# roymor1/OptimalStrategiesAgainstGenerativeAttacks

Measured on AMD Instinct MI355X. Metric: GIM episodes/sec (64x64x3, m=1 n=5 k=10), higher is better.
Workload: dtype f32

## Files before the change

### include/gim_hip.h

```cpp
#ifndef GIM_HIP_H
#define GIM_HIP_H

#include <stddef.h>
#include <stdint.h>

#ifdef __cplusplus
extern "C" {
#endif

#define GIM_OK 0
#define GIM_E_BADARG (-1)
#define GIM_E_LAUNCH (-2)

const char* gim_last_error(void);
int gim_version(void);

typedef struct {
    int32_t N, H, W, Cin, Cout, KH, ups;
    float pre_slope;
    int32_t pool, wfold, res_ups;
    int32_t tune_tile, tune_ksplit, tune_wgrad;
    int32_t out_zeroed;
    float post_slope;
    int32_t prec;
} gim_conv_shape;

int gim_conv2d_fold_weights(const float* w, float* f, int Cout, int Cin, int KH, void* stream);
typedef struct {
    const float* w;
    float* f;
    int32_t Cout, Cin, KH, reserved;
} gim_fold_job;
int gim_conv2d_fold_weights_batched(const gim_fold_job* jobs, const int32_t* tab, int n_blocks, void* stream);

int gim_conv2d_fwd(const float* x, const float* w, const float* bias, const float* sigma, const float* residual,
                   float* y, const gim_conv_shape* s, void* stream);

int gim_conv2d_dgrad(const float* dy, const float* w, const float* sigma, const float* mask_x, float* dx,
                     const gim_conv_shape* s, void* stream);

int gim_conv2d_dgrad_res(const float* dy, const float* w, const float* sigma, const float* mask_x, const float* res_half,
                         float res_scale, float* dx, const gim_conv_shape* s, void* stream);

int gim_conv2d_wgrad_slabs(const gim_conv_shape* s);
int gim_conv2d_wgrad(const float* dy, const float* x, float* slabs, float* bias_slabs, int n_slabs, const gim_conv_shape* s,
                     void* stream);

int gim_wgrad_finish(const float* slabs, const float* bias_slabs, int n_slabs, const float* w, const float* sigma,
                     const float* u, const float* v, float* dw, float* db, float* scratch, int Cout, int Cin, int KH,
                     int fold, float* acc_dw, float* acc_db, void* stream);

int gim_spectral_sigma(const float* w, float* u, float* v, float* sigma, float* u_out, float* v_out, float* scratch,
                       int Cout, int Cin, int KH, int training, void* stream);

typedef struct {
    const float* w;
    float* u;
    float* v;
    int64_t off_sigma, off_u, off_v, off_scratch;
    int32_t Cout, Cin, KH, reserved;
} gim_sn_job;
int gim_spectral_sigma_batched(const gim_sn_job* jobs, int n_jobs, const int32_t* tab_cols, int n_col_blocks,
                               const int32_t* tab_rows, int n_row_blocks, float* out_base, int training, void* stream);

int gim_conv2d_transpose_weights(const float* w, float* wt, int Cout, int Cin, int KF, void* stream);
int gim_conv2d_dgrad_t(const float* dy, const float* wt, const float* sigma, const float* mask_x, float* dx,
                       const gim_conv_shape* shape, void* stream);

int gim_conv2d_xfold_weights(const float* w, float* wx, int Cout, int Cin, int KH, int J, void* stream);
int gim_conv2d_dgrad_xfold(const float* dy, const float* wx, const float* sigma, const float* mask_x, float* dx,
                           const gim_conv_shape* shape, int J, void* stream);

int gim_pad_image(const float* x, float* xp, int N, int H, int W, int C, int pad, float slope, void* stream);
int gim_conv2d_pack_rows_weights(const float* w, float* wp, int Cout, int Cin, int KH, void* stream);
int gim_conv2d_fwd_rows(const float* xp, const float* wp, const float* bias, const float* sigma, const float* residual,
                        float* y, const gim_conv_shape* shape, void* stream);
int gim_conv2d_wgrad_rows_acc(const float* dy, const float* xp, float* acc, float* bias_acc, const gim_conv_shape* shape, void* stream);

int gim_conv2d_pack_subpixel_weights(const float* wf, float* wm, int Cout, int Cin, int KH, void* stream);
int gim_depth_to_space2(const float* y4, const float* bias, float* y, int N, int Hs, int Ws, int C, float post_slope, void* stream);

int gim_conv_launch_plan(const gim_conv_shape* shape, int kind, int32_t* out);

int gim_conv2d_wgrad_acc(const float* dy, const float* x, float* acc, float* bias_acc, const gim_conv_shape* shape, void* stream);

typedef struct {
    const float* src;
    const float* bias_src;
    const float* w;
    const float* sigma;
    const float* u;
    const float* v;
    float* tmp;
    float* partial;
    float* grad_w;
    float* grad_b;
    int32_t Cout, Cin, K, fold;
    int32_t n_chunks, exclusive;
} gim_wgrad_job;
int gim_wgrad_finish_batched(const gim_wgrad_job* jobs, int n_jobs, const int32_t* tab, int n_blocks, const int32_t* tab_sn,
                             int n_blocks_sn, void* stream);

int gim_colsum(const float* x, float* out, float* scratch, int64_t rows, int C, void* stream);

int gim_colsum_acc(const float* x, float* out, float* scratch, int64_t rows, int C, void* stream);
int gim_colsum2(const float* a, const float* b, float* out_a, float* out_b, int rows, int C, int accumulate, void* stream);

int gim_norm_fwd(const float* x, const float* scale, const float* shift, const float* residual, float* y, float* stats,
                 int N, int HW, int C, int mode, float eps, void* stream);
int gim_norm_fwd_act(const float* x, const float* scale, const float* shift, const float* residual, float* y, float* stats,
                     int N, int HW, int C, int mode, float eps, float post_slope, void* stream);
int gim_norm_bwd(const float* dy, const float* x, const float* scale, const float* stats, float* dx, float* dscale_nc,
                 float* dshift_nc, int N, int HW, int C, int mode, void* stream);

int gim_avgpool2_fwd(const float* x, float* y, int N, int H, int W, int C, void* stream);
int gim_avgpool2_fwd_act(const float* x, float* y, int N, int H, int W, int C, float in_slope, void* stream);
int gim_box2_fwd(const float* x, float* p, int N, int H, int W, int C, float slope, void* stream);
int gim_add_n(const float* a, const float* b, const float* c, const float* d, float* out, int64_t n, void* stream);
int gim_add_avgpool2_bwd(const float* g, const float* dy_pooled, float* out, int N, int H, int W, int C, void* stream);
int gim_avgpool2_bwd(const float* dy, float* dx, int N, int H, int W, int C, void* stream);
int gim_upsample2x_bwd(const float* dy_up, const float* mask_x, float slope, float* dx, int N, int H, int W, int C, void* stream);

int gim_maxpool_lrelu_fwd(const float* x, float* y, int32_t* idx, int N, int HW, int C, float slope, void* stream);
int gim_maxpool_lrelu_bwd(const float* dy, const float* y, const int32_t* idx, float* dx, int N, int HW, int C, float slope, void* stream);

int gim_attn_prob_fwd(const float* f, const float* g, float* P, int batch, int T, int K, void* stream);

int gim_bgemm(const float* A, const float* B, float* C, int batch, int M, int N, int K,
              int64_t sAb, int64_t sAi, int64_t sAk, int64_t sBb, int64_t sBk, int64_t sBj, void* stream);

typedef struct {
    const float* A;
    const float* B;
    float* C;
    const float* bias;
    int32_t M, N, K, ldc;
    int64_t sAi, sAk, sBk, sBj;
    int32_t flags, reserved;
} gim_gemm_job;
int gim_bgemm_grouped(const gim_gemm_job* jobs, const int32_t* tiles, int n_tiles, void* stream);
int gim_colsum_grouped(const gim_gemm_job* jobs, const int32_t* tiles, int n_tiles, void* stream);

int gim_softmax_dim1_fwd(const float* s, float* p, int B, int R, int Ccols, void* stream);
int gim_softmax_dim1_bwd(const float* dp, const float* p, float* ds, int B, int R, int Ccols, void* stream);

int gim_scale_add_fwd(const float* a, const float* x, const float* gamma, float* y, int64_t n, void* stream);
int gim_scale_add_fwd_act(const float* a, const float* x, const float* gamma, float* y, int64_t n, float post_slope, void* stream);
int gim_scale_add_bwd(const float* dy, const float* a, const float* gamma, float* da, float* dgamma, float* scratch,
                      int64_t n, void* stream);

int gim_tanh_fwd(const float* x, float* y, int64_t n, void* stream);
int gim_tanh_bwd(const float* dy, const float* y, float* dx, int64_t n, void* stream);

int gim_nchw_to_nhwc(const float* x, float* y, int N, int C, int HW, void* stream);
int gim_nhwc_to_nchw(const float* x, float* y, int N, int C, int HW, void* stream);

int gim_set_stats_fwd(const float* x, float* mean, float* std, int B, int t, int D, int64_t ld_mean, int64_t ld_std, void* stream);
int gim_set_stats_bwd(const float* x, const float* dmean, const float* dstd, float* dx, int B, int t, int D,
                      int64_t ld_dmean, int64_t ld_dstd, void* stream);

int gim_bce_logits_fwd(const float* x, float* loss, float target, int n, void* stream);
int gim_bce_logits_bwd(const float* dloss, const float* x, float* dx, float target, int n, void* stream);

int gim_sum_dim1(const float* x, float* y, int B, int t, int D, float scale, void* stream);
int gim_repeat_dim1(const float* x, float* y, int B, int t, int D, float scale, void* stream);
// ... 125 lines not shown
```

### optimalstrategiesagainstgenerativeattacks_amd/_lib.py

```python
import ctypes
import os
from ctypes import POINTER, c_float, c_int, c_int32, c_int64, c_uint64, c_void_p

_HERE = os.path.dirname(os.path.abspath(__file__))
LIB_PATH = os.environ.get("GIM_LIB_PATH") or os.path.join(_HERE, "csrc", "libgim_hip.so")


class GimConvShape(ctypes.Structure):
    _fields_ = [("N", c_int32), ("H", c_int32), ("W", c_int32), ("Cin", c_int32), ("Cout", c_int32),
                ("KH", c_int32), ("ups", c_int32), ("pre_slope", c_float),
                ("pool", c_int32), ("wfold", c_int32), ("res_ups", c_int32),
                ("tune_tile", c_int32), ("tune_ksplit", c_int32), ("tune_wgrad", c_int32),
                ("out_zeroed", c_int32), ("post_slope", c_float), ("prec", c_int32)]


class GimInferConv(ctypes.Structure):
    _fields_ = [("N", c_int32), ("H", c_int32), ("W", c_int32), ("Cin", c_int32), ("Cout", c_int32),
                ("KH", c_int32), ("stride", c_int32)]


P = c_void_p
SP = POINTER(GimConvShape)


class GimFoldJob(ctypes.Structure):
    _fields_ = [("w", P), ("f", P), ("Cout", c_int32), ("Cin", c_int32), ("KH", c_int32), ("reserved", c_int32)]


class GimSnJob(ctypes.Structure):
    _fields_ = [("w", P), ("u", P), ("v", P), ("off_sigma", c_int64), ("off_u", c_int64), ("off_v", c_int64), ("off_scratch", c_int64),
                ("Cout", c_int32), ("Cin", c_int32), ("KH", c_int32), ("reserved", c_int32)]


class GimWgradJob(ctypes.Structure):
    _fields_ = [("src", P), ("bias_src", P), ("w", P), ("sigma", P), ("u", P), ("v", P), ("tmp", P), ("partial", P),
                ("grad_w", P), ("grad_b", P), ("Cout", c_int32), ("Cin", c_int32), ("K", c_int32), ("fold", c_int32),
                ("n_chunks", c_int32), ("exclusive", c_int32)]


class GimGemmJob(ctypes.Structure):
    _fields_ = [("A", P), ("B", P), ("C", P), ("bias", P), ("M", c_int32), ("N", c_int32), ("K", c_int32), ("ldc", c_int32),
                ("sAi", c_int64), ("sAk", c_int64), ("sBk", c_int64), ("sBj", c_int64), ("flags", c_int32), ("reserved", c_int32)]


SIGNATURES = {
    "gim_conv2d_fwd": [P, P, P, P, P, P, SP, P],
    "gim_conv2d_dgrad": [P, P, P, P, P, SP, P],
    "gim_conv2d_dgrad_res": [P, P, P, P, P, c_float, P, SP, P],
    "gim_conv2d_wgrad_slabs": [SP],
    "gim_conv2d_wgrad": [P, P, P, P, c_int, SP, P],
    "gim_wgrad_finish": [P, P, c_int, P, P, P, P, P, P, P, c_int, c_int, c_int, c_int, P, P, P],
    "gim_conv2d_fold_weights": [P, P, c_int, c_int, c_int, P],
    "gim_conv2d_fold_weights_batched": [P, P, c_int, P],
    "gim_spectral_sigma": [P, P, P, P, P, P, P, c_int, c_int, c_int, c_int, P],
    "gim_spectral_sigma_batched": [P, c_int, P, c_int, P, c_int, P, c_int, P],
    "gim_colsum": [P, P, P, c_int64, c_int, P],
    "gim_norm_fwd": [P, P, P, P, P, P, c_int, c_int, c_int, c_int, c_float, P],
    "gim_norm_fwd_act": [P, P, P, P, P, P, c_int, c_int, c_int, c_int, c_float, c_float, P],
    "gim_norm_bwd": [P, P, P, P, P, P, P, c_int, c_int, c_int, c_int, P],
    "gim_avgpool2_fwd": [P, P, c_int, c_int, c_int, c_int, P],
    "gim_avgpool2_fwd_act": [P, P, c_int, c_int, c_int, c_int, c_float, P],
    "gim_box2_fwd": [P, P, c_int, c_int, c_int, c_int, c_float, P],
    "gim_add_n": [P, P, P, P, P, c_int64, P],
    "gim_add_avgpool2_bwd": [P, P, P, c_int, c_int, c_int, c_int, P],
    "gim_avgpool2_bwd": [P, P, c_int, c_int, c_int, c_int, P],
    "gim_upsample2x_bwd": [P, P, c_float, P, c_int, c_int, c_int, c_int, P],
    "gim_maxpool_lrelu_fwd": [P, P, P, c_int, c_int, c_int, c_float, P],
    "gim_maxpool_lrelu_bwd": [P, P, P, P, c_int, c_int, c_int, c_float, P],
    "gim_bgemm": [P, P, P, c_int, c_int, c_int, c_int, c_int64, c_int64, c_int64, c_int64, c_int64, c_int64, P],
    "gim_attn_prob_fwd": [P, P, P, c_int, c_int, c_int, P],
    "gim_softmax_dim1_fwd": [P, P, c_int, c_int, c_int, P],
    "gim_softmax_dim1_bwd": [P, P, P, c_int, c_int, c_int, P],
    "gim_bgemm_grouped": [P, P, c_int, P],
    "gim_colsum_grouped": [P, P, c_int, P],
    "gim_scale_add_fwd": [P, P, P, P, c_int64, P],
    "gim_scale_add_fwd_act": [P, P, P, P, c_int64, c_float, P],
    "gim_scale_add_bwd": [P, P, P, P, P, P, c_int64, P],
    "gim_tanh_fwd": [P, P, c_int64, P],
    "gim_tanh_bwd": [P, P, P, c_int64, P],
    "gim_nchw_to_nhwc": [P, P, c_int, c_int, c_int, P],
    "gim_nhwc_to_nchw": [P, P, c_int, c_int, c_int, P],
    "gim_set_stats_fwd": [P, P, P, c_int, c_int, c_int, c_int64, c_int64, P],
    "gim_set_stats_bwd": [P, P, P, P, c_int, c_int, c_int, c_int64, c_int64, P],
    "gim_bce_logits_fwd": [P, P, c_float, c_int, P],
    "gim_bce_logits_bwd": [P, P, P, c_float, c_int, P],
    "gim_sum_dim1": [P, P, c_int, c_int, c_int, c_float, P],
    "gim_repeat_dim1": [P, P, c_int, c_int, c_int, c_float, P],
    "gim_noise_combine": [P, P, P, c_int, c_int, c_int, c_int, P],
    "gim_concat2": [P, P, P, c_int64, c_int, c_int, c_int, c_int, P],
    "gim_slice_channels": [P, P, c_int64, c_int, c_int, P],
    "gim_conv2d_wgrad_acc": [P, P, P, P, SP, P],
    "gim_wgrad_finish_batched": [P, c_int, P, c_int, P, c_int, P],
    "gim_colsum_acc": [P, P, P, c_int64, c_int, P],
    "gim_colsum2": [P, P, P, P, c_int, c_int, c_int, P],
    "gim_conv_launch_plan": [SP, c_int, P],
    "gim_conv2d_transpose_weights": [P, P, c_int, c_int, c_int, P],
    "gim_conv2d_dgrad_t": [P, P, P, P, P, SP, P],
    "gim_conv2d_xfold_weights": [P, P, c_int, c_int, c_int, c_int, P],
    "gim_conv2d_dgrad_xfold": [P, P, P, P, P, SP, c_int, P],
    "gim_episode_gather": [P, P, P, P, c_int, c_int, c_int, c_int, P],
    "gim_resize_bilinear_u8": [P, c_int64, c_int, c_int, c_int, c_int, P, c_int, c_int, P, P, c_int, P, P, c_int, P],
    "gim_maxpool_gather": [P, P, P, P, c_int, c_int, c_int, c_float, P],
    "gim_softmax_dim1_bwd_dp": [P, P, P, P, c_int, c_int, c_int, P],
    "gim_set_stats_bwd_bwd": [P, P, P, P, P, P, c_int, c_int, c_int, c_int64, c_int64, P],
    "gim_lrelu_mask_mul": [P, P, c_float, P, c_int64, P],
    "gim_sqsum_rows_fwd": [P, P, c_int, c_int64, P],
    "gim_sqsum_rows_bwd": [P, P, P, c_int, c_int64, P],
    "gim_img_att_mix_fwd": [P, P, P, P, P, P, P, P, c_int64, c_int, P],
    "gim_img_att_mix_bwd": [P, P, P, P, P, P, P, P, P, P, P, P, P, P, c_int64, c_int, P],
    "gim_adam_step": [P, P, P, P, c_int64, P, P, c_int, c_float, c_float, c_float, c_float, P, P],
    "gim_adam_step_scaled": [P, P, P, P, c_int64, P, P, c_int, c_float, c_float, c_float, c_float, P, P, P],
    "gim_ema_update": [P, P, c_int64, c_float, P, P],
    "gim_buffer_exchange": [P, P, c_int64, P],
    "gim_adam_optimism": [P, P, P, P, c_int64, P, P, c_int, c_float, c_float, c_float, c_float, P, P, P],
    "gim_spin": [c_int, P],
    "gim_pad_image": [P, P, c_int, c_int, c_int, c_int, c_int, c_float, P],
    "gim_conv2d_pack_rows_weights": [P, P, c_int, c_int, c_int, P],
    "gim_conv2d_pack_subpixel_weights": [P, P, c_int, c_int, c_int, P],
    "gim_depth_to_space2": [P, P, P, c_int, c_int, c_int, c_int, c_float, P],
    "gim_conv2d_fwd_rows": [P, P, P, P, P, P, SP, P],
    "gim_conv2d_wgrad_rows_acc": [P, P, P, P, SP, P],
    "gim_conv2d_infer": [P, P, P, P, P, POINTER(GimInferConv), P],
    "gim_maxpool2_act": [P, P, c_int, c_int, c_int, c_int, c_int, P],
    "gim_channel_affine": [P, P, P, P, c_int64, c_int, P],
    "gim_se_tail": [P, P, P, P, P, P, P, c_int, c_int, c_int, c_int, c_int, P],
    "gim_pair_score": [P, P, P, c_int, c_int, P],
    "gim_l2norm_rows": [P, P, c_int, c_int, P],
    "gim_absdiff": [P, P, P, c_int64, P],
    "gim_bn_slabs": [c_int64],
    "gim_bn_partials_floats": [c_int64, c_int],
    "gim_bn_stats": [P, P, P, P, P, P, P, c_int64, c_int, c_float, c_float, P],
    "gim_bn_relu_maxpool2_fwd": [P, P, P, P, P, P, c_int, c_int, c_int, c_int, P],
    "gim_bn_pool_bwd_reduce": [P, P, P, P, P, P, P, P, P, P, P, c_int, c_int, c_int, c_int, P],
    "gim_bn_pool_bwd_dx": [P, P, P, P, P, P, P, P, P, c_int, c_int, c_int, c_int, P],
    "gim_bn_stats_record": [P, P, P, c_int64, c_int, P],
    "gim_bn_stats_merge": [P, POINTER(c_int64), c_int, c_int, P, P, P, P, P, c_float, c_float, P],
    "gim_bn_pool_bwd_dx_total": [P, P, P, P, P, P, P, P, P, c_int, c_int, c_int, c_int, c_int64, P],
    "gim_absdiff_bwd": [P, P, P, P, P, c_int64, P],
    "gim_logit_accuracy": [P, c_int, c_int, P, P],
    "gim_bn_apply_fwd": [P, P, P, P, P, P, P, c_int64, c_int, P],
    "gim_bn_bwd_reduce": [P, P, P, P, P, P, P, P, P, P, P, P, P, P, c_int64, c_int, P],
    "gim_bn_bwd_dx": [P, P, P, P, P, P, P, P, P, P, c_int64, c_int, P],
    "gim_bn_bwd_dx_total": [P, P, P, P, P, P, P, P, P, P, c_int64, c_int64, c_int, P],
    "gim_prelu_fwd": [P, P, P, c_int64, c_int, P],
    "gim_prelu_bwd": [P, P, P, P, P, P, P, c_int64, c_int, P],
    "gim_se_tail_bwd": [P, P, P, P, P, c_int, c_int, c_int, c_int, P],
    "gim_subsample2_fwd": [P, P, c_int, c_int, c_int, c_int, P],
    "gim_subsample2_bwd": [P, P, c_int, c_int, c_int, c_int, P],
    "gim_dropout": [P, P, c_int64, c_float, c_uint64, c_uint64, P],
    "gim_l2norm_rows_bwd": [P, P, P, c_int, c_int, P],
    "gim_col_l2norm_fwd": [P, P, c_int, c_int, P],
    "gim_col_l2norm_bwd": [P, P, P, c_int, c_int, P],
    "gim_arcface_margin_fwd": [P, P, P, c_int, c_int, c_float, c_float, c_float, c_float, c_float, P],
    "gim_arcface_margin_bwd": [P, P, P, P, c_int, c_int, c_float, c_float, c_float, c_float, c_float, P],
    "gim_softmax_ce_fwd": [P, P, P, P, P, c_int, c_int, P],
    "gim_softmax_ce_bwd": [P, P, P, P, P, c_int, c_int, P],
    "gim_conv2d_strided_fwd": [P, P, P, P, POINTER(GimInferConv), P],
    "gim_conv2d_strided_dgrad": [P, P, P, POINTER(GimInferConv), c_int, P],
    "gim_conv2d_strided_wgrad_workspace": [POINTER(GimInferConv), POINTER(c_int64)],
    "gim_conv2d_strided_wgrad": [P, P, P, P, POINTER(GimInferConv), c_int, P, P],
    "gim_conv2d_strided_plan": [POINTER(GimInferConv), c_int, P],
    "gim_roc_slices": [c_int64, c_int64],
    "gim_roc_counts": [P, c_int, P, c_int, P, c_int, P, P],
    "gim_roc_calibrate": [P, c_int, P, c_int, P, P, P],
    "gim_version": [],
}

_lib = None


def load():
    global _lib
    if _lib is not None:
        return _lib
    if not os.path.exists(LIB_PATH):
        raise RuntimeError(
            "libgim_hip.so not found at %s: the HIP extension is not built "
            "(run __graft_entry__.build()); there is no CPU fallback" % LIB_PATH)
# ... 16 lines not shown
```

### optimalstrategiesagainstgenerativeattacks_amd/csrc/conv_f16.inc

```
typedef _Float16 h8_t __attribute__((ext_vector_type(8)));
typedef _Float16 h4_t __attribute__((ext_vector_type(4)));
typedef _Float16 h2_t __attribute__((ext_vector_type(2)));
typedef float f32x2 __attribute__((ext_vector_type(2)));
typedef short s16x4 __attribute__((ext_vector_type(4)));

template <bool SAT>
__device__ __forceinline__ f32x4 sat16(f32x4 v) {
    if constexpr (SAT) {
#pragma unroll
        for (int e = 0; e < 4; ++e) v[e] = __builtin_amdgcn_fmed3f(v[e], -65504.f, 65504.f);
    }
    return v;
}
template <bool SAT>
__device__ __forceinline__ h8_t cvt8_f16(f32x4 lo, f32x4 hi) {
    lo = sat16<SAT>(lo); hi = sat16<SAT>(hi);
    const h2_t a = __builtin_convertvector(f32x2{lo[0], lo[1]}, h2_t), b = __builtin_convertvector(f32x2{lo[2], lo[3]}, h2_t);
    const h2_t c = __builtin_convertvector(f32x2{hi[0], hi[1]}, h2_t), d = __builtin_convertvector(f32x2{hi[2], hi[3]}, h2_t);
    return h8_t{a[0], a[1], b[0], b[1], c[0], c[1], d[0], d[1]};
}
template <bool SAT>
__device__ __forceinline__ h4_t cvt4_f16(f32x4 v) {
    v = sat16<SAT>(v);
    const h2_t a = __builtin_convertvector(f32x2{v[0], v[1]}, h2_t), b = __builtin_convertvector(f32x2{v[2], v[3]}, h2_t);
// ... 70 lines not shown
#pragma unroll
        for (int i = 0; i < B_ROWS; ++i) {
            rb[i][0] = buf_load4(rw, b_voff[i], sb);
            rb[i][1] = buf_load4(rw, b_voff[i], sb + 16u);
        }
        k_c0 += KB;
        if (k_c0 == p.Ca) {
            k_c0 = 0;
            if (++k_tb == g.Tw) { k_tb = 0; ++k_ta; }
            set_tap(k_ta, k_tb);
        }
    };
    const bool has_act = p.pre_slope != 1.0f;
    auto store_tiles = [&](int buf) {
#pragma unroll
        for (int i = 0; i < A_ROWS; ++i) {
            if (has_act) {
#pragma unroll
                for (int q = 0; q < 2; ++q)
#pragma unroll
                    for (int e = 0; e < 4; ++e) ra[i][q][e] = __builtin_amdgcn_fmed3f(ra[i][q][e], ra[i][q][e] * p.pre_slope, p.pos_inf);
            }
            *reinterpret_cast<h8_t*>(&As[buf * A_SZ + (arow + 64 * i) * LDH + aq]) = cvt8_f16<SAT>(ra[i][0], ra[i][1]);
        }
#pragma unroll
        for (int i = 0; i < B_ROWS; ++i)
            *reinterpret_cast<h8_t*>(&Bs[buf * B_SZ + (arow + 64 * i) * LDH + aq]) = cvt8_f16<false>(rb[i][0], rb[i][1]);
    };
    const int lane = t & 63, r = lane & 31, h = lane >> 5, wv = t >> 6;
    const int wm0 = (wv / WAVES_N) * 32 * TM, wn0 = (wv % WAVES_N) * 32 * TN;
    f32x16 acc[TM][TN];
#pragma unroll
    for (int i = 0; i < TM; ++i)
#pragma unroll
        for (int j = 0; j < TN; ++j)
#pragma unroll
            for (int e = 0; e < 16; ++e) acc[i][j][e] = 0.f;
    const int nk_all = p.Ktot / KB;
    const int ks0 = kslice * p.kper;
    const int nk = min(nk_all, ks0 + p.kper);
    seek(ks0 * KB);
    load_tiles();
    store_tiles(0);
    __syncthreads();
    auto kstep = [&](int ks, auto BUFC, auto MAINC) {
        constexpr int buf = decltype(BUFC)::value;
        constexpr bool MAIN = decltype(MAINC)::value;
        if (MAIN || ks + 1 < nk) load_tiles();
        __builtin_amdgcn_sched_barrier(0);
        const _Float16* Ab = As + buf * A_SZ;
        const _Float16* Bb = Bs + buf * B_SZ;
        h8_t a[2][TM], b[2][TN];
#pragma unroll
        for (int kk = 0; kk < 2; ++kk) {
#pragma unroll
            for (int i = 0; i < TM; ++i) a[kk][i] = *reinterpret_cast<const h8_t*>(&Ab[(wm0 + 32 * i + r) * LDH + 16 * kk + 8 * h]);
#pragma unroll
            for (int j = 0; j < TN; ++j) b[kk][j] = *reinterpret_cast<const h8_t*>(&Bb[(wn0 + 32 * j + r) * LDH + 16 * kk + 8 * h]);
        }
#pragma unroll
        for (int kk = 0; kk < 2; ++kk)
#pragma unroll
            for (int i = 0; i < TM; ++i)
#pragma unroll
                for (int j = 0; j < TN; ++j)
                    acc[i][j] = __builtin_amdgcn_mfma_f32_32x32x16_f16(a[kk][i], b[kk][j], acc[i][j], 0, 0, 0);
        __builtin_amdgcn_sched_barrier(0);
        if (MAIN || ks + 1 < nk) store_tiles(buf ^ 1);
        __syncthreads();
    };
    int ks = ks0;
    for (; ks + 2 < nk; ks += 2) {
        kstep(ks, std::integral_constant<int, 0>(), std::true_type());
        kstep(ks + 1, std::integral_constant<int, 1>(), std::true_type());
    }
    for (; ks < nk; ks += 2) {
        kstep(ks, std::integral_constant<int, 0>(), std::false_type());
        if (ks + 1 < nk) kstep(ks + 1, std::integral_constant<int, 1>(), std::false_type());
    }

    EpiCtx ec;
    const bool first = kslice == 0;
    bool has_res, has_mask;
    epi_fill<false, false>(ec, p, g, first, has_res, has_mask);
    auto run = [&](auto MODEC) {
        constexpr int MODE = decltype(MODEC)::value;
#pragma unroll
        for (int i = 0; i < TM; ++i)
#pragma unroll
            for (int j = 0; j < TN; ++j) {
                const int co = n0 + wn0 + 32 * j + r;
                const bool cok = co < p.Cb;
                const float bv = (p.bias && first && cok) ? p.bias[co] : 0.f;
                float a_[16];
#pragma unroll
                for (int e = 0; e < 16; ++e) a_[e] = acc[i][j][e];
                epi_block<16, MODE>(ec, a_, m0 + wm0 + 32 * i + 4 * h, co, cok, bv);
            }
    };
    epi_dispatch<0, 0>(p, has_res, has_mask, run);
}

template <int BM, int BN, int TM, int TN, bool SAT = true>
__global__ __launch_bounds__(256, 2) void conv_igemm_patch_f16_kernel(const ConvP p) {
    constexpr int KB = 32, LDH = 40;
    constexpr int WAVES_N = BN / (32 * TN), WAVES_M = BM / (32 * TM);
    static_assert(WAVES_M * WAVES_N == 4, "4 waves per workgroup");
    constexpr int P_PER = BM == 64 ? 4 : 5;
    constexpr int B_ROWS = BN / 64;
    constexpr int B_SZ = BN * LDH;
    extern __shared__ __attribute__((aligned(16))) _Float16 patch16_lds[];
    const Geo& g = p.g;
    const int t = threadIdx.x, lane = t & 63, wv = t >> 6;
    const int kslice = blockIdx.z;
    const int m0 = blockIdx.x * BM, n0 = blockIdx.y * BN;
    const int Wt = min(g.W, BM), logWt = 31 - __builtin_clz(Wt);
    const int PW = Wt + 2, PP = (BM / Wt + 2) * PW;
    const int P_SZ = (PP * LDH + 7) & ~7;
    _Float16* Ps = patch16_lds;
    _Float16* Bs = patch16_lds + 2 * P_SZ;
    const int n_img = m0 >> (g.logH + g.logW);
    const int oy0 = ((m0 >> g.logW) & (g.H - 1)) + g.off_y, ox0 = (m0 & (g.W - 1)) + g.off_x;
    const int KF2 = g.KF * g.KFw;
    const __amdgpu_buffer_rsrc_t rx = __builtin_amdgcn_make_buffer_rsrc((void*)p.x, 0, p.x_bytes, 0x00020000);
    const __amdgpu_buffer_rsrc_t rw = __builtin_amdgcn_make_buffer_rsrc((void*)p.w, 0, 0xFFFFFFFFu, 0x00020000);
    unsigned p_voff[P_PER];
    int p_lds[P_PER];
#pragma unroll
    for (int i = 0; i < P_PER; ++i) {
        const int q = t + 256 * i, pp = q >> 2, grp = q & 3;
        const int pr = pp / PW, pc = pp - pr * PW;
        const int iy = oy0 + pr, ix = ox0 + pc;
        const bool v = pp < PP && (unsigned)iy < (unsigned)g.H && (unsigned)ix < (unsigned)g.W;
        p_voff[i] = v ? (unsigned)((((n_img * g.Hin + iy) * g.Win + ix) * p.Ca + grp * 8) * 4) : BUF_OOB;
        p_lds[i] = pp < PP ? pp * LDH + grp * 8 : -1;
    }
    unsigned b_voff[B_ROWS];
    const int brow = t >> 2, bq = (t & 3) * 8;
#pragma unroll
    for (int i = 0; i < B_ROWS; ++i) b_voff[i] = (unsigned)((min(n0 + brow + 64 * i, p.Cb - 1) * KF2 * p.Cin_w + bq) * 4);
    const bool has_act = p.pre_slope != 1.0f;
    f32x4 rp[P_PER][2], rb[B_ROWS][2];
    auto load_patch = [&](int c0) __attribute__((always_inline)) {
#pragma unroll
        for (int i = 0; i < P_PER; ++i) {
            rp[i][0] = buf_load4(rx, p_voff[i], (unsigned)(c0 * 4));
            rp[i][1] = buf_load4(rx, p_voff[i], (unsigned)(c0 * 4) + 16u);
        }
    };
    int p_wr = 0;
    auto store_patch = [&]() __attribute__((always_inline)) {
#pragma unroll
        for (int i = 0; i < P_PER; ++i) {
            if (has_act) {
#pragma unroll
                for (int q = 0; q < 2; ++q)
#pragma unroll
                    for (int e = 0; e < 4; ++e) rp[i][q][e] = __builtin_amdgcn_fmed3f(rp[i][q][e], rp[i][q][e] * p.pre_slope, p.pos_inf);
            }
            if (p_lds[i] >= 0) *reinterpret_cast<h8_t*>(&Ps[p_wr + p_lds[i]]) = cvt8_f16<SAT>(rp[i][0], rp[i][1]);
        }
        p_wr = p_wr ? 0 : P_SZ;
    };
    auto load_b = [&](int ta, int tb, int c0) __attribute__((always_inline)) {
        const int wtap = (g.wa_base + g.wa_step * ta) * g.KFw + g.wb_base + g.wb_step * tb;
        const unsigned sb = (unsigned)((wtap * p.Cin_w + c0) * 4);
#pragma unroll
// ... 11 lines not shown
    int a_row[3][TM];
#pragma unroll
    for (int i = 0; i < TM; ++i) {
        const int q = wm0 + 32 * i + r;
        const int base = ((q >> logWt) * PW + (q & (Wt - 1))) * LDH + 8 * h;
#pragma unroll
        for (int ta = 0; ta < 3; ++ta) a_row[ta][i] = base + ta * PW * LDH;
    }
    f32x16 acc[TM][TN];
#pragma unroll
    for (int i = 0; i < TM; ++i)
#pragma unroll
        for (int j = 0; j < TN; ++j)
#pragma unroll
            for (int e = 0; e < 16; ++e) acc[i][j][e] = 0.f;
    const int nchunk = p.Ca / KB;
    const int ch0 = kslice * (p.kper / 9);
    const int ch1 = min(nchunk, ch0 + p.kper / 9);
    load_patch(ch0 * KB);
    load_b(0, 0, ch0 * KB);
    store_patch();
    store_b(0);
    __syncthreads();
    auto kstep = [&](int ch, bool more_chunks, auto TAPC, auto BBC) __attribute__((always_inline)) {
        constexpr int TAP = decltype(TAPC)::value, BB = decltype(BBC)::value;
        constexpr int TA = TAP / 3, TB = TAP % 3;
        if (TAP == 0 && more_chunks) load_patch((ch + 1) * KB);
        if (TAP < 8) load_b((TAP + 1) / 3, (TAP + 1) % 3, ch * KB);
        else if (more_chunks) load_b(0, 0, (ch + 1) * KB);
        __builtin_amdgcn_sched_barrier(0);
        const _Float16* Bb = Bs + BB * B_SZ;
        h8_t a[2][TM], b[2][TN];
#pragma unroll
        for (int kk = 0; kk < 2; ++kk) {
#pragma unroll
            for (int i = 0; i < TM; ++i) a[kk][i] = *reinterpret_cast<const h8_t*>(&Ps[a_row[TA][i] + TB * LDH + 16 * kk]);
#pragma unroll
            for (int j = 0; j < TN; ++j) b[kk][j] = *reinterpret_cast<const h8_t*>(&Bb[(wn0 + 32 * j + r) * LDH + 16 * kk + 8 * h]);
        }
#pragma unroll
        for (int kk = 0; kk < 2; ++kk)
#pragma unroll
            for (int i = 0; i < TM; ++i)
#pragma unroll
                for (int j = 0; j < TN; ++j)
                    acc[i][j] = __builtin_amdgcn_mfma_f32_32x32x16_f16(a[kk][i], b[kk][j], acc[i][j], 0, 0, 0);
        __builtin_amdgcn_sched_barrier(0);
        if (TAP < 8 || more_chunks) store_b(BB ^ 1);
        if (TAP == 8 && more_chunks) store_patch();
        __syncthreads();
    };
    int pbuf = 0;
    auto chunk = [&](int ch, auto B0C) __attribute__((always_inline)) {
        constexpr int B0 = decltype(B0C)::value;
        using Ba = std::integral_constant<int, B0>;
        using Bb_ = std::integral_constant<int, B0 ^ 1>;
        const bool more_chunks = ch + 1 < ch1;
        kstep(ch, more_chunks, std::integral_constant<int, 0>(), Ba());
        kstep(ch, more_chunks, std::integral_constant<int, 1>(), Bb_());
        kstep(ch, more_chunks, std::integral_constant<int, 2>(), Ba());
        kstep(ch, more_chunks, std::integral_constant<int, 3>(), Bb_());
        kstep(ch, more_chunks, std::integral_constant<int, 4>(), Ba());
        kstep(ch, more_chunks, std::integral_constant<int, 5>(), Bb_());
        kstep(ch, more_chunks, std::integral_constant<int, 6>(), Ba());
        kstep(ch, more_chunks, std::integral_constant<int, 7>(), Bb_());
        kstep(ch, more_chunks, std::integral_constant<int, 8>(), Ba());
        const int d = pbuf ? -P_SZ : P_SZ;
        pbuf ^= 1;
#pragma unroll
        for (int ta = 0; ta < 3; ++ta)
#pragma unroll
            for (int i = 0; i < TM; ++i) a_row[ta][i] += d;
    };
    int ch = ch0;
    for (; ch + 1 < ch1; ch += 2) {
        chunk(ch, std::integral_constant<int, 0>());
        chunk(ch + 1, std::integral_constant<int, 1>());
    }
    if (ch < ch1) chunk(ch, std::integral_constant<int, 0>());

    EpiCtx ec;
    const bool first = kslice == 0;
    bool has_res, has_mask;
    epi_fill<true, false>(ec, p, g, first, has_res, has_mask);
    auto run = [&](auto MODEC) {
        constexpr int MODE = decltype(MODEC)::value;
#pragma unroll
        for (int i = 0; i < TM; ++i)
#pragma unroll
            for (int j = 0; j < TN; ++j) {
                const int co = n0 + wn0 + 32 * j + r;
                const bool cok = co < p.Cb;
                const float bv = (p.bias && first && cok) ? p.bias[co] : 0.f;
                float a_[16];
#pragma unroll
                for (int e = 0; e < 16; ++e) a_[e] = acc[i][j][e];
                epi_block<16, MODE>(ec, a_, m0 + wm0 + 32 * i + 4 * h, co, cok, bv);
            }
    };
    epi_dispatch<0, 0>(p, has_res, has_mask, run);
}

__device__ __forceinline__ int wg16_off(int row, int chunk) {
    return 256 * row + 16 * (chunk ^ (((row & 3) << 2) | ((row >> 2) & 3)));
}

template <bool FASTB, bool SAT = true>
__global__ __launch_bounds__(256, 2) void conv_wgrad_f16_kernel(const WgP p) {
    constexpr int BM = 128, BN = 128, TM = 2, TN = 2, WBK = 32;
    constexpr int IMG = WBK * 256;
    constexpr int PER = 4;
    __shared__ __attribute__((aligned(16))) char lds[4 * IMG];
    const Geo& g = p.g;
    const int t = threadIdx.x;
    int bx, by, bz;
    if (!wgrad_block(p, bx, by, bz)) return;
    const int j0 = bx * BN, co0 = by * BM;
    const int mbeg = bz * p.mper, mend = min(p.M, mbeg + p.mper);
    const int He = g.Hin << g.ups, We = g.Win << g.ups;
    const int cq = t & 31, ak = t >> 5;
    const int ac = cq * 4;
    const int j = j0 + ac;
    const bool b_jok = j < p.Kcols;
    const int tap = b_jok ? j / p.Cin : 0;
    const int ci = b_jok ? j - tap * p.Cin : 0;
    const int ta = tap / g.Tw, tb = tap - ta * g.Tw;
    const int dh = ta + g.off_y, dw = tb + g.off_x;
    const bool do_bias = p.bias_slabs != nullptr && bx == 0;
    const int b_bias = ((g.off_y < 0 ? -g.off_y : 0) * g.Win + (g.off_x < 0 ? -g.off_x : 0)) * p.Cin * 4;
    const __amdgpu_buffer_rsrc_t rxb = __builtin_amdgcn_make_buffer_rsrc((void*)((const char*)p.x - b_bias), 0, p.x_bytes + (unsigned)b_bias, 0x00020000);
    unsigned a_v[PER], b_l[PER];
    int b_dx[PER], b_dy[PER], st_off[PER];
    const bool a_cok = co0 + ac < p.Cout;
#pragma unroll
    for (int i = 0; i < PER; ++i) {
        const int row = ak + 8 * i;
        a_v[i] = a_cok ? (unsigned)((row * p.Cout + co0 + ac) * 4) : BUF_OOB;
        b_dy[i] = (row >> g.logW) * g.s_in + dh;
        b_dx[i] = (row & (g.W - 1)) * g.s_in + dw;
        b_l[i] = b_jok ? (unsigned)(((b_dy[i] * g.Win + b_dx[i]) * p.Cin + ci) * 4 + b_bias) : BUF_OOB;
        st_off[i] = wg16_off(row, cq >> 1) + 8 * (cq & 1);
    }
    f32x4 ra[PER], rb[PER];
    float bsum[4] = {0.f, 0.f, 0.f, 0.f};
    auto load_tiles = [&](int mb) {
        const int left = mend - mb;
        const __amdgpu_buffer_rsrc_t ra_rs = __builtin_amdgcn_make_buffer_rsrc(
            (void*)(p.dy + (long long)mb * p.Cout), 0, (unsigned)min(left, WBK) * (unsigned)p.Cout * 4u, 0x00020000);
#pragma unroll
        for (int i = 0; i < PER; ++i) ra[i] = buf_load4(ra_rs, a_v[i], 0);
        if constexpr (FASTB) {
            const int n = mb >> (g.logH + g.logW);
            const int oys = ((mb >> g.logW) & (g.H - 1)) * g.s_in, oxs = (mb & (g.W - 1)) * g.s_in;
            const unsigned u = (unsigned)((((n * g.Hin + oys) * g.Win) + oxs) * p.Cin * 4);
#pragma unroll
            for (int i = 0; i < PER; ++i) {
                const bool v = (unsigned)(oys + b_dy[i]) < (unsigned)He && (unsigned)(oxs + b_dx[i]) < (unsigned)We;
                rb[i] = buf_load4(rxb, v ? b_l[i] : BUF_OOB, u);
            }
        } else {
#pragma unroll
            for (int i = 0; i < PER; ++i) {
                const int m = mb + ak + 8 * i;
                const int n = m >> (g.logH + g.logW);
                const int iy = ((m >> g.logW) & (g.H - 1)) * g.s_in + dh;
                const int ix = (m & (g.W - 1)) * g.s_in + dw;
                const bool v = b_jok && m < mend && (unsigned)iy < (unsigned)He && (unsigned)ix < (unsigned)We;
// ... 137 lines not shown
```

### optimalstrategiesagainstgenerativeattacks_amd/csrc/conv_igemm.hip

```cpp
#include <stdlib.h>

#include "common.h"
#include <type_traits>

#define PM_MAX_PIXELS 16
#define PM_MIN_IMAGES 32
#define BK 16

struct Geo {
    int N, H, W, logH, logW;
    int Hin, Win;
    int ups;
    int s_in;
    int s_in_x;
    int off_y, off_x;
    int Th, Tw;
    int KF;
    int KFw;
    int wa_base, wa_step, wb_base, wb_step;
    int os, py, px;
    int pc, pc_kind, pc_K;
    int pm;
    unsigned long long pm_perm;
    unsigned long long pm_perm_cls[4];
};

__host__ __device__ __forceinline__ int pm_pixel(unsigned long long perm, int slot) { return (int)((perm >> (4 * slot)) & 15ull); }


__device__ __forceinline__ void geo_row(const Geo& g, int m, int& n, int& oy, int& ox) {
    if (g.pm) {
        const int slot = m / g.N;
        n = m - slot * g.N;
        const int pix = pm_pixel(g.pm_perm, slot);
        oy = pix >> g.logW;
        ox = pix & (g.W - 1);
    } else {
        n = m >> (g.logH + g.logW);
        oy = (m >> g.logW) & (g.H - 1);
        ox = m & (g.W - 1);
    }
}

__host__ __device__ __forceinline__ void geo_select_class(Geo& g, int cls) {
    const int py = cls >> 1, px = cls & 1;
    const int K = g.pc_K, pd = (K - 1) / 2;
    g.py = py;
    g.px = px;
    if (g.pc_kind == 0) {
        const int oy = (py - pd) >> 1, ox = (px - pd) >> 1;
        g.off_y = oy;
        g.off_x = ox;
        g.wa_base = pd + 1 - py + 2 * oy;
        g.wb_base = pd + 1 - px + 2 * ox;
        g.wa_step = g.wb_step = 2;
    } else {
        const int th = (K + 1) / 2;
        const int a0 = (py + pd) & 1, b0 = (px + pd) & 1;
        g.off_y = ((py + pd - a0) >> 1) - (th - 1);
        g.off_x = ((px + pd - b0) >> 1) - (th - 1);
        g.wa_base = a0 + 2 * (th - 1);
        g.wb_base = b0 + 2 * (th - 1);
        g.wa_step = g.wb_step = -2;
    }
}

struct ConvP {
    Geo g;
    const float* x;
    const float* w;
    const float* bias;
    const float* sigma;
    const float* res;
    const float* mask_x;
    float* y;
    int Ca, Cb;
    int Cin_w;
    int M;
    int Ktot;
    const float* zero;
    unsigned x_bytes;
    int tune_ks;
    int tune_tile;
    int y_zeroed;
    int tune_kind;
    float pos_inf;
    float pre_slope, mask_slope, out_scale;
    float res_scale;
    float post_slope;
    int res_ups;
    int ksplit;
    int kper;
    int pix;
    int f16;
    const float* slope;
    int epi;
    int no_split;
};

__device__ __attribute__((aligned(16))) float g_zero4[4] = {0.f, 0.f, 0.f, 0.f};

static const float* zero_page() {
    static const float* z = [] {
        void* ptr = nullptr;
        if (hipGetSymbolAddress(&ptr, HIP_SYMBOL(g_zero4)) != hipSuccess) ptr = nullptr;
        return (const float*)ptr;
    }();
    return z;
}

typedef unsigned u32x4 __attribute__((ext_vector_type(4)));
#define BUF_OOB 0x80000000u
#define BUF_MAX_BYTES 0x7FFFFFF0ull
__device__ __forceinline__ f32x4 buf_load4(__amdgpu_buffer_rsrc_t r, unsigned voff, unsigned soff) {
    return __builtin_bit_cast(f32x4, __builtin_amdgcn_raw_buffer_load_b128(r, voff, soff, 0));
}

struct EpiCtx {
    __amdgpu_buffer_rsrc_t ry, rr, rm;
    float scale, mask_slope, post_slope;
    float res_scale;
    int M, Cb, logH, logW, Hm1, Wm1, os, py, px, Ho, Wo;
    int pmN;
    unsigned long long pm_perm;
    bool atom, remap;
};

template <int MODE>
__device__ __forceinline__ void epi_elem_off(const EpiCtx& c, int m, int co, unsigned& o, unsigned& ro) {
    const int n = m >> (c.logH + c.logW);
    const int oy = ((m >> c.logW) & c.Hm1) * c.os + c.py;
    const int ox = (m & c.Wm1) * c.os + c.px;
    o = (unsigned)((((n * c.Ho + oy) * c.Wo + ox) * c.Cb + co) * 4);
    if constexpr (MODE == 2 || MODE == 4) ro = (unsigned)((((n * (c.Ho >> 1) + (oy >> 1)) * (c.Wo >> 1) + (ox >> 1)) * c.Cb + co) * 4);
}

template <int NE, int MODE>
__device__ __forceinline__ void epi_block(const EpiCtx& c, const float (&a)[NE], int mbase, int co, bool cok, float bv, float sv = 1.f) {
    constexpr int CH = NE < 8 ? NE : 8;
    const unsigned rowb = (unsigned)c.Cb * 4u;
#pragma unroll
    for (int e0 = 0; e0 < NE; e0 += CH) {
        unsigned off[CH], roff[(MODE == 2 || MODE == 4) ? CH : 1];
        if (!c.remap && !c.pmN && MODE != 2 && MODE != 4) {
            const unsigned base = (unsigned)((mbase * c.Cb + co) * 4);
#pragma unroll
            for (int q = 0; q < CH; ++q) off[q] = base + (unsigned)(((e0 + q) & 3) + 8 * ((e0 + q) >> 2)) * rowb;
        } else if (c.Wm1 >= 3 && !c.pmN) {
#pragma unroll
            for (int g4 = 0; g4 < CH; g4 += 4) {
                unsigned o, ro = 0;
                epi_elem_off<MODE>(c, mbase + 8 * ((e0 + g4) >> 2), co, o, ro);
#pragma unroll
                for (int k = 0; k < 4 && g4 + k < CH; ++k) {
                    off[g4 + k] = o + (unsigned)(k * c.os) * rowb;
                    if constexpr (MODE == 2 || MODE == 4) roff[g4 + k] = ro + (unsigned)(((c.px + k * c.os) >> 1) - (c.px >> 1)) * rowb;
                }
            }
        } else if (c.pmN) {
            const int slot0 = mbase / c.pmN, n0 = mbase - slot0 * c.pmN;
            const int pixa = pm_pixel(c.pm_perm, slot0), pixb = pm_pixel(c.pm_perm, (slot0 + 1) & 15);
#pragma unroll
            for (int q = 0; q < CH; ++q) {
                const int d = ((e0 + q) & 3) + 8 * ((e0 + q) >> 2);
                const bool wrap = n0 + d >= c.pmN;
                const int n = wrap ? n0 + d - c.pmN : n0 + d, pix = wrap ? pixb : pixa;
                const int oy = ((pix >> c.logW) & c.Hm1) * c.os + c.py, ox = (pix & c.Wm1) * c.os + c.px;
                off[q] = (unsigned)((((n * c.Ho + oy) * c.Wo + ox) * c.Cb + co) * 4);
                if constexpr (MODE == 2 || MODE == 4) roff[q] = (unsigned)((((n * (c.Ho >> 1) + (oy >> 1)) * (c.Wo >> 1) + (ox >> 1)) * c.Cb + co) * 4);
            }
        } else {
#pragma unroll
            for (int q = 0; q < CH; ++q) {
                unsigned ro = 0;
                epi_elem_off<MODE>(c, mbase + ((e0 + q) & 3) + 8 * ((e0 + q) >> 2), co, off[q], ro);
                if constexpr (MODE == 2 || MODE == 4) roff[q] = ro;
            }
        }
#pragma unroll
        for (int q = 0; q < CH; ++q) {
            const unsigned bad = (cok && mbase + ((e0 + q) & 3) + 8 * ((e0 + q) >> 2) < c.M) ? 0u : BUF_OOB;
            off[q] |= bad;
            if constexpr (MODE == 2 || MODE == 4) roff[q] |= bad;
        }
        float ld[(MODE == 0 || MODE == 5) ? 1 : CH], ld2[MODE == 4 ? CH : 1];
        if constexpr (MODE == 4) {
#pragma unroll
            for (int q = 0; q < CH; ++q) ld[q] = __builtin_bit_cast(float, __builtin_amdgcn_raw_buffer_load_b32(c.rm, off[q], 0, 0));
#pragma unroll
            for (int q = 0; q < CH; ++q) ld2[q] = __builtin_bit_cast(float, __builtin_amdgcn_raw_buffer_load_b32(c.rr, roff[q], 0, 0));
        } else if constexpr (MODE == 1 || MODE == 2) {
#pragma unroll
            for (int q = 0; q < CH; ++q) ld[q] = __builtin_bit_cast(float, __builtin_amdgcn_raw_buffer_load_b32(c.rr, MODE == 2 ? roff[q] : off[q], 0, 0));
        } else if constexpr (MODE == 3) {
#pragma unroll
            for (int q = 0; q < CH; ++q) ld[q] = __builtin_bit_cast(float, __builtin_amdgcn_raw_buffer_load_b32(c.rm, off[q], 0, 0));
        }
        float v[CH];
#pragma unroll
        for (int q = 0; q < CH; ++q) {
            v[q] = a[e0 + q] * c.scale + bv;
            if constexpr (MODE == 1 || MODE == 2) v[q] += ld[q];
            if constexpr (MODE == 3 || MODE == 4) v[q] *= (ld[q] > 0.f ? 1.0f : c.mask_slope);
            if constexpr (MODE == 4) v[q] += c.res_scale * ld2[q];
            if constexpr (MODE == 5) v[q] = v[q] >= 0.f ? v[q] : v[q] * sv;
            else if constexpr (MODE != 3 && MODE != 4) v[q] = fmaxf(v[q], v[q] * c.post_slope);
        }
        if (c.atom) {
#pragma unroll
            for (int q = 0; q < CH; ++q) (void)__builtin_amdgcn_raw_ptr_buffer_atomic_fadd_f32(v[q], c.ry, off[q], 0, 0);
        } else {
#pragma unroll
            for (int q = 0; q < CH; ++q) __builtin_amdgcn_raw_buffer_store_b32(__builtin_bit_cast(unsigned, v[q]), c.ry, off[q], 0, 0);
        }
        __builtin_amdgcn_sched_barrier(0);
    }
}

template <bool PLAIN, bool PM>
__device__ __forceinline__ void epi_fill(EpiCtx& ec, const ConvP& p, const Geo& g, bool first, bool& has_res, bool& has_mask) {
    ec.scale = p.out_scale * (p.sigma ? 1.0f / p.sigma[0] : 1.0f);
    ec.mask_slope = p.mask_slope;
    ec.post_slope = p.post_slope;
    ec.res_scale = p.res_scale;
    has_res = p.res != nullptr && first;
    has_mask = p.mask_x != nullptr;
    ec.atom = p.ksplit > 1;
    ec.remap = PLAIN ? false : g.os != 1;
    ec.M = p.M; ec.Cb = p.Cb;
    ec.logH = g.logH; ec.logW = g.logW; ec.Hm1 = g.H - 1; ec.Wm1 = g.W - 1;
    ec.os = PLAIN ? 1 : g.os; ec.py = PLAIN ? 0 : g.py; ec.px = PLAIN ? 0 : g.px;
    ec.Ho = g.H * ec.os; ec.Wo = g.W * ec.os;
    ec.pmN = (PM && g.pm) ? g.N : 0;
    if constexpr (PM) ec.pm_perm = g.pm_perm;
    const unsigned ybytes = (unsigned)g.N * (unsigned)ec.Ho * (unsigned)ec.Wo * (unsigned)p.Cb * 4u;
    ec.ry = __builtin_amdgcn_make_buffer_rsrc((void*)p.y, 0, ybytes, 0x00020000);
    ec.rr = __builtin_amdgcn_make_buffer_rsrc((void*)p.res, 0, has_res ? ((p.res_ups || has_mask) ? ybytes >> 2 : ybytes) : 0u, 0x00020000);
    ec.rm = __builtin_amdgcn_make_buffer_rsrc((void*)p.mask_x, 0, has_mask ? ybytes : 0u, 0x00020000);
}

template <int EPI, int BMODE, class Run>
__device__ __forceinline__ void epi_dispatch(const ConvP& p, bool has_res, bool has_mask, Run&& run) {
    if constexpr (EPI == 1) {
        run(std::integral_constant<int, 5>());
    } else if (has_res) {
        if constexpr (BMODE == 1) run(std::integral_constant<int, 4>());
        else if (p.res_ups) run(std::integral_constant<int, 2>());
        else run(std::integral_constant<int, 1>());
    } else if (has_mask) {
        run(std::integral_constant<int, 3>());
    } else {
        run(std::integral_constant<int, 0>());
    }
}

constexpr int igemm_lds_bytes(int BM, int BN, int KB, int BMODE) {
    return 2 * (BM * (KB + 4) + (BMODE == 0 ? BN * (KB + 4) : KB * BN)) * 4;
}

template <int BM, int BN, int TM, int TN, int BMODE, int GENF, int KB, int EPI = 0>
__global__ __launch_bounds__(256, igemm_lds_bytes(BM, BN, KB, BMODE) <= 40960 ? 4 : 2) void conv_igemm_kernel(const ConvP p) {
    constexpr bool GEN = (GENF & 1) != 0;
    constexpr bool BSCALAR = (GENF & 2) != 0;
    constexpr bool N16 = BN == 16;
    constexpr int WAVES_N = N16 ? 1 : BN / (32 * TN);
    constexpr int WAVES_M = BM / (32 * TM);
    static_assert(WAVES_M * WAVES_N == 4, "4 waves per workgroup");
    constexpr int LDK = KB + 4;
    constexpr int QPR = KB / 4;
    constexpr int RP = 256 / QPR;
    constexpr int A_ROWS = BM / RP;
    constexpr int B_ROWS = (BN + RP - 1) / RP;
    constexpr int B_PER = KB * BN / 256;
    constexpr int B_U = BN / 4;
    constexpr int B_RSTEP = 256 / B_U;
    constexpr int B_PER4 = (KB + B_RSTEP - 1) / B_RSTEP;
    constexpr int LDA = LDK;
    constexpr int A_SZ = BM * LDA;
    constexpr int B_SZ = (BMODE == 0) ? BN * LDA : KB * BN;
    __shared__ __attribute__((aligned(16))) float lds[2 * A_SZ + 2 * B_SZ];
    float* As = lds;
    float* Bs = lds + 2 * A_SZ;

    Geo g = p.g;
    int kslice = blockIdx.z;
    if (g.pc) {
        geo_select_class(g, blockIdx.z & 3);
        g.pm_perm = p.g.pm_perm_cls[blockIdx.z & 3];
        kslice = blockIdx.z >> 2;
    }
    const int t = threadIdx.x;
    const int m0 = blockIdx.x * BM;
    const int n0 = blockIdx.y * BN;
    const int arow = t / QPR, aq = (t % QPR) * 4;
    const int He = g.Hin << g.ups, We = g.Win << g.ups;
    const int KF2 = g.KF * g.KFw;

    int a_oy[A_ROWS], a_ox[A_ROWS];
    long long a_off[A_ROWS];
    bool a_ok[A_ROWS];
#pragma unroll
    for (int i = 0; i < A_ROWS; ++i) {
        const int m = m0 + arow + RP * i;
        a_ok[i] = m < p.M;
// ... 260 lines not shown
            const int per = (nv + p.ksplit - 1) / p.ksplit;
            ks0 = kslice * per;
            nk = min(nv, ks0 + per);
            if (ks0 >= nk) {
                if (kslice != 0) return;
            }
            pm_seek(ks0);
            set_tap(k_ta, k_tb);
            pm_started = true;
        }
    }
    if constexpr (!GEN) { if (!pm_started) seek(ks0 * KB); }
    load_tiles(ks0 * KB);
    store_tiles(0);
    __syncthreads();
    auto kstep = [&](int ks, auto BUFC, auto MAINC) {
        constexpr int buf = decltype(BUFC)::value;
        constexpr bool MAIN = decltype(MAINC)::value;
        if (MAIN || ks + 1 < nk) load_tiles((ks + 1) * KB);
        __builtin_amdgcn_sched_barrier(0);
        const float* Ab = As + buf * A_SZ;
        const float* Bb = Bs + buf * B_SZ;
        if constexpr (N16) {
#pragma unroll
            for (int kk = 0; kk < KB / 16; ++kk) {
                f32x4 a[NB16], b;
#pragma unroll
                for (int i = 0; i < NB16; ++i) a[i] = *reinterpret_cast<const f32x4*>(&Ab[(wm0 + 16 * i + r16) * LDK + 16 * kk + 4 * q16]);
                if constexpr (BMODE == 0) {
                    b = *reinterpret_cast<const f32x4*>(&Bb[r16 * LDK + 16 * kk + 4 * q16]);
                } else {
#pragma unroll
                    for (int e = 0; e < 4; ++e) b[e] = Bb[(16 * kk + 4 * q16 + e) * BN + r16];
                }
#pragma unroll
                for (int e = 0; e < 4; ++e)
#pragma unroll
                    for (int i = 0; i < NB16; ++i) acc16[i] = __builtin_amdgcn_mfma_f32_16x16x4f32(a[i][e], b[e], acc16[i], 0, 0, 0);
            }
        } else {
            f32x4 a[KB / 8][TM], b[KB / 8][TN];
#pragma unroll
            for (int kk = 0; kk < KB / 8; ++kk) {
#pragma unroll
                for (int i = 0; i < TM; ++i) a[kk][i] = *reinterpret_cast<const f32x4*>(&Ab[(wm0 + 32 * i + r) * LDK + 8 * kk + 4 * h]);
#pragma unroll
                for (int j = 0; j < TN; ++j) {
                    if constexpr (BMODE == 0) {
                        b[kk][j] = *reinterpret_cast<const f32x4*>(&Bb[(wn0 + 32 * j + r) * LDK + 8 * kk + 4 * h]);
                    } else {
#pragma unroll
                        for (int e = 0; e < 4; ++e) b[kk][j][e] = Bb[(8 * kk + 4 * h + e) * BN + wn0 + 32 * j + r];
                    }
                }
            }
            if constexpr (TM * TN <= 2) __builtin_amdgcn_sched_barrier(0);
#pragma unroll
            for (int kk = 0; kk < KB / 8; ++kk)
#pragma unroll
                for (int e = 0; e < 4; ++e)
#pragma unroll
                    for (int i = 0; i < TM; ++i)
#pragma unroll
                        for (int j = 0; j < TN; ++j)
                            acc[i][j] = __builtin_amdgcn_mfma_f32_32x32x2f32(a[kk][i][e], b[kk][j][e], acc[i][j], 0, 0, 0);
        }
        __builtin_amdgcn_sched_barrier(0);
        if (MAIN || ks + 1 < nk) store_tiles(buf ^ 1);
        __syncthreads();
    };
    int ks = ks0;
    for (; ks + 2 < nk; ks += 2) {
        kstep(ks, std::integral_constant<int, 0>(), std::true_type());
        kstep(ks + 1, std::integral_constant<int, 1>(), std::true_type());
    }
    for (; ks < nk; ks += 2) {
        kstep(ks, std::integral_constant<int, 0>(), std::false_type());
        if (ks + 1 < nk) kstep(ks + 1, std::integral_constant<int, 1>(), std::false_type());
    }

    EpiCtx ec;
    const bool first = kslice == 0;
    bool has_res, has_mask;
    epi_fill<false, true>(ec, p, g, first, has_res, has_mask);
    auto run = [&](auto MODEC) {
        constexpr int MODE = decltype(MODEC)::value;
        if constexpr (N16) {
            const int co = n0 + r16;
            const bool cok = co < p.Cb;
            const float bv = (p.bias && first && cok) ? p.bias[co] : 0.f;
#pragma unroll
            for (int i = 0; i < NB16; ++i) {
                const float a[4] = {acc16[i][0], acc16[i][1], acc16[i][2], acc16[i][3]};
                if constexpr (MODE == 5) epi_block<4, MODE>(ec, a, m0 + wm0 + 16 * i + 4 * q16, co, cok, bv, (p.slope && cok) ? p.slope[co] : 1.f);
                else epi_block<4, MODE>(ec, a, m0 + wm0 + 16 * i + 4 * q16, co, cok, bv);
            }
        } else {
#pragma unroll
            for (int i = 0; i < TM; ++i)
#pragma unroll
                for (int j = 0; j < TN; ++j) {
                    const int co = n0 + wn0 + 32 * j + r;
                    const bool cok = co < p.Cb;
                    const float bv = (p.bias && first && cok) ? p.bias[co] : 0.f;
                    float a[16];
#pragma unroll
                    for (int e = 0; e < 16; ++e) a[e] = acc[i][j][e];
                    if constexpr (MODE == 5) epi_block<16, MODE>(ec, a, m0 + wm0 + 32 * i + 4 * h, co, cok, bv, (p.slope && cok) ? p.slope[co] : 1.f);
                    else epi_block<16, MODE>(ec, a, m0 + wm0 + 32 * i + 4 * h, co, cok, bv);
                }
        }
    };
    epi_dispatch<EPI, BMODE>(p, has_res, has_mask, run);
}

template <int BM, int BN, int TM, int TN, int BMODE, int EPI = 0>
__global__ __launch_bounds__(256, TM * TN <= 2 ? 3 : 2) void conv_igemm_patch_kernel(const ConvP p) {
    constexpr int KB = 16, LDK = KB + 4;
    constexpr int WAVES_N = BN / (32 * TN), WAVES_M = BM / (32 * TM);
    static_assert(WAVES_M * WAVES_N == 4, "4 waves per workgroup");
    constexpr int P_PER = BM == 64 ? 4 : 5;
    constexpr int B_ROWS = BN / 64;
    constexpr int B_U = BN / 4, B_RSTEP = 256 / B_U;
    constexpr int B_PER4 = (KB + B_RSTEP - 1) / B_RSTEP;
    constexpr int B_SZ = (BMODE == 0) ? BN * LDK : KB * BN;
    extern __shared__ __attribute__((aligned(16))) float patch_lds[];
    const Geo& g = p.g;
    const int t = threadIdx.x, lane = t & 63, wv = t >> 6;
    const int kslice = blockIdx.z;
    const int m0 = blockIdx.x * BM, n0 = blockIdx.y * BN;
    const int Wt = min(g.W, BM), logWt = 31 - __builtin_clz(Wt);
    const int PW = Wt + 2, PP = (BM / Wt + 2) * PW;
    const int P_SZ = (PP * LDK + 3) & ~3;
    float* Ps = patch_lds;
    float* Bs = patch_lds + 2 * P_SZ;
    const int n_img = m0 >> (g.logH + g.logW);
    const int oy0 = ((m0 >> g.logW) & (g.H - 1)) + g.off_y, ox0 = (m0 & (g.W - 1)) + g.off_x;
    const int KF2 = g.KF * g.KFw;
    const __amdgpu_buffer_rsrc_t rx = __builtin_amdgcn_make_buffer_rsrc((void*)p.x, 0, p.x_bytes, 0x00020000);
    const __amdgpu_buffer_rsrc_t rw = __builtin_amdgcn_make_buffer_rsrc((void*)p.w, 0, 0xFFFFFFFFu, 0x00020000);
    unsigned p_voff[P_PER];
    int p_lds[P_PER];
#pragma unroll
    for (int i = 0; i < P_PER; ++i) {
        const int q = t + 256 * i, pp = q >> 2, quad = q & 3;
        const int pr = pp / PW, pc = pp - pr * PW;
        const int iy = oy0 + pr, ix = ox0 + pc;
        const bool v = pp < PP && (unsigned)iy < (unsigned)g.H && (unsigned)ix < (unsigned)g.W;
        p_voff[i] = v ? (unsigned)((((n_img * g.Hin + iy) * g.Win + ix) * p.Ca + quad * 4) * 4) : BUF_OOB;
        p_lds[i] = pp < PP ? pp * LDK + quad * 4 : -1;
    }
    unsigned b_voff[BMODE == 0 ? B_ROWS : B_PER4];
    const int brow = t >> 2, bq = (t & 3) * 4;
    const int b4_krow = t / B_U, b4_col = (t % B_U) * 4;
    if constexpr (BMODE == 0) {
#pragma unroll
        for (int i = 0; i < B_ROWS; ++i) b_voff[i] = (unsigned)((min(n0 + brow + 64 * i, p.Cb - 1) * KF2 * p.Cin_w + bq) * 4);
    } else {
#pragma unroll
        for (int i = 0; i < B_PER4; ++i)
            b_voff[i] = (unsigned)((min(b4_krow + i * B_RSTEP, KB - 1) * KF2 * p.Cin_w + min(n0 + b4_col, p.Cb - 4)) * 4);
    }
    const bool has_act = p.pre_slope != 1.0f;
    f32x4 rp[P_PER], rb[BMODE == 0 ? B_ROWS : B_PER4];
    auto load_patch = [&](int c0) __attribute__((always_inline)) {
#pragma unroll
        for (int i = 0; i < P_PER; ++i) rp[i] = buf_load4(rx, p_voff[i], (unsigned)(c0 * 4));
// ... 50 lines not shown
#pragma unroll
        for (int j = 0; j < TN; ++j)
#pragma unroll
            for (int e = 0; e < 16; ++e) acc[i][j][e] = 0.f;

    const int nchunk = p.Ca / KB;
    const int ch0 = kslice * (p.kper / 9);
    const int ch1 = min(nchunk, ch0 + p.kper / 9);
    load_patch(ch0 * KB);
    load_b(0, 0, ch0 * KB);
    store_patch();
    store_b(0);
    __syncthreads();
    auto kstep = [&](int ch, bool more_chunks, auto TAPC, auto BBC) __attribute__((always_inline)) {
        constexpr int TAP = decltype(TAPC)::value, BB = decltype(BBC)::value;
        constexpr int TA = TAP / 3, TB = TAP % 3;
        if (TAP == 0 && more_chunks) load_patch((ch + 1) * KB);
        if (TAP < 8) load_b((TAP + 1) / 3, (TAP + 1) % 3, ch * KB);
        else if (more_chunks) load_b(0, 0, (ch + 1) * KB);
        __builtin_amdgcn_sched_barrier(0);
        const float* Bb = Bs + BB * B_SZ;
        f32x4 a[2][TM], b[2][TN];
#pragma unroll
        for (int kk = 0; kk < 2; ++kk) {
#pragma unroll
            for (int i = 0; i < TM; ++i) a[kk][i] = *reinterpret_cast<const f32x4*>(&Ps[a_row[TA][i] + TB * LDK + 8 * kk]);
#pragma unroll
            for (int j = 0; j < TN; ++j) {
                if constexpr (BMODE == 0) {
                    b[kk][j] = *reinterpret_cast<const f32x4*>(&Bb[(wn0 + 32 * j + r) * LDK + 8 * kk + 4 * h]);
                } else {
#pragma unroll
                    for (int e = 0; e < 4; ++e) b[kk][j][e] = Bb[(8 * kk + 4 * h + e) * BN + wn0 + 32 * j + r];
                }
            }
        }
        if constexpr (TM * TN <= 2) __builtin_amdgcn_sched_barrier(0);
#pragma unroll
        for (int kk = 0; kk < 2; ++kk)
#pragma unroll
            for (int e = 0; e < 4; ++e)
#pragma unroll
                for (int i = 0; i < TM; ++i)
#pragma unroll
                    for (int j = 0; j < TN; ++j)
                        acc[i][j] = __builtin_amdgcn_mfma_f32_32x32x2f32(a[kk][i][e], b[kk][j][e], acc[i][j], 0, 0, 0);
        __builtin_amdgcn_sched_barrier(0);
        if (TAP < 8 || more_chunks) store_b(BB ^ 1);
        if (TAP == 8 && more_chunks) store_patch();
        __syncthreads();
    };
    int pbuf = 0;
    auto chunk = [&](int ch, auto B0C) __attribute__((always_inline)) {
        constexpr int B0 = decltype(B0C)::value;
        using Ba = std::integral_constant<int, B0>;
        using Bb_ = std::integral_constant<int, B0 ^ 1>;
        const bool more_chunks = ch + 1 < ch1;
        kstep(ch, more_chunks, std::integral_constant<int, 0>(), Ba());
        kstep(ch, more_chunks, std::integral_constant<int, 1>(), Bb_());
        kstep(ch, more_chunks, std::integral_constant<int, 2>(), Ba());
        kstep(ch, more_chunks, std::integral_constant<int, 3>(), Bb_());
        kstep(ch, more_chunks, std::integral_constant<int, 4>(), Ba());
        kstep(ch, more_chunks, std::integral_constant<int, 5>(), Bb_());
        kstep(ch, more_chunks, std::integral_constant<int, 6>(), Ba());
        kstep(ch, more_chunks, std::integral_constant<int, 7>(), Bb_());
        kstep(ch, more_chunks, std::integral_constant<int, 8>(), Ba());
        const int d = pbuf ? -P_SZ : P_SZ;
        pbuf ^= 1;
#pragma unroll
        for (int ta = 0; ta < 3; ++ta)
#pragma unroll
            for (int i = 0; i < TM; ++i) a_row[ta][i] += d;
    };
    int ch = ch0;
    for (; ch + 1 < ch1; ch += 2) {
        chunk(ch, std::integral_constant<int, 0>());
        chunk(ch + 1, std::integral_constant<int, 1>());
    }
    if (ch < ch1) chunk(ch, std::integral_constant<int, 0>());

    EpiCtx ec;
    const bool first = kslice == 0;
    bool has_res, has_mask;
    epi_fill<true, false>(ec, p, g, first, has_res, has_mask);
    auto run = [&](auto MODEC) {
        constexpr int MODE = decltype(MODEC)::value;
#pragma unroll
        for (int i = 0; i < TM; ++i)
#pragma unroll
            for (int j = 0; j < TN; ++j) {
                const int co = n0 + wn0 + 32 * j + r;
                const bool cok = co < p.Cb;
                const float bv = (p.bias && first && cok) ? p.bias[co] : 0.f;
                float a[16];
#pragma unroll
                for (int e = 0; e < 16; ++e) a[e] = acc[i][j][e];
                if constexpr (MODE == 5) epi_block<16, MODE>(ec, a, m0 + wm0 + 32 * i + 4 * h, co, cok, bv, (p.slope && cok) ? p.slope[co] : 1.f);
                else epi_block<16, MODE>(ec, a, m0 + wm0 + 32 * i + 4 * h, co, cok, bv);
            }
    };
    epi_dispatch<EPI, BMODE>(p, has_res, has_mask, run);
}

struct WgP {
    Geo g;
    const float* dy;
    const float* x;
    float* slabs;
    float* bias_slabs;
    int Cin, Cout;
    int M;
    int Kcols;
    int mper;
    float pre_slope;
    float a_slope;
    const float* zero;
    unsigned x_bytes;
    float pos_inf;
    int atomic;
    int ns;
    int xcd;
    int pix;
};

__device__ __forceinline__ bool wgrad_block(const WgP& p, int& bx, int& by, int& bz) {
    if (!p.xcd) {
        bx = blockIdx.x; by = blockIdx.y; bz = blockIdx.z;
        return true;
    }
    const unsigned gx = gridDim.x, gy = gridDim.y;
    const unsigned L = blockIdx.x + gx * (blockIdx.y + gy * blockIdx.z);
    const unsigned xcd = L & 7u, q = L >> 3, ntiles = gx * gy;
    const unsigned tile = (q + xcd * ((ntiles + 7u) / 8u)) % ntiles, slice = (q / ntiles) * 8u + xcd;
    bx = (int)(tile % gx); by = (int)(tile / gx); bz = (int)slice;
    return slice < (unsigned)p.ns;
}

template <int BM, int BN, int TM, int TN, int VA, int VB, bool FASTB, int WBK = BK>
__global__ __launch_bounds__(256, 1) void conv_wgrad_kernel(const WgP p) {
    constexpr int WAVES_N = BN / (32 * TN);
    constexpr int WAVES_M = BM / (32 * TM);
    static_assert(WAVES_M * WAVES_N == 4, "4 waves per workgroup");
    static_assert(!FASTB || VB == 4, "fast B addressing: vector path only");
    constexpr int AU = BM / VA, BU = BN / VB;
    constexpr int A_RSTEP = 256 / AU, B_RSTEP = 256 / BU;
    constexpr int A_PER = (WBK + A_RSTEP - 1) / A_RSTEP, B_PER = (WBK + B_RSTEP - 1) / B_RSTEP;
    constexpr int A_FLOATS = WBK * BM, B_FLOATS = WBK * BN;
    __shared__ __attribute__((aligned(16))) float As[2][A_FLOATS];
    __shared__ __attribute__((aligned(16))) float Bs[2][B_FLOATS];

    const Geo& g = p.g;
    const int t = threadIdx.x;
    int bx, by, bz;
    if (!wgrad_block(p, bx, by, bz)) return;
    const int j0 = bx * BN, co0 = by * BM;
    const int mbeg = bz * p.mper;
    const int mend = min(p.M, mbeg + p.mper);
    const int He = g.Hin << g.ups, We = g.Win << g.ups;

    const int ac = (t % AU) * VA, ak = t / AU;
    const bool a_cok = (co0 + ac) < p.Cout;
    const int bc = (t % BU) * VB, bk = t / BU;
    const int j = j0 + bc;
    const bool b_jok = j < p.Kcols;
    const int tap = b_jok ? j / p.Cin : 0;
    const int ci = b_jok ? j - tap * p.Cin : 0;
    const int ta = tap / g.Tw, tb = tap - ta * g.Tw;
// ... 551 lines not shown
                if ((unsigned)(oy + ta) < (unsigned)He && (unsigned)(ox + tb) < (unsigned)We) mk |= 1u << (ta * g.Tw + tb);
        mask[pix] = mk;
        order[pix] = pix;
    }
    for (int i = 1; i < P; ++i)
        for (int j = i; j > 0 && mask[order[j - 1]] > mask[order[j]]; --j) { const int t = order[j]; order[j] = order[j - 1]; order[j - 1] = t; }
    unsigned long long perm = 0;
    for (int sl = 0; sl < P; ++sl) perm |= (unsigned long long)order[sl] << (4 * sl);
    return perm;
}
static void pm_make_perms(Geo& g) {
    if (g.pc) {
        for (int cls = 0; cls < 4; ++cls) {
            Geo c = g;
            geo_select_class(c, cls);
            g.pm_perm_cls[cls] = pm_perm_of(c);
        }
    } else {
        g.pm_perm = pm_perm_of(g);
    }
}

static int pm_valid_permille(const Geo& g0, int M, int BM) {
    if (!g0.pm) return 1000;
    long long valid = 0, total = 0;
    for (int cls = 0; cls < (g0.pc ? 4 : 1); ++cls) {
        Geo g = g0;
        if (g.pc) { geo_select_class(g, cls); g.pm_perm = g0.pm_perm_cls[cls]; }
        const int He = g.Hin << g.ups, We = g.Win << g.ups;
        for (int m0 = 0; m0 < M; m0 += BM) {
            unsigned mask = 0;
            const int last = m0 + BM - 1 < M - 1 ? m0 + BM - 1 : M - 1;
            for (int slot = m0 / g.N; slot <= last / g.N; ++slot) {
                const int pix = pm_pixel(g.pm_perm, slot);
                const int oy = (pix >> g.logW) * g.s_in + g.off_y, ox = (pix & (g.W - 1)) * g.s_in_x + g.off_x;
                for (int ta = 0; ta < g.Th; ++ta)
                    for (int tb = 0; tb < g.Tw; ++tb)
                        if ((unsigned)(oy + ta) < (unsigned)He && (unsigned)(ox + tb) < (unsigned)We) mask |= 1u << (ta * g.Tw + tb);
            }
            valid += __builtin_popcount(mask);
            total += g.Th * g.Tw;
        }
    }
    return (int)((valid * 1000 + total / 2) / total);
}

static int plan_ksplit(long long wgs, int nk, int tile_area, int want_ks) {
    if (want_ks > 0) return want_ks > nk ? nk : want_ks;
    const long long target = tile_area >= 128 * 128 ? 512 : 1024;
    if (wgs >= target - target / 8 || nk < 16) return 1;
    long long ks = (target + wgs / 2) / wgs;
    if (ks > nk / 8) ks = nk / 8;
    if (ks > 6) ks = 6;
    return ks < 1 ? 1 : (int)ks;
}

enum IgemmFamily { IGEMM_TAP = 0, IGEMM_PATCH = 1, IGEMM_F16 = 2, IGEMM_PATCH_F16 = 3 };
struct IgemmPlan {
    int family;
    int BM, BN, KB;
    int ksplit, kper;
    int gx, gy, gz;
    int lds_bytes;
    int table_hit;
};

struct TileCfg { int code, BM, BN; };
static const TileCfg g_tiles[] = {{128, 128, 128}, {641, 64, 128}, {1264, 128, 64}, {64, 64, 64}, {12832, 128, 32}, {12816, 128, 16}};

static int heuristic_tile(int family, int M, int Cb, long long t128, bool rows128) {
    if (family == IGEMM_TAP || family == IGEMM_PATCH) {
        if (Cb > 64) return M <= 64 ? 641 : (t128 < GIM_SMALL_TILES ? 64 : 641);
        return M <= 64 ? 64 : 1264;
    }
    if (family == IGEMM_F16) {
        if (M <= 64 || t128 < GIM_SMALL_TILES) return 64;
        return Cb > 64 ? (t128 < 256 ? 641 : 128) : 1264;
    }
    if (Cb > 64) {
        if (rows128 && t128 >= 256) return 128;
        return (M > 64 && t128 >= GIM_SMALL_TILES) ? 641 : 64;
    }
    return (rows128 && t128 >= GIM_SMALL_TILES) ? 1264 : 64;
}

static IgemmPlan plan_igemm(ConvP& p, int bmode, int gen) {
    IgemmPlan q{};
    const Geo& g = p.g;
    const int M = p.M, Cb = p.Cb, HW = g.H * g.W, ncls = g.pc ? 4 : 1;
    const long long t128 = (long long)((M + 127) / 128) * ((Cb + 127) / 128) * ncls;
    const bool vec_ops = p.pix == p.Ca && Cb >= 32 && !((uintptr_t)p.x & 15) && !((uintptr_t)p.w & 15);
    const bool plain3x3 = !g.pc && !g.ups && g.s_in == 1 && g.s_in_x == 1 && g.os == 1 && g.Th == 3 && g.Tw == 3 && HW >= 64 && g.W >= 2;
    const bool rows128 = HW >= 128 && g.W <= 64;
    int want_ks = p.tune_ks, cfg;
    if (bmode == 0 && gen == 0 && p.f16 && p.Ca % 32 == 0 && vec_ops) {
        q.family = plain3x3 ? IGEMM_PATCH_F16 : IGEMM_F16;
        q.KB = 32;
        cfg = heuristic_tile(q.family, M, Cb, t128, rows128);
    } else {
        const bool forced = p.tune_tile != 0 || p.tune_ks > 0;
        const TuneEntry* te = forced ? nullptr : tune_lookup(p.tune_kind, M, p.Ca, Cb, p.Ktot, g.pc);
        if (te) want_ks = te->ks;
        q.table_hit = te != nullptr;
        int want = p.tune_tile > 0 ? p.tune_tile : (te ? te->tile : 0);
        const bool patch_row = want >= 20000;
        if (patch_row) want -= 20000;
        const bool patch_ok = gen == 0 && plain3x3 && vec_ops && p.Ca % 16 == 0 && !(bmode == 1 && Cb % 4 != 0);
        q.KB = 16;
        if ((patch_row || (!te && p.tune_tile == 0 && p.tune_ks == 0)) && patch_ok) {
            q.family = IGEMM_PATCH;
            cfg = want == 6432 ? 64 : want;
            if (cfg != 128 && cfg != 641 && cfg != 1264 && cfg != 64) cfg = heuristic_tile(q.family, M, Cb, t128, rows128);
            if (Cb <= 64 && (cfg == 128 || cfg == 641)) cfg = cfg == 128 ? 1264 : 64;
            if ((cfg == 128 || cfg == 1264) && !rows128) cfg = cfg == 128 ? 641 : 64;
            if (Cb <= 64 && cfg == 641) cfg = 64;
        } else {
            q.family = IGEMM_TAP;
            if (Cb > 64) {
                cfg = want ? want : heuristic_tile(q.family, M, Cb, t128, rows128);
                if (cfg != 641 && cfg != 1264 && cfg != 64 && cfg != 6432) cfg = 128;
            } else if (Cb > 32) {
                cfg = (want == 64 || want == 6432 || want == 1264) ? want : heuristic_tile(q.family, M, Cb, t128, rows128);
            } else {
                cfg = Cb > 16 ? 12832 : 12816;
            }
            if (cfg == 6432 && gen == 0 && p.Ca % 32 == 0) q.KB = 32;
            if (cfg == 6432) cfg = 64;
        }
    }
    for (const TileCfg& t : g_tiles)
        if (t.code == cfg) { q.BM = t.BM; q.BN = t.BN; }
#ifndef GIM_NO_PM
    if (q.family == IGEMM_TAP && gen == 0) {
        const int taps = g.Th * g.Tw;
        p.g.pm = (taps > 1 && taps <= 32 && HW <= PM_MAX_PIXELS && g.N >= PM_MIN_IMAGES && p.pix == p.Ca && p.Ca % q.KB == 0) ? 1 : 0;
        if (p.g.pm) pm_make_perms(p.g);
    }
#endif
    q.gx = (M + q.BM - 1) / q.BM;
    q.gy = (Cb + q.BN - 1) / q.BN;
    const bool patch = q.family == IGEMM_PATCH || q.family == IGEMM_PATCH_F16;
    if (patch) {
        const int chunks = p.Ca / q.KB, T = 9;
        int ks = p.no_split ? 1 : plan_ksplit((long long)q.gx * q.gy, chunks * T, q.BM * q.BN, want_ks);
        if (ks > chunks) ks = chunks;
        const int cps = (chunks + ks - 1) / ks;
        q.ksplit = (chunks + cps - 1) / cps;
        q.kper = cps * T;
        const int Wt = g.W < q.BM ? g.W : q.BM;
        const int PP = (q.BM / Wt + 2) * (Wt + 2);
        if (q.family == IGEMM_PATCH) {
            const int P_SZ = (PP * 20 + 3) & ~3, B_SZ = (bmode == 0) ? q.BN * 20 : 16 * q.BN;
            q.lds_bytes = (2 * P_SZ + 2 * B_SZ) * (int)sizeof(float);
        } else {
            const int P_SZ = (PP * 40 + 7) & ~7;
            q.lds_bytes = (2 * P_SZ + 2 * q.BN * 40) * (int)sizeof(_Float16);
        }
    } else {
        const int nk = (p.Ktot + q.KB - 1) / q.KB;
        q.ksplit = p.no_split ? 1 : plan_ksplit((long long)q.gx * q.gy * ncls, nk, q.BM * q.BN, want_ks);
        q.kper = (nk + q.ksplit - 1) / q.ksplit;
        q.ksplit = (nk + q.kper - 1) / q.kper;
    }
    q.gz = q.ksplit * ncls;
    p.ksplit = q.ksplit;
    p.kper = q.kper;
    return q;
}

template <int BM, int BN, int TM, int TN, int BMODE, int GEN>
static void launch_tile(const ConvP& p, const IgemmPlan& q, hipStream_t st) {
    constexpr bool WIDE = BN >= 64;
    constexpr bool HAS_EPI = BMODE == 0 && (GEN & 2) == 0;
    void (*kernel)(const ConvP) = conv_igemm_kernel<BM, BN, TM, TN, BMODE, GEN, 16>;
    if constexpr (HAS_EPI) { if (p.epi) kernel = conv_igemm_kernel<BM, BN, TM, TN, BMODE, GEN, 16, 1>; }
    if constexpr (BM == 64 && BN == 64 && GEN == 0) {
        if (q.KB == 32) kernel = conv_igemm_kernel<BM, BN, TM, TN, BMODE, GEN, 32>;
        if constexpr (HAS_EPI) { if (q.KB == 32 && p.epi) kernel = conv_igemm_kernel<BM, BN, TM, TN, BMODE, GEN, 32, 1>; }
    }
    if constexpr (WIDE && GEN == 0) {
        if (q.family == IGEMM_PATCH) kernel = conv_igemm_patch_kernel<BM, BN, TM, TN, BMODE>;
        if constexpr (BMODE == 0) { if (q.family == IGEMM_PATCH && p.epi) kernel = conv_igemm_patch_kernel<BM, BN, TM, TN, BMODE, 1>; }
    }
    if constexpr (WIDE && BMODE == 0 && GEN == 0) {
        if (q.family == IGEMM_F16) kernel = p.f16 == 2 ? conv_igemm_f16_kernel<BM, BN, TM, TN, false> : conv_igemm_f16_kernel<BM, BN, TM, TN>;
        if (q.family == IGEMM_PATCH_F16) kernel = p.f16 == 2 ? conv_igemm_patch_f16_kernel<BM, BN, TM, TN, false> : conv_igemm_patch_f16_kernel<BM, BN, TM, TN>;
    }
    hipLaunchKernelGGL(kernel, dim3(q.gx, q.gy, q.gz), dim3(256), q.lds_bytes, st, p);
}

template <int BMODE, int GEN>
static int run_igemm(const ConvP& p, const IgemmPlan& q, size_t y_elems, hipStream_t st) {
    if (q.ksplit > 1 && p.post_slope != 1.f) {
        gim_set_error("conv fwd: post_slope with a launch that splits K (ask gim_conv_launch_plan first)");
        return GIM_E_BADARG;
    }
    if (p.res && (BMODE == 1) != (p.mask_x != nullptr)) {
        gim_set_error(BMODE == 0 ? "conv: residual and mask_x together on k-contiguous weights (the k-major dgrad has that epilogue)"
                                 : "conv dgrad (k-major): a residual needs mask_x");
        return GIM_E_BADARG;
    }
    if (q.ksplit > 1 && !p.y_zeroed) (void)hipMemsetAsync(p.y, 0, y_elems * sizeof(float), st);
    if (q.BM == 128 && q.BN == 128) launch_tile<128, 128, 2, 2, BMODE, GEN>(p, q, st);
    else if (q.BM == 64 && q.BN == 128) launch_tile<64, 128, 1, 2, BMODE, GEN>(p, q, st);
    else if (q.BM == 128 && q.BN == 64) launch_tile<128, 64, 2, 1, BMODE, GEN>(p, q, st);
    else if (q.BM == 64 && q.BN == 64) launch_tile<64, 64, 1, 1, BMODE, GEN>(p, q, st);
    else if (q.BN == 32) launch_tile<128, 32, 1, 1, BMODE, GEN>(p, q, st);
    else launch_tile<128, 16, 1, 1, BMODE, GEN>(p, q, st);
    return GIM_OK;
}

struct ConvCall { ConvP p; size_t y_elems; int bmode, gen; };

static int run_planned(const ConvCall& c, const IgemmPlan& q, void* stream, const char* what) {
    hipStream_t st = (hipStream_t)stream;
    int rc;
    if (c.bmode == 0) rc = c.gen ? run_igemm<0, 1>(c.p, q, c.y_elems, st) : run_igemm<0, 0>(c.p, q, c.y_elems, st);
    else if (c.gen == 0) rc = run_igemm<1, 0>(c.p, q, c.y_elems, st);
// ... 256 lines not shown
}

__global__ __launch_bounds__(256) void pack_rows_weights_kernel(const float* __restrict__ w, float* __restrict__ wp, int Cout, int Cin, int K, int CaP) {
    const int total = Cout * K * CaP;
    for (int i = blockIdx.x * 256 + threadIdx.x; i < total; i += gridDim.x * 256) {
        const int c = i % CaP, r = i / CaP;
        wp[i] = c < K * Cin ? w[r * K * Cin + c] : 0.f;
    }
}

extern "C" int gim_conv2d_pack_rows_weights(const float* w, float* wp, int Cout, int Cin, int KH, void* stream) {
    GIM_CHECK_ARG(w && wp && Cout > 0 && Cin > 0 && KH > 0 && (KH & 1) && KH * Cin <= 64, "pack_rows_weights: bad args");
    const int CaP = (KH * Cin + 15) & ~15, total = Cout * KH * CaP;
    hipLaunchKernelGGL(pack_rows_weights_kernel, dim3((total + 255) / 256 < 1024 ? (total + 255) / 256 : 1024), dim3(256), 0, (hipStream_t)stream,
                       w, wp, Cout, Cin, KH, CaP);
    return gim_check_launch("gim_conv2d_pack_rows_weights");
}

__global__ __launch_bounds__(256) void pad_image_kernel(const float* __restrict__ x, float* __restrict__ xp, int N, int H, int W, int C, int pad, float slope) {
    const int Hp = H + 2 * pad, Wp = W + 2 * pad;
    const long long total = (long long)N * Hp * Wp * C;
    for (long long i = (long long)blockIdx.x * 256 + threadIdx.x; i < total; i += (long long)gridDim.x * 256) {
        const int c = (int)(i % C);
        long long r = i / C;
        const int xx = (int)(r % Wp) - pad; r /= Wp;
        const int yy = (int)(r % Hp) - pad;
        const int n = (int)(r / Hp);
        float v = 0.f;
        if ((unsigned)yy < (unsigned)H && (unsigned)xx < (unsigned)W) v = x[(((long long)n * H + yy) * W + xx) * C + c];
        xp[i] = fmaxf(v, v * slope);
    }
}

extern "C" int gim_pad_image(const float* x, float* xp, int N, int H, int W, int C, int pad, float slope, void* stream) {
    GIM_CHECK_ARG(x && xp && N > 0 && H > 0 && W > 0 && C > 0 && pad >= 0 && slope > 0.f && slope <= 1.f, "pad_image: bad args");
    const long long total = (long long)N * (H + 2 * pad) * (W + 2 * pad) * C;
    hipLaunchKernelGGL(pad_image_kernel, dim3((unsigned)((total + 255) / 256 < 4096 ? (total + 255) / 256 : 4096)), dim3(256), 0, (hipStream_t)stream,
                       x, xp, N, H, W, C, pad, slope);
    return gim_check_launch("gim_pad_image");
}

__global__ __launch_bounds__(256) void pack_subpixel_weights_kernel(const float* __restrict__ f, float* __restrict__ wm, int Cout, int Cin, int K) {
    const int KF = K + 1, T = KF / 2;
    const int total = 4 * Cout * T * T * Cin;
    for (int i = blockIdx.x * 256 + threadIdx.x; i < total; i += gridDim.x * 256) {
        const int ci = i % Cin;
        int r = i / Cin;
        const int tb = r % T; r /= T;
        const int ta = r % T; r /= T;
        const int co = r % Cout, cls = r / Cout;
        const int py = cls >> 1, px = cls & 1;
        wm[i] = f[((co * KF + 1 - py + 2 * ta) * KF + 1 - px + 2 * tb) * Cin + ci];
    }
}

extern "C" int gim_conv2d_pack_subpixel_weights(const float* wf, float* wm, int Cout, int Cin, int KH, void* stream) {
    GIM_CHECK_ARG(wf && wm && Cout > 0 && Cin > 0 && KH >= 5 && (KH & 3) == 1, "pack_subpixel_weights: KH must be 5, 9, 13, ...");
    const int T = (KH + 1) / 2, total = 4 * Cout * T * T * Cin;
    hipLaunchKernelGGL(pack_subpixel_weights_kernel, dim3((total + 255) / 256 < 1024 ? (total + 255) / 256 : 1024), dim3(256), 0, (hipStream_t)stream,
                       wf, wm, Cout, Cin, KH);
    return gim_check_launch("gim_conv2d_pack_subpixel_weights");
}

static int rows_shape_ok(const gim_conv_shape* s) {
    int rc = check_shape(s);
    if (rc) return rc;
    GIM_CHECK_ARG(!s->ups && !s->pool && !s->wfold && !s->res_ups, "conv rows form: plain stride-1 convolutions only");
    GIM_CHECK_ARG(s->Cin <= 8 && s->KH * s->Cin <= 64 && s->Cout >= 16, "conv rows form: <= 8 input channels, K * Cin <= 64, >= 16 output channels");
    return GIM_OK;
}

static Geo geo_rows(const gim_conv_shape* s) {
    Geo g{};
    const int pad = (s->KH - 1) / 2;
    geo_grid(g, s->N, s->H, s->W);
    g.ups = 0; g.Hin = s->H + 2 * pad; g.Win = s->W + 2 * pad;
    g.s_in = g.s_in_x = 1; g.off_y = g.off_x = 0;
    g.Th = g.KF = s->KH; g.Tw = g.KFw = 1;
    g.wa_base = 0; g.wa_step = 1; g.wb_base = 0; g.wb_step = 0;
    g.os = 1;
    return g;
}

extern "C" int gim_conv2d_fwd_rows(const float* xp, const float* wp, const float* bias, const float* sigma, const float* residual,
                                   float* y, const gim_conv_shape* s, void* stream) {
    int rc = rows_shape_ok(s);
    if (rc) return rc;
    GIM_CHECK_ARG(xp && wp && y && !((uintptr_t)xp & 15) && !((uintptr_t)wp & 15), "conv fwd (rows form): null or unaligned pointer");
    ConvCall c;
    const int CaP = (s->KH * s->Cin + 15) & ~15;
    rc = convp_begin(c, geo_rows(s), CaP, s->Cout, s->Cin, 6, s, "conv fwd (rows form): the padded image batch exceeds 2 GiB (32-bit buffer offsets): split the batch");
    if (rc) return rc;
    ConvP& p = c.p;
    p.x = xp; p.w = wp; p.bias = bias; p.sigma = sigma; p.res = residual; p.y = y;
    p.Cin_w = CaP;
    rc = set_post_slope(p, s->post_slope);
    if (!rc) rc = set_y_elems(c, (size_t)s->N * s->H * s->W * s->Cout, "conv: the output exceeds 2 GiB (32-bit buffer offsets): split the batch");
    return rc ? rc : plan_and_run(c, stream, "gim_conv2d_fwd_rows");
}
template <int VA, int VB, bool FASTB>
static void launch_wgrad(const WgP& p, int bm, int bn, int bk, dim3 g, hipStream_t st) {
    if constexpr (VA == 4 && VB == 4) {
        if (bk == 32 && bm == 64 && bn == 64) {
            hipLaunchKernelGGL((conv_wgrad_kernel<64, 64, 1, 1, 4, 4, FASTB, 32>), g, dim3(256), 0, st, p);
            return;
        }
    }
    if (bm == 128 && bn == 128) hipLaunchKernelGGL((conv_wgrad_kernel<128, 128, 2, 2, VA, VB, FASTB>), g, dim3(256), 0, st, p);
    else if (bm == 128 && bn == 64) hipLaunchKernelGGL((conv_wgrad_kernel<128, 64, 2, 1, VA, VB, FASTB>), g, dim3(256), 0, st, p);
    else if (bm == 64 && bn == 128) hipLaunchKernelGGL((conv_wgrad_kernel<64, 128, 1, 2, VA, VB, FASTB>), g, dim3(256), 0, st, p);
    else if (bm == 64 && bn == 64) hipLaunchKernelGGL((conv_wgrad_kernel<64, 64, 1, 1, VA, VB, FASTB>), g, dim3(256), 0, st, p);
    else hipLaunchKernelGGL((conv_wgrad_kernel<32, 128, 1, 1, VA, VB, FASTB>), g, dim3(256), 0, st, p);
}

constexpr int NARROW_PARTS = 16, NARROW_MPER = 512, NARROW_U = 8, NARROW_ROWS = NARROW_MPER / NARROW_PARTS;
template <int CN, bool EXACT>
__global__ __launch_bounds__(64 * NARROW_PARTS) void wgrad_1x1_narrow_kernel(const float* __restrict__ wide, const float* __restrict__ nar,
                                                                             float* __restrict__ out, float* __restrict__ bias_out, int M, int Cw,
                                                                             int Cn_, float slope_x, int wide_is_dy) {
    __shared__ float red[NARROW_PARTS][9][64];
    const int Cn = EXACT ? CN : Cn_;
    const int lane = threadIdx.x & 63, part = __builtin_amdgcn_readfirstlane(threadIdx.x >> 6);
    const int c = blockIdx.y * 64 + lane, cc = min(c, Cw - 1);
    const int m0 = blockIdx.x * NARROW_MPER, m1 = min(M, m0 + NARROW_MPER);
    float acc[CN], bsum = 0.f;
#pragma unroll
    for (int j = 0; j < CN; ++j) acc[j] = 0.f;
    const int mw = m0 + part * NARROW_ROWS, me = min(m1, mw + NARROW_ROWS);
    for (int mb = mw; mb < me; mb += NARROW_U) {
        float wv[NARROW_U], nv[NARROW_U][CN];
        const float* nrow = nar + (long long)mb * Cn;
#pragma unroll
        for (int u = 0; u < NARROW_U; ++u) {
            wv[u] = wide[(long long)(mb + u) * Cw + cc];
#pragma unroll
            for (int j = 0; j < CN; ++j) nv[u][j] = nrow[u * Cn + (EXACT ? j : min(j, Cn - 1))];
        }
#pragma unroll
        for (int u = 0; u < NARROW_U; ++u) {
            float w_ = wv[u];
            bsum += w_;
            if (!wide_is_dy) w_ = fmaxf(w_, w_ * slope_x);
#pragma unroll
            for (int j = 0; j < CN; ++j) {
                float n_ = nv[u][j];
                if (wide_is_dy) n_ = fmaxf(n_, n_ * slope_x);
                acc[j] += w_ * n_;
            }
        }
    }
#pragma unroll
    for (int j = 0; j < 8; ++j) red[part][j][lane] = j < CN ? acc[j < CN ? j : 0] : 0.f;
    red[part][8][lane] = bsum;
    __syncthreads();
    if (wide_is_dy) {
        const int t = threadIdx.x, cl = t / Cn, j = t - cl * Cn, cg = blockIdx.y * 64 + cl;
        if (t < 64 * Cn && cg < Cw) {
            float v = 0.f;
#pragma unroll
            for (int q = 0; q < NARROW_PARTS; ++q) v += red[q][j][cl];
            atomicAdd(&out[(long long)cg * Cn + j], v);
        } else if (part == 8 && bias_out && c < Cw) {
            float v = 0.f;
#pragma unroll
            for (int q = 0; q < NARROW_PARTS; ++q) v += red[q][8][lane];
            atomicAdd(&bias_out[c], v);
        }
    } else if (part < Cn && c < Cw) {
        float v = 0.f;
#pragma unroll
        for (int q = 0; q < NARROW_PARTS; ++q) v += red[q][part][lane];
        atomicAdd(&out[(long long)part * Cw + c], v);
    }
    if (bias_out && !wide_is_dy && blockIdx.y == 0) {
        __syncthreads();
        float sb = 0.f;
        if (part < Cn)
            for (int m = m0 + lane; m < m1; m += 64) sb += nar[(long long)m * Cn + part];
        if (part < 8) red[0][part][lane] = sb;
        __syncthreads();
        if (threadIdx.x < Cn) {
            float v = 0.f;
// ... 190 lines not shown
        else hipLaunchKernelGGL(conv_wgrad_row_kernel<4>, g, dim3(256), 0, st, p);
        break;
    case WG_NARROW: {
        const int wide_is_dy = s->Cin <= 8 ? 1 : 0;
        const int Cw = wide_is_dy ? s->Cout : s->Cin, Cn = wide_is_dy ? s->Cin : s->Cout;
        const dim3 b(64 * NARROW_PARTS);
        const float *wd = wide_is_dy ? dy : x, *nr = wide_is_dy ? x : dy;
        if (Cn == 3) hipLaunchKernelGGL((wgrad_1x1_narrow_kernel<3, true>), g, b, 0, st, wd, nr, slabs, bias_slabs, q.M, Cw, Cn, s->pre_slope, wide_is_dy);
        else if (Cn == 6) hipLaunchKernelGGL((wgrad_1x1_narrow_kernel<6, true>), g, b, 0, st, wd, nr, slabs, bias_slabs, q.M, Cw, Cn, s->pre_slope, wide_is_dy);
        else hipLaunchKernelGGL((wgrad_1x1_narrow_kernel<8, false>), g, b, 0, st, wd, nr, slabs, bias_slabs, q.M, Cw, Cn, s->pre_slope, wide_is_dy);
        break;
    }
    default:
        launch_wgrad_mfma(p, q, s->prec, st);
    }
    return gim_check_launch("gim_conv2d_wgrad");
}

extern "C" int gim_conv2d_wgrad(const float* dy, const float* x, float* slabs, float* bias_slabs, int n_slabs,
                                const gim_conv_shape* s, void* stream) {
    return wgrad_impl(dy, x, slabs, bias_slabs, n_slabs, s, stream, false);
}

extern "C" int gim_conv2d_wgrad_acc(const float* dy, const float* x, float* acc, float* bias_acc, const gim_conv_shape* s, void* stream) {
    const int rc = check_shape(s);
    if (rc) return rc;
    size_t xi, yi;
    image_elems(s, false, xi, yi);
    return over_batch_halves(*s, xi, yi, [&](const gim_conv_shape& h, size_t n0, bool) {
        return wgrad_impl(dy + n0 * yi, x + n0 * xi, acc, bias_acc, 1, &h, stream, true);
    });
}

extern "C" int gim_conv2d_wgrad_rows_acc(const float* dy, const float* xp, float* acc, float* bias_acc, const gim_conv_shape* s, void* stream) {
    int rc = rows_shape_ok(s);
    if (rc) return rc;
    GIM_CHECK_ARG(s->Cout % 4 == 0 && dy && xp && !((uintptr_t)dy & 15) && !((uintptr_t)xp & 15), "conv wgrad (rows form): Cout % 4 == 0 and 16-byte aligned operands required");
    return wgrad_impl(dy, xp, acc, bias_acc, 1, s, stream, true, true);
}

static void plan_row(int32_t* out, int table_hit, int bm, int bn, int slices, int gx, int gy, int gz, int form) {
    const int32_t v[8] = {table_hit, bm, bn, slices, gx, gy, gz, form};
    for (int i = 0; i < 8; ++i) out[i] = v[i];
}

static int launch_plan(const gim_conv_shape* s, int kind, int32_t* out) {
    float* const fake = reinterpret_cast<float*>(uintptr_t(4096));
    int rc = check_shape(s);
    if (rc) return rc;
    if (kind < 2 && tiny_route(s)) {
        const dim3 g = gim_tiny_grid(s);
        plan_row(out, 0, GIM_TINY_TILE * GIM_TINY_TILE, kind == 0 ? s->Cout : s->Cin, 1, g.x, g.y, 1, 3);
        return GIM_OK;
    }
    size_t xi, yi;
    image_elems(s, kind == 1 || kind == 2, xi, yi);
    return over_batch_halves(*s, xi, yi, [&](const gim_conv_shape& h, size_t, bool) {
        if (kind == 3) {
            const int form[] = {0, 2, 3, 1, 0};
            WgP p;
            WgPlan q;
            const int rc = wgrad_call(p, q, fake, fake, fake, nullptr, 1, &h, true, false);
            if (!rc) plan_row(out, q.table_hit, q.bm, q.bn, q.slices, q.gx, q.gy, q.gz, form[q.family]);
            return rc;
        }
        const int form[] = {0, 1, 2, 2};
        ConvCall c;
        const int rc = kind == 0 ? fwd_call(c, fake, fake, nullptr, nullptr, nullptr, fake, &h)
                                 : dgrad_call(c, fake, fake, nullptr, nullptr, fake, &h, kind == 2, nullptr, 0.f);
        if (rc) return rc;
        const IgemmPlan q = plan_igemm(c.p, c.bmode, c.gen);
        const int skipped = 1000 - pm_valid_permille(c.p.g, c.p.M, q.BM);
        plan_row(out, q.table_hit, q.BM, q.BN, q.ksplit, q.gx, q.gy, q.gz, form[q.family] | (skipped << 8));
        return (int)GIM_OK;
    });
}

extern "C" int gim_conv_launch_plan(const gim_conv_shape* s, int kind, int32_t* out) {
    GIM_CHECK_ARG(s && out && kind >= 0 && kind <= 3, "conv_launch_plan: bad args");
    for (int i = 0; i < 8; ++i) out[i] = -1;
    return launch_plan(s, kind, out);
}


extern "C" int gim_conv2d_strided_fwd(const float* x, const float* w, const float* bias, float* y, const gim_infer_conv* s, void* stream) {
    const int rc = check_infer_conv(s, "conv2d_strided_fwd", true);
    if (rc) return rc;
    GIM_CHECK_ARG(x && w && y, "conv2d_strided_fwd: null pointer");
    return gim_conv2d_infer(x, w, bias, nullptr, y, s, stream);
}

struct StridedDgrad {
    ConvCall c[4];
    IgemmPlan q[4];
    int taps[4];
};

static int strided_dgrad_fill(StridedDgrad& d, const float* dy, const float* w, float* dx, const gim_infer_conv* s, int deterministic) {
    const int K = s->KH, pd = (K - 1) / 2, Ho = s->H / 2, Wo = s->W / 2;
    for (int cls = 0; cls < 4; ++cls) {
        const int par[2] = {cls >> 1, cls & 1};
        int th[2], off[2], base[2];
        for (int d2 = 0; d2 < 2; ++d2) {
            const int a0 = (par[d2] + pd) & 1;
            th[d2] = a0 <= K - 1 ? (K - 1 - a0) / 2 + 1 : 0;
            base[d2] = a0 + 2 * (th[d2] - 1);
            off[d2] = (par[d2] + pd - base[d2]) / 2;
        }
        d.taps[cls] = th[0] * th[1];
        if (!d.taps[cls]) continue;
        Geo g{};
        geo_grid(g, s->N, Ho, Wo);
        g.Hin = Ho; g.Win = Wo; g.ups = 0;
        g.s_in = g.s_in_x = 1; g.off_y = off[0]; g.off_x = off[1]; g.Th = th[0]; g.Tw = th[1]; g.KF = g.KFw = K;
        g.wa_base = base[0]; g.wb_base = base[1]; g.wa_step = g.wb_step = -2;
        g.os = 2; g.py = par[0]; g.px = par[1];
        ConvCall& c = d.c[cls];
        const int rc = convp_begin(c, g, s->Cout, s->Cin, s->Cout, 6, nullptr, "conv2d_strided_dgrad: one image exceeds 2 GiB (32-bit buffer offsets)");
        if (rc) return rc;
        ConvP& p = c.p;
        p.x = dy; p.w = w; p.y = dx;
        p.Cin_w = s->Cin;
        p.tune_ks = deterministic ? 1 : 0;
        c.y_elems = (size_t)s->N * s->H * s->W * s->Cin;
        c.bmode = 1; c.gen = gen_dgrad(s->Cout, s->Cin, dy, w);
        d.q[cls] = plan_igemm(p, c.bmode, c.gen);
    }
    return GIM_OK;
}

static gim_conv_shape plain_shape_of(const gim_infer_conv* s) {
    gim_conv_shape v{};
    v.N = s->N; v.H = s->H / s->stride; v.W = s->W / s->stride; v.Cin = s->Cin; v.Cout = s->Cout; v.KH = s->KH; v.pre_slope = 1.f;
    return v;
}

extern "C" int gim_conv2d_strided_dgrad(const float* dy, const float* w, float* dx, const gim_infer_conv* s, int deterministic, void* stream) {
    const int rc = check_infer_conv(s, "conv2d_strided_dgrad", true);
    if (rc) return rc;
    GIM_CHECK_ARG(dy && w && dx, "conv2d_strided_dgrad: null pointer");
    if (s->stride == 1) {
        gim_conv_shape v = plain_shape_of(s);
        v.tune_ksplit = deterministic ? 1 : 0;
        return gim_conv2d_dgrad(dy, w, nullptr, nullptr, dx, &v, stream);
    }
    size_t xi, yi;
    strided_image_elems(s, xi, yi);
    return over_batch_halves(*s, xi, yi, [&](const gim_infer_conv& h, size_t n0, bool) {
        float* const dxh = dx + n0 * xi;
        StridedDgrad d;
        int rc = strided_dgrad_fill(d, dy + n0 * yi, w, dxh, &h, deterministic);
        if (rc) return rc;
        bool clear = false;
        for (int cls = 0; cls < 4; ++cls) clear = clear || !d.taps[cls] || d.q[cls].ksplit > 1;
        if (clear) (void)hipMemsetAsync(dxh, 0, xi * h.N * sizeof(float), (hipStream_t)stream);
        for (int cls = 0; cls < 4 && !rc; ++cls) {
            if (!d.taps[cls]) continue;
            d.c[cls].p.y_zeroed = 1;
            rc = run_planned(d.c[cls], d.q[cls], stream, "gim_conv2d_strided_dgrad");
        }
        return rc;
    });
}

static WgPlan strided_wgrad_plan(const gim_infer_conv* s, int combine) {
    gim_conv_shape v = plain_shape_of(s);
// ... 80 lines not shown
```

### optimalstrategiesagainstgenerativeattacks_amd/gim_img_models.py

```python
import math
import os

import torch
import torch.nn as nn

from . import model_blocks as mb
from . import ops
from .gim_basic_models import GIMMeanStdFcStat


_TWO_STREAMS = os.environ.get("GIM_SINGLE_STREAM") is None
_PER_SAMPLE_STREAMS = os.environ.get("GIM_PER_SAMPLE_STREAMS") is not None
_LANE1_SIDE = os.environ.get("GIM_NO_LANE1_SIDE") is None
_STREAMS = {}


def _use_side_streams(t):
    if not (_TWO_STREAMS and t.is_cuda):
        return False
    if ops.current_lane() == 0:
        return True
    return _LANE1_SIDE and not torch.cuda.is_current_stream_capturing()


_STREAM_MAP = [int(v) for v in os.environ.get("GIM_STREAM_MAP", "0,1,2,2,0").split(",")]
assert len(_STREAM_MAP) == 5, "GIM_STREAM_MAP: five comma-separated stream ids (roles 0..4)"
_POOL = {}


def _role_stream(device, role):
    key = (device.type, device.index, _STREAM_MAP[role])
    if key not in _POOL:
        _POOL[key] = torch.cuda.Stream(device=device)
    return _POOL[key]


def _side_streams(device, n=2):
    assert n == 2 or _PER_SAMPLE_STREAMS
    lane = ops.current_lane()
    if n == 2:
        return [_role_stream(device, 3 * lane), _role_stream(device, 3 * lane + 1)]
    key = (device.type, device.index, "many", lane)
    have = _STREAMS.setdefault(key, [])
    while len(have) < n:
        have.append(torch.cuda.Stream(device=device))
    return have[:n]


def lane_stream(device, lane):
    assert lane == 1
    return _role_stream(device, 2)


def stream_concurrency_check(device, usec=300, warn=True):
    import warnings
    from . import _lib
    lib = _lib.load()
    cur = torch.cuda.current_stream(device)
    streams, seen = [cur], {cur.cuda_stream}
    for role in range(5):
        st = _role_stream(device, role)
        if st.cuda_stream not in seen:
            seen.add(st.cuda_stream)
            streams.append(st)

    def run(sts):
        e0, e1 = torch.cuda.Event(enable_timing=True), torch.cuda.Event(enable_timing=True)
        e0.record(cur)
        for st in sts[1:]:
            st.wait_stream(cur)
        for st in sts:
            _lib.check(lib.gim_spin(usec, st.cuda_stream), "spin")
        for st in sts[1:]:
            cur.wait_stream(st)
        e1.record(cur)
        e1.synchronize()
        return e0.elapsed_time(e1)
    run(streams)
    one = min(run(streams[:1]) for _ in range(3))
    alls = min(run(streams) for _ in range(3))
    ser = alls / max(one, 1e-6)
    res = {"streams": len(streams), "one_ms": round(one, 4), "all_ms": round(alls, 4), "serialization": round(ser, 2),
           "concurrent": ser < 1.5, "GPU_MAX_HW_QUEUES": os.environ.get("GPU_MAX_HW_QUEUES")}
    if warn and not res["concurrent"]:
        warnings.warn("GIM engine: its %d HIP streams do NOT run concurrently (spin test: %.2f ms together vs %.2f ms alone): at least two "
                      "share a hardware queue and the training step will be 6-12 %% slower.  Set GPU_MAX_HW_QUEUES=8 in the environment "
                      "BEFORE the process makes its first GPU call (importing this package first does it)." % (len(streams), alls, one),
                      RuntimeWarning, stacklevel=2)
    return res


class Encoder(nn.Module):

    def __init__(self, img_size, img_channels, style_dim=512, min_n_channels=64, use_out_lrelu=True):
        super().__init__()
        assert use_out_lrelu, "the hot path fuses the output LeakyReLU into the max-pool kernel"
# ... 145 lines not shown
            ops.stream_wait(side, cur)
            with torch.cuda.stream(side):
                if not self.group_style_linears or ops.deterministic():
                    svs_res = [b.style_vectors(style) for b in self.adain_res_block.res_blocks]
                    svs_up = [b.style_vectors(style) for b in self.adain_up_block.up_blocks]
                else:
                    blocks = list(self.adain_res_block.res_blocks) + list(self.adain_up_block.up_blocks)
                    lins = [l_ for b in blocks for l_ in (b.lin1_mean, b.lin1_std, b.lin2_mean, b.lin2_std)]
                    shp = style.shape
                    ys = ops.grouped_linear(style.reshape(-1, shp[-1]), [(l_.weight, l_.bias) for l_ in lins])
                    ys = [y.view(*shp[:-1], y.shape[-1]) for y in ys]
                    svs = [tuple(ys[4 * i:4 * i + 4]) for i in range(len(blocks))]
                    svs_res, svs_up = svs[:len(self.adain_res_block.res_blocks)], svs[len(self.adain_res_block.res_blocks):]
            style.record_stream(side)
        x = self.down_block(x)
        if svs_res is not None:
            ops.stream_wait(cur, side)
            for sv in svs_res + svs_up:
                for t in sv:
                    t.record_stream(cur)
        x = self.adain_res_block(x=x, style=style, svs=svs_res)
        return self.adain_up_block(x=x, style=style, svs=svs_up)


def _set_training(module, mode):
    if not isinstance(mode, bool):
        raise ValueError("training mode is expected to be boolean")
    for m in module.modules():
        m.__dict__["training"] = mode
    return module



class GIMFaceDis(nn.Module):

    def __init__(self, src_dim, env_dim, stat):
        super().__init__()
        self.src_dim, self.env_dim = src_dim, env_dim
        self.stat = stat
        self.n_stats = stat.n_stats
        mlp_input_dim = 2 * (self.n_stats * env_dim + src_dim)
        self.mlp = mb.MLP((mlp_input_dim, env_dim + src_dim, 2 * (env_dim + src_dim), 1))
        for m in self.mlp.model:
            if isinstance(m, mb.GimLinear):
                nn.init.kaiming_normal_(m.weight.data, a=0.2)
                nn.init.constant_(m.bias.data, 0.0)

    def forward(self, test_src, test_env, si_src, si_env):
        fc_test = self.stat.fc.per_sample(test_env)
        fc_si = self.stat.fc.per_sample(si_env)
        x = ops.head_cat(test_src, test_env, si_src, si_env, fc_test, fc_si)
        return self.mlp(x)


def _encode_sample(encoder, sample):
    B, t = sample.size(0), sample.size(1)
    x = ops.to_nhwc(sample.reshape(B * t, *sample.size()[2:]))
    return encoder(x).view(B, t, -1)


class GIMFaceAuthenticator(nn.Module):

    def __init__(self, src_encoder, env_encoder, dis):
        super().__init__()
        self.src_encoder = src_encoder
        self.env_encoder = env_encoder
        self.dis = dis
        self._sn_plan = None

    def train(self, mode=True):
        return _set_training(self, mode)

    def prefetch_spectral(self, rounds):
        if self._sn_plan is None:
            self._sn_plan = mb.SNPlan(mb.sn_convs(self.src_encoder, self.env_encoder))
        self._sn_plan.run(rounds, self.training)

    def forward(self, test_sample, si_sample):
        self.prefetch_spectral(2)
        (test_src, si_src), (test_env, si_env) = self.encode_samples([test_sample, si_sample])
        return self.dis(test_src=test_src, test_env=test_env, si_src=si_src, si_env=si_env)

    def encode_samples(self, samples):
        cur = torch.cuda.current_stream()
        if not _use_side_streams(samples[0]):
            return ([self.src_encode_sample(s) for s in samples], [self.env_encode_sample(s) for s in samples])
        per_sample = _PER_SAMPLE_STREAMS
        streams = _side_streams(samples[0].device, 2 * len(samples) if per_sample else 2)
        outs = []
        for e, enc in enumerate((self.src_encoder, self.env_encoder)):
            feats = []
            for i, smp in enumerate(samples):
                st = streams[e * len(samples) + i] if per_sample else streams[e]
                if per_sample or i == 0:
                    ops.stream_wait(st, cur)
                with torch.cuda.stream(st):
                    f = _encode_sample(enc, smp)
                f.record_stream(cur)
                smp.record_stream(st)
                feats.append(f)
            outs.append(feats)
        for st in streams:
            ops.stream_wait(cur, st)
        return outs[0], outs[1]

    def src_encode_sample(self, sample):
        return _encode_sample(self.src_encoder, sample)

    def env_encode_sample(self, sample):
        return _encode_sample(self.env_encoder, sample)


class GIMFaceImpersonator(nn.Module):

    def __init__(self, src_encoder, env_encoder, env_decoder, img2img, env_noise_mapper, use_img_att=False):
        super().__init__()
        self.src_encoder = src_encoder
        self.env_encoder = env_encoder
        self.env_decoder = env_decoder
        self.img2img = img2img
        self.env_noise_mapper = env_noise_mapper
        self.style_dim = src_encoder.style_dim
        assert src_encoder.style_dim == env_encoder.style_dim == env_decoder.style_dim == img2img.style_dim
        self.use_img_att = use_img_att
        self.img_att = mb.ImgAttention(img1_channels=self.src_encoder.img_channels, img2_channels=self.img2img.out_channels)
        self._sn_plan = None

    def train(self, mode=True):
        return _set_training(self, mode)

    def forward(self, leaked_sample, n, remove_noise_mean=True, z=None):
        if self._sn_plan is None:
            mods = [self.src_encoder, self.env_encoder, self.env_decoder, self.img2img] + ([self.img_att] if self.use_img_att else [])
            self._sn_plan = mb.SNPlan(mb.sn_convs(*mods))
        self._sn_plan.run(1, self.training)
        B, m, C, S, _ = leaked_sample.size()
        leaked = ops.to_nhwc(leaked_sample.reshape(B * m, C, S, S))
        side = None
        if _use_side_streams(leaked):
            cur = torch.cuda.current_stream()
            side = _side_streams(leaked.device)[1]
            ops.stream_wait(side, cur)
            with torch.cuda.stream(side):
                src = ops.mean_dim1(self.src_encoder(leaked).view(B, m, -1))
            leaked.record_stream(side)
        else:
            src = ops.mean_dim1(self.src_encoder(leaked).view(B, m, -1))
        env = ops.mean_dim1(self.env_encoder(leaked).view(B, m, -1))
        if z is None:
            z = torch.randn((B, n, self.style_dim), device=leaked_sample.device)
        w = self.env_noise_mapper(z)
        noisy_env = ops.noise_combine(env, w, remove_noise_mean)
        env_img = self.env_decoder(noisy_env.view(B * n, -1))
        if side is not None:
            ops.stream_wait(cur, side)
            src.record_stream(cur)
        first = leaked.view(B, m, S, S, C)[:, 0]
        x = ops.concat2(env_img, first, n)
        style = ops.repeat_dim1(src, n).view(B * n, self.style_dim)
        out = self.img2img(x=x, style=style)
        if self.use_img_att:
            x1 = ops.repeat_dim1(first.reshape(B, S * S * C), n).view(B * n, S, S, C)
            out = self.img_att(x1=x1, x2=out)
        return ops.to_nchw(out).view(B, n, C, S, S)

    def src_encode_sample(self, sample):
        return _encode_sample(self.src_encoder, sample)

    def env_encode_sample(self, sample):
        return _encode_sample(self.env_encoder, sample)


def get_im(img_size, img_channels, style_dim, use_img_att=False, num_env_noise_layers=4):
    src_encoder = Encoder(img_size=img_size, img_channels=img_channels, style_dim=style_dim)
    env_encoder = Encoder(img_size=img_size, img_channels=img_channels, style_dim=style_dim)
    decoder = EnvDecoder(img_size=img_size, img_channels=img_channels, style_dim=style_dim)
    img2img = AdaInImage2Image(img_size=img_size, in_channels=2 * img_channels, out_channels=img_channels, style_dim=style_dim)
    env_noise_mapper = mb.MLP([style_dim for _ in range(num_env_noise_layers + 1)])
    return GIMFaceImpersonator(src_encoder=src_encoder, env_encoder=env_encoder, env_decoder=decoder, img2img=img2img,
                               env_noise_mapper=env_noise_mapper, use_img_att=use_img_att)


def get_au(img_size, img_channels, style_dim):
    stat = GIMMeanStdFcStat(style_dim=style_dim, fc_n_stats=2, fc_hidden_layers=(style_dim * 2, style_dim * 3, style_dim * 2))
# ... 5 lines not shown
```

### optimalstrategiesagainstgenerativeattacks_amd/model_blocks.py

```python
import collections
import math

import torch
import torch.nn as nn

from . import _lib
from . import ops

LRELU = 0.2


def _kaiming_uniform_like_torch(weight, bias, fan_in):
    nn.init.kaiming_uniform_(weight, a=math.sqrt(5))
    if bias is not None:
        bound = 1.0 / math.sqrt(fan_in) if fan_in > 0 else 0.0
        nn.init.uniform_(bias, -bound, bound)


class GimLinear(nn.Module):

    def __init__(self, in_features, out_features):
        super().__init__()
        self.in_features, self.out_features = in_features, out_features
        self.weight = nn.Parameter(torch.empty(out_features, in_features))
# ... 32 lines not shown
            else:
                x = layer(x, pre_slope=slope)
                slope = 1.0
        return x


class SNReplay:

    def __init__(self):
        self.micro = 0

    def micro_batch(self, j):
        return _SNMicroBatch(self, j)


class _SNMicroBatch:
    def __init__(self, state, j):
        self.state, self.j = state, j

    def __enter__(self):
        self.prev = _SN_REPLAY[0]
        self.state.micro = self.j
        _SN_REPLAY[0] = self.state

    def __exit__(self, *exc):
        _SN_REPLAY[0] = self.prev


_SN_REPLAY = [None]


class _SNTape:

    def __init__(self):
        self.state, self.items, self.micro, self.pos = None, [], 0, 0

    def next(self, state, key, make):
        if self.state is not state:
            self.state, self.items, self.micro, self.pos = state, [], 0, 0
        if self.micro != state.micro:
            self.micro, self.pos = state.micro, 0
        if state.micro == 0:
            item = make()
            self.items.append((key, item))
            return item
        if self.pos >= len(self.items) or self.items[self.pos][0] != key:
            raise RuntimeError("accumulated step: micro-batch %d makes spectral-norm call %d %r of a site, which micro-batch 0 "
                               "did not make: the micro-batches of a step must run the same forward passes" % (state.micro, self.pos, key))
        item = self.items[self.pos][1]
        self.pos += 1
        return item


class SNConv2d(nn.Module):

    def __init__(self, in_channels, out_channels, kernel_size, padding=0):
        super().__init__()
        assert padding == (kernel_size - 1) // 2, "only 'same' stride-1 convolutions are on the GIM hot path"
        self.in_channels, self.out_channels, self.kernel_size = in_channels, out_channels, kernel_size
        w = torch.empty(out_channels, in_channels, kernel_size, kernel_size)
        b = torch.empty(out_channels)
        _kaiming_uniform_like_torch(w, b, in_channels * kernel_size * kernel_size)
        u = nn.functional.normalize(w.new_empty(out_channels).normal_(0, 1), dim=0, eps=1e-12)
        v = nn.functional.normalize(w.new_empty(in_channels * kernel_size * kernel_size).normal_(0, 1), dim=0, eps=1e-12)
        self.bias = nn.Parameter(b)
        self.weight_orig = nn.Parameter(w.contiguous(memory_format=torch.channels_last))
        self.register_buffer("weight_u", u)
        self.register_buffer("weight_v", v)

        self._sn_queue = collections.deque()
        self._sn_tape = _SNTape()
        self._wants_fold = False
        self._fold_slot = (kernel_size + 1, "fold")

    def fold_is_stale(self):
        return ops._WT_CACHE.is_stale(self.weight_orig, self._fold_slot)

    def folded(self):
        self._wants_fold = True
        return ops._WT_CACHE.get(self.weight_orig, self._fold_slot, lambda: ops._folded(
            ops.weight_phys(self.weight_orig), self.out_channels, self.in_channels, self.kernel_size))

    def forward(self, x, res=None, ups=0, pre_slope=1.0, pool=False, res_ups=False, post_slope=1.0, x_act=False, fork_pool_slope=None):
        guard = None
        if self._sn_queue:
            sigma, u_s, v_s, guard = self._sn_queue.popleft()
        elif _SN_REPLAY[0] is not None:
            sigma, u_s, v_s = self._sn_tape.next(_SN_REPLAY[0], None, lambda: ops.spectral_sigma(
                self.weight_orig, self.weight_u, self.weight_v, self.training))
        else:
            sigma, u_s, v_s = ops.spectral_sigma(self.weight_orig, self.weight_u, self.weight_v, self.training)
        if fork_pool_slope is not None:
            assert res is None and not ups and not pool and not res_ups
            return ops.conv2d_forkpool(x, self.weight_orig, self.bias, sigma, u_s, v_s, pre_slope, guard, post_slope, x_act, fork_pool_slope)
        wf = self.folded() if (pool or (ups and self.kernel_size > 1)) else None
        if post_slope != 1.0:
            return ops.conv2d_post_act(x, self.weight_orig, self.bias, res, sigma, u_s, v_s, ups, pre_slope, pool, res_ups, wf, guard, post_slope, x_act)
        return ops.conv2d(x, self.weight_orig, self.bias, res, sigma, u_s, v_s, ups, pre_slope, pool, res_ups, wf, guard, x_act)

    def extra_repr(self):
        return "%d, %d, kernel_size=%d (spectral norm)" % (self.in_channels, self.out_channels, self.kernel_size)


class SNPlan:

    def __init__(self, convs):
        self.convs = [c for c in convs if isinstance(c, SNConv2d)]
        self._gen = 0
        self._bufs = {}
        self._tape = _SNTape()
        self._tables = ops._TableCache("SNPlan", 1)
        self._fold_tables = ops._TableCache("SNPlan folds", None, skip_in_capture=True)

    def stale(self, gen):
        return self._gen - gen > 2

    def _build(self):
        jobs = (_lib.GimSnJob * len(self.convs))()
        cols, rows, views = [], [], []
        off = 0

        def take(n):
            nonlocal off
            o = off
            off += (n + 3) // 4 * 4
            return o
        for j, c in enumerate(self.convs):
            Cout, Cin, KH = c.out_channels, c.in_channels, c.kernel_size
            K = Cin * KH * KH
            if not c.weight_orig.permute(0, 2, 3, 1).is_contiguous():
                raise RuntimeError("SNPlan: weight_orig must be stored channels-last")
            o_s, o_u, o_v, o_scr = take(1), take(Cout), take(K), take(10 * K + Cout)
            jobs[j] = (c.weight_orig.data_ptr(), c.weight_u.data_ptr(), c.weight_v.data_ptr(), o_s, o_u, o_v, o_scr, Cout, Cin, KH, 0)
            R = min(8, (Cout + 63) // 64)
            rows_per = (Cout + R - 1) // R
            for xb in range((K + 255) // 256):
                for r in range(R):
                    cols.append((j, xb, r, rows_per))
            for rb in range((Cout + 3) // 4):
                rows.append((j, rb))
            views.append((o_s, o_u, Cout, o_v, K))
        return ops._DeviceTable(jobs, cols, rows, extra=(len(jobs), len(cols), len(rows), off, views))

    def run(self, rounds, training):
        if not self.convs:
            return
        state = _SN_REPLAY[0]
        if state is None:
            return self._launch(rounds, training)

        def record():
            self._launch(rounds, training)
            return [tuple(c._sn_queue) for c in self.convs]
        queued = self._tape.next(state, rounds, record)
        if state.micro > 0:
            if self.stale(queued[0][0][3][1]):
                raise RuntimeError("accumulated step: the spectral-norm buffers of micro-batch 0 were overwritten by forward passes "
                                   "outside the step")
            for c, q in zip(self.convs, queued):
                c._sn_queue.clear()
                c._sn_queue.extend(q)

    @torch.no_grad()
    def _launch(self, rounds, training):
        w0 = self.convs[0].weight_orig
        if not (w0.is_cuda and w0.dtype == torch.float32):
            raise RuntimeError("weights must be CUDA float32 (got %s on %s): the GIM engine has no CPU path" % (w0.dtype, w0.device))
        tab = self._tables.get(tuple(t.data_ptr() for c in self.convs for t in (c.weight_orig, c.weight_u, c.weight_v)), self._build)
        (d_jobs, d_cols, d_rows), (n_jobs, n_cols, n_rows, total, views) = tab.ptrs, tab.extra
        raw = ops._stream()
        tab.use_on_current_stream(raw)
        for c in self.convs:
            c._sn_queue.clear()
        gen = self._gen
        self._gen += 1
        for r in range(rounds):
            out = self._bufs.get((gen & 1, r))
            if out is None or out.numel() != total or out.device != w0.device:
                out = self._bufs[(gen & 1, r)] = torch.empty(total, device=w0.device, dtype=torch.float32)
            _lib.check(_lib.load().gim_spectral_sigma_batched(d_jobs, n_jobs, d_cols, n_cols, d_rows, n_rows, out.data_ptr(), 1 if training else 0, raw),
                       "spectral_sigma_batched")
# ... 190 lines not shown
```

### optimalstrategiesagainstgenerativeattacks_amd/ops.py

```python
import collections
import ctypes
import math
import os
import struct
import warnings
import weakref

import torch
from torch.autograd import Function
from torch.autograd.function import once_differentiable

from . import _lib, optim
from ._lib import GimConvShape, GimGemmJob, GimWgradJob, check

LRELU_SLOPE = 0.2

_HIGHER = {"input_grad_only": False}


class input_grad_only:
    def __enter__(self):
        self.prev = _HIGHER["input_grad_only"]
        _HIGHER["input_grad_only"] = True

# ... 184 lines not shown

class armed_backward:

    def __init__(self, scaler):
        self.on = 1 if scaler is not None else 0

    def __enter__(self):
        _ARMED[0] += self.on

    def __exit__(self, *exc):
        _ARMED[0] -= self.on


def set_matrix_path(name):
    if name not in ("fp32", "fp16"):
        raise ValueError("matrix path must be 'fp32' or 'fp16'")
    prev = matrix_path()
    _PREC[0] = 1 if name == "fp16" else 0
    if prev != name:
        _SPLITS_K.clear()
    return prev


_SHAPES = {}


def _shape(N, H, W, Cin, Cout, KH, ups, pre_slope, pool=0, wfold=0, res_ups=0):
    prec = 2 if (_PREC[0] and _ARMED[0]) else _PREC[0]
    key = (N, H, W, Cin, Cout, KH, ups, pre_slope, pool, wfold, res_ups, _DETERMINISTIC[0], prec)
    t = _SHAPES.get(key)
    if t is None:
        t = _SHAPES[key] = GimConvShape(N, H, W, Cin, Cout, KH, ups, pre_slope, pool, wfold, res_ups, 0, 1 if _DETERMINISTIC[0] else 0, 0, 0, 0.0,
                                        prec if H * W > 1 else 0)
    return GimConvShape.from_buffer_copy(t)


_TUNE_OVERRIDE = {}


def _tuned(sh, kind, key):
    ov = _TUNE_OVERRIDE.get((kind, key)) if _TUNE_OVERRIDE else None
    if ov is not None:
        sh.tune_tile = ov[0]
        if kind == "wgrad":
            sh.tune_wgrad = ov[1]
        else:
            sh.tune_ksplit = ov[1]
    return sh


_ZERO_POOL = os.environ.get("GIM_NO_ZERO_POOL") is None
_SPLITS_K = {}
_ZERO_PAGES = {}
_ZERO_PAGE = 16 << 20
_Plan = collections.namedtuple("_Plan", "ksplit skipped_permille")


def _launch_plan(sh, plan_kind, key):
    k_ = (plan_kind,) + key
    v = _SPLITS_K.get(k_)
    if v is None:
        out = (ctypes.c_int32 * 8)()
        check(_lib.load().gim_conv_launch_plan(ctypes.byref(sh), plan_kind, ctypes.cast(out, ctypes.c_void_p)), "conv_launch_plan")
        v = _SPLITS_K[k_] = _Plan(out[3], out[7] >> 8)
    return v


def _zeros_from_pool(shape, device):
    n = 1
    for d in shape:
        n *= d
    na = (n + 63) & ~63
    if na > _ZERO_PAGE >> 1:
        return torch.zeros(shape, device=device, dtype=torch.float32)
    raw = (torch._C._cuda_getDevice(), _stream())
    pg = _ZERO_PAGES.get(raw)
    if pg is None or pg[1] + na > pg[0].numel():
        pg = _ZERO_PAGES[raw] = [torch.zeros(_ZERO_PAGE, device=device, dtype=torch.float32), 0]
    v = pg[0][pg[1]:pg[1] + n].view(shape)
    pg[1] += na
    return v


def _conv_out(sh, plan_kind, key, shape, device):
    if _ZERO_POOL and _launch_plan(sh, plan_kind, key).ksplit > 1 and not torch.cuda.is_current_stream_capturing():
        sh.out_zeroed = 1
        return _zeros_from_pool(shape, device)
    return torch.empty(shape, device=device, dtype=torch.float32)


@torch.no_grad()
def spectral_sigma(w, u, v, training):
    lib = _lib.load()
    wp = weight_phys(w)
    Cout, Cin = w.shape[0], w.shape[1]
    KH = w.shape[2] if w.dim() == 4 else 1
    K = Cin * KH * KH
    sigma = torch.empty(1, device=w.device, dtype=torch.float32)
    u_s = torch.empty_like(u)
    v_s = torch.empty_like(v)
    scratch = torch.empty(9 * K + Cout, device=w.device, dtype=torch.float32)
    check(lib.gim_spectral_sigma(_p(wp), _p(u), _p(v), _p(sigma), _p(u_s), _p(v_s), _p(scratch), Cout, Cin, KH,
                                 1 if training else 0, _stream()), "spectral_sigma")
    return sigma, u_s, v_s


def _folded(wp, Cout, Cin, KH):
    f = torch.empty(Cout * (KH + 1) * (KH + 1) * Cin, device=wp.device, dtype=torch.float32)
    check(_lib.load().gim_conv2d_fold_weights(_p(wp), _p(f), Cout, Cin, KH, _stream()), "fold_weights")
    return f


class _StreamReady:
    __slots__ = ("tensor", "event", "streams", "in_capture")

    def __init__(self, tensor):
        self.tensor = tensor
        self.rewritten()

    def rewritten(self):
        self.event = torch.cuda.current_stream().record_event()
        self.streams = {_stream()}
        self.in_capture = torch.cuda.is_current_stream_capturing()

    def use_on_current_stream(self, raw=None):
        if raw is None:
            raw = _stream()
        if raw not in self.streams:
            cur = torch.cuda.current_stream()
            if self.in_capture or not torch.cuda.is_current_stream_capturing():
                cur.wait_event(self.event)
            self.tensor.record_stream(cur)
            self.streams.add(raw)
        return self.tensor


def layout_tables(jobs, *tables):
    blob, offsets = bytearray(), []
    for sec in [bytes(jobs)] + [struct.pack("<%di" % (len(t) * len(t[0])), *(v for row in t for v in row)) if t else bytes(8)
                                for t in tables]:
        blob += bytes(-len(blob) % 16)
        offsets.append(len(blob))
        blob += sec
    return bytes(blob), offsets


class _DeviceTable(_StreamReady):
    __slots__ = ("host", "ptrs", "extra")

    def __init__(self, jobs, *tables, extra=None):
        blob, offsets = layout_tables(jobs, *tables)
        self.host = torch.frombuffer(bytearray(blob), dtype=torch.uint8).pin_memory()
        super().__init__(self.host.to(torch.device("cuda", torch._C._cuda_getDevice()), non_blocking=True))
        self.ptrs, self.extra = [self.tensor.data_ptr() + o for o in offsets], extra


class _TableCache(collections.OrderedDict):

    def __init__(self, what, capacity=None, skip_in_capture=False):
        super().__init__()
        self.what, self.capacity, self.skip_in_capture = what, capacity, skip_in_capture

    def get(self, sig, build):
        if sig in self:
            self.move_to_end(sig)
        elif not (torch.cuda.is_initialized() and torch.cuda.is_current_stream_capturing()):
            self[sig] = build()
            if self.capacity is not None and len(self) > self.capacity:
# ... 168 lines not shown
        return cls.make(N, Hs << ups, Ws << ups, Cin, w.shape[0], w.shape[2] if w.dim() == 4 else 1, ups, pre_slope, pool, res_ups,
                        bias is not None, res is not None, x_act, x.dim() == 2)

    out_pixels = property(lambda s: s.N * (s.H >> s.pool) * (s.W >> s.pool))
    out_shape = property(lambda s: (s.N, s.Cout) if s.linear else (s.N, s.H >> s.pool, s.W >> s.pool, s.Cout))
    K = property(lambda s: s.KH * s.KH * s.Cin)
    KFF = property(lambda s: (s.KH + 1) * (s.KH + 1) * s.Cin if s.fold else s.K)

    def shape(self, kind, pre_slope=None):
        return _tuned(_shape(self.N, self.H, self.W, self.Cin, self.Cout, self.KH, self.ups, self.pre_slope if pre_slope is None else pre_slope,
                             self.key[7], self.fold, 1 if self.res_ups else 0), kind, self.key)

    def box(self):
        return self._replace(fold=0, pre_slope=1.0, key=self.key[:7] + (2, 0))

    def linear_map(self):
        return ConvGeom.make(self.N, self.H, self.W, self.Cin, self.Cout, self.KH, 0, 1.0, self.pool, linear=self.linear)


_ACT_STORAGE = os.environ.get("GIM_NO_ACT_STORAGE") is None
_ROWS_FORM = os.environ.get("GIM_NO_ROWS_FORM") is None
_MERGED_SUBPIXEL = os.environ.get("GIM_NO_MERGED_SUBPIXEL") is None
_NARROW_DGRAD_T = os.environ.get("GIM_NO_NARROW_DGRAD_T") is None
_NARROW_XFOLD = os.environ.get("GIM_NO_NARROW_XFOLD") is None
_BOX_POOL = os.environ.get("GIM_NO_BOX_POOL") is None


def _fwd_route(g, tune_tile):
    if g.linear or tune_tile != 0:
        return "plain"
    if _ROWS_FORM and g.KH >= 3 and g.Cin <= 8 and g.KH * g.Cin <= 64 and g.Cout >= 16 and g.Cout % 4 == 0 and not (g.ups or g.pool or g.res_ups):
        return "rows"
    if _MERGED_SUBPIXEL and g.ups and g.KH >= 5 and (g.KH & 3) == 1 and g.Cout <= 4 and not g.has_res:
        return "subpixel"
    return "plain"


def _pool_route(g, prec, tune_tile=0):
    if not (_BOX_POOL and g.pool) or g.linear or g.ups or g.KH != 3 or g.Cin % 16 != 0 or prec != 0 or tune_tile != 0:
        return "fold"
    return "box"


def _fwd_launch(g, tap_slope=None):
    sh = g.shape("fwd", tap_slope)
    if g.pool and _pool_route(g, sh.prec, sh.tune_tile or (1 if ("wgrad", g.key) in _TUNE_OVERRIDE else 0)) == "box":
        g = g.box()
        sh = g.shape("fwd")
    return g, sh


def _xfold_factor(Cin, W):
    J = 4 if Cin <= 6 else 2
    return J if (Cin <= 8 and W % J == 0 and W // J >= 1) else 0


def _dgrad_route(g, prec, has_w, has_res_half=False):
    f16_t = prec >= 1 and g.Cout % 32 == 0 and g.Cin >= 32
    J = 0
    if has_w and g.Cout % 16 == 0 and not (g.ups and not g.fold) and ((g.Cin <= 8 and _NARROW_DGRAD_T) or f16_t):
        if g.KH >= 3 and not (g.ups or g.pool or g.fold) and _NARROW_XFOLD and not f16_t:
            J = _xfold_factor(g.Cin, g.W)
        route = "xfold" if J else "t"
    else:
        route = "ups" if (g.ups and not g.fold) else "plain"
    if not has_res_half:
        return route, J, False
    if route == "plain" and not (g.pool or g.fold) and g.pre_slope != 1.0 and not f16_t:
        return "res", 0, False
    return route, J, True


def _wgrad_route(g, sh, has_target, has_sigma, bias_untargeted=False, rows_copy=False):
    if has_target and wgrad_queue.enabled and not _DETERMINISTIC[0] and not bias_untargeted:
        return ("queued_rows" if rows_copy else "queued"), 1
    ns = 1
    if _WGRAD_SLABS or _DETERMINISTIC[0]:
        ns = _lib.load().gim_conv2d_wgrad_slabs(sh)
        if ns <= 0:
            check(ns, "conv2d_wgrad_slabs")
    return ("direct" if (ns == 1 and not has_sigma and not g.fold and not has_target) else "slabs"), ns


def _stores_activated(g, post_slope):
    if not (_ACT_STORAGE and post_slope != 1.0) or g.linear:
        return False
    gl, sh = _fwd_launch(g)
    return _fwd_route(g, sh.tune_tile) == "subpixel" or _launch_plan(sh, 0, gl.key).ksplit == 1


def _merged_subpixel(x, w, ups, res, sh):
    return _fwd_route(ConvGeom.of(x, w, ups, 1.0, False, False, None, res, False), sh.tune_tile) == "subpixel"


class ConvFn(Function):
    N_EXTRA = 11

    @staticmethod
    def forward(ctx, x, w, bias, res, sigma, u_s, v_s, ups, pre_slope, pool, res_ups, wf=None, guard=None, post_slope=1.0, x_act=False):
        lib = _lib.load()
        x = _req(x, "x")
        wp = weight_phys(_req_w(w))
        g = ConvGeom.of(x, w, ups, pre_slope, pool, res_ups, bias, res, x_act)
        N, H, W, Cin, Cout, KH = g.N, g.H, g.W, g.Cin, g.Cout, g.KH
        tap_slope = 1.0 if x_act else pre_slope
        gl, sh = _fwd_launch(g, tap_slope)
        route = _fwd_route(g, sh.tune_tile)
        if post_slope != 1.0 and route != "subpixel":
            if g.linear or _launch_plan(sh, 0, gl.key).ksplit > 1:
                raise RuntimeError("conv: an activated output (post_slope) cannot be combined with a split-K launch or a linear layer")
            sh.post_slope = post_slope
        if res is not None:
            res = _req(res, "res")
        xp = None
        if route == "rows":
            pad = (KH - 1) // 2
            xp = torch.empty((N, H + 2 * pad, W + 2 * pad, Cin), device=x.device, dtype=torch.float32)
            check(lib.gim_pad_image(_p(x), _p(xp), N, H, W, Cin, pad, tap_slope, _stream()), "pad_image")
            wrows = _transposed(lib, w, wp, Cout, Cin, KH, rows=True)
            sh.tune_ksplit = 1
            y = torch.empty(g.out_shape, device=x.device, dtype=torch.float32)
            check(lib.gim_conv2d_fwd_rows(_p(xp), _p(wrows), _p(bias), _p(sigma), _p(res), _p(y), sh, _stream()), "conv2d_fwd_rows")
        elif route == "subpixel":
            if wf is None:
                wf = _folded(wp, Cout, Cin, KH)
            wm = _transposed(lib, w, wf, Cout, Cin, KH, subpix=True)
            gm = ConvGeom.make(N, H >> 1, W >> 1, Cin, 4 * Cout, (KH + 1) // 2)
            shm = gm.shape("fwd", tap_slope)
            y4 = _conv_out(shm, 0, gm.key, gm.out_shape, x.device)
            check(lib.gim_conv2d_fwd(_p(x), _p(wm), None, _p(sigma), None, _p(y4), shm, _stream()), "conv2d_fwd")
            y = torch.empty(g.out_shape, device=x.device, dtype=torch.float32)
            check(lib.gim_depth_to_space2(_p(y4), _p(bias), _p(y), N, H >> 1, W >> 1, Cout, post_slope, _stream()), "depth_to_space2")
        elif gl is not g:
            xp = torch.empty((N, H + 1, W + 1, Cin), device=x.device, dtype=torch.float32)
            check(lib.gim_box2_fwd(_p(x), _p(xp), N, H, W, Cin, tap_slope, _stream()), "box2_fwd")
            y = _conv_out(sh, 0, gl.key, g.out_shape, x.device)
            check(lib.gim_conv2d_fwd(_p(xp), _p(wp), _p(bias), _p(sigma), _p(res), _p(y), sh, _stream()), "conv2d_fwd")
        else:
            y = _conv_out(sh, 0, g.key, g.out_shape, x.device)
            if g.fold and wf is None:
                wf = _folded(wp, Cout, Cin, KH)
            check(lib.gim_conv2d_fwd(_p(x), _p(wf if g.fold else wp), _p(bias), _p(sigma), _p(res), _p(y), sh, _stream()), "conv2d_fwd")
        ctx.save_for_backward(x, w, sigma, u_s, v_s, wf if g.fold else None, bias, xp)
        ctx.cfg = g
        ctx.guard = guard
        if _FLOPS is not None:
            _note_conv("fwd", gl, sh, 0)
        return y

    @staticmethod
    def backward(ctx, dy):
        lib = _lib.load()
        x, w, sigma, u_s, v_s, wf, bias, xp = ctx.saved_tensors
        g = ctx.cfg
        dy = _req(dy, "dy")
        if ctx.guard is not None and ctx.guard[0].stale(ctx.guard[1]):
            raise RuntimeError("the spectral-norm state (sigma, u, v) of this forward pass was overwritten by later forward "
                               "passes of the same model: run backward before the third forward")
        need = ctx.needs_input_grad
        box = g.pool and xp is not None
        if g.fold and wf is None and need[0]:
            with torch.no_grad():
                wf = _folded(weight_phys(w), g.Cout, g.Cin, g.KH)
        if _second_order():
            if g.ups or g.res_ups:
                raise NotImplementedError("second-order backward of an upsampling convolution is not on the R1 path")
            dx = ConvDgradFn.apply(dy, w, x, sigma, u_s, v_s, wf, g) if need[0] else None
            return (dx, None, None, dy if g.has_res and need[3] else None) + (None,) * ConvFn.N_EXTRA
        wp = weight_phys(w)
        st = _stream()
        dev = dy.device
        dx = dw = db = dres = None
        if need[0]:
            dx = _conv_dgrad(lib, dy, x, wp, wf, sigma, g.shape("dgrad"), g, st, w, getattr(ctx, "dgrad_res", None))
        want_b = g.has_bias and need[2]
        if need[1] and box:
            gb = g.box()
            dw, db = _conv_wgrad(lib, dy, xp, w, wp, bias, sigma, u_s, v_s, gb.shape("wgrad"), gb, want_b, st)
        elif need[1]:
            dw, db = _conv_wgrad(lib, dy, x, w, wp, bias, sigma, u_s, v_s, g.shape("wgrad", 1.0 if g.x_act else None), g, want_b, st, xp)
        elif want_b:
            db = torch.empty(g.Cout, device=dev, dtype=torch.float32)
            scratch = torch.empty(256 * g.Cout, device=dev, dtype=torch.float32)
            check(lib.gim_colsum(_p(dy), _p(db), _p(scratch), g.out_pixels, g.Cout, st), "colsum")
        if g.has_res and need[3]:
            if g.res_ups:
                dres = torch.empty((g.N, g.H >> 1, g.W >> 1, g.Cout), device=dev, dtype=torch.float32)
                check(lib.gim_upsample2x_bwd(_p(dy), None, 1.0, _p(dres), g.N, g.H >> 1, g.W >> 1, g.Cout, st), "upsample2x_bwd")
            else:
                dres = dy
        return (dx, dw, db, dres) + (None,) * ConvFn.N_EXTRA


class _DerivedWeights(_StreamReady):
    __slots__ = ("version", "param")


class _DerivedWeightCache(dict):

    def _fresh(self, w, slot):
        ent = dict.get(self, (w.data_ptr(),) + slot)
        return ent if ent is not None and ent.version == (w._version, optim.weights_epoch(w)) and ent.param() is w else None

    def is_stale(self, w, slot):
        return self._fresh(w, slot) is None

    def install(self, w, slot, tensor):
        key = (w.data_ptr(),) + slot
        ent = self[key] = _DerivedWeights(tensor)
        ent.version, ent.param = (w._version, optim.weights_epoch(w)), weakref.ref(w, lambda _r: self.pop(key, None))
        return ent

    def get(self, w, slot, make, raw=None):
        ent = self._fresh(w, slot)
        if ent is None:
            with torch.no_grad():
                ent = self.install(w, slot, make())
        return ent.use_on_current_stream(raw)


_WT_CACHE = _DerivedWeightCache()


def _transposed(lib, w, wk, Cout, Cin, KF, xfold=0, rows=False, subpix=False):
    raw = _stream()

    def run(fn, n, what, *tail):
        wt = torch.empty(n, device=wk.device, dtype=torch.float32)
        check(fn(_p(wk), _p(wt), Cout, Cin, KF, *tail, raw), what)
        return wt
    if rows:
        layout, make = "rows", lambda: run(lib.gim_conv2d_pack_rows_weights, Cout * KF * ((KF * Cin + 15) & ~15), "pack_rows_weights")
    elif subpix:
        layout, make = "subpix", lambda: run(lib.gim_conv2d_pack_subpixel_weights, 4 * Cout * ((KF + 1) // 2) ** 2 * Cin, "pack_subpixel_weights")
    elif xfold:
        layout, make = xfold, lambda: run(lib.gim_conv2d_xfold_weights, xfold * Cin * KF * (KF + xfold - 1) * Cout, "xfold_weights", xfold)
    else:
        layout, make = 0, lambda: run(lib.gim_conv2d_transpose_weights, Cin * KF * KF * Cout, "transpose_weights")
    return _WT_CACHE.get(w, (KF, layout), make, raw)


def _conv_dgrad(lib, dy, x, wp, wf, sigma, sh, g, st, w=None, res_half=None):
    route, J, add_res = _dgrad_route(g, sh.prec, w is not None, res_half is not None)
    if _FLOPS is not None:
        _note_conv("dgrad", g, sh, 1)
    N, H, W, Cin, Cout, KH = g.N, g.H, g.W, g.Cin, g.Cout, g.KH
    mask = x if g.pre_slope != 1.0 else None
    wk = wf if g.fold else wp
    if route == "xfold":
        wx = _transposed(lib, w, wk, Cout, Cin, KH, xfold=J)
        dx = torch.empty(tuple(x.shape), device=x.device, dtype=torch.float32)
        check(lib.gim_conv2d_dgrad_xfold(_p(dy), _p(wx), _p(sigma), _p(mask), _p(dx), sh, J, st), "conv2d_dgrad_xfold")
    elif route == "t":
        wt = _transposed(lib, w, wk, Cout, Cin, KH + 1 if g.fold else KH)
        dx = _conv_out(sh, 2, g.key, tuple(x.shape), x.device)
        check(lib.gim_conv2d_dgrad_t(_p(dy), _p(wt), _p(sigma), _p(mask), _p(dx), sh, st), "conv2d_dgrad_t")
    elif route == "ups":
        dxu = _conv_out(sh, 1, g.key, (N, H, W, Cin), dy.device)
        dx = torch.empty_like(x)
        check(lib.gim_conv2d_dgrad(_p(dy), _p(wk), _p(sigma), None, _p(dxu), sh, st), "conv2d_dgrad")
        check(lib.gim_upsample2x_bwd(_p(dxu), _p(mask), g.pre_slope, _p(dx), N, H >> 1, W >> 1, Cin, st), "upsample2x_bwd")
    else:
        dx = _conv_out(sh, 1, g.key, tuple(x.shape), x.device)
        if route == "res":
            check(lib.gim_conv2d_dgrad_res(_p(dy), _p(wk), _p(sigma), _p(mask), _p(_req(res_half, "res_half")), 0.25, _p(dx), sh, st), "conv2d_dgrad_res")
        else:
            check(lib.gim_conv2d_dgrad(_p(dy), _p(wk), _p(sigma), _p(mask), _p(dx), sh, st), "conv2d_dgrad")
    if add_res:
        out = torch.empty_like(dx)
        check(lib.gim_add_avgpool2_bwd(_p(dx), _p(_req(res_half, "res_half")), _p(out), N, H, W, Cin, st), "add_avgpool2_bwd")
        return out
    return dx


def _conv_wgrad(lib, dy, x, w, wp, bias, sigma, u_s, v_s, sh, g, want_b, st, xp=None):
    if _FLOPS is not None:
        _note_conv("wgrad", g)
    Cin, Cout, KH, ups, fold = g.Cin, g.Cout, g.KH, g.ups, g.fold
    dev = dy.device
    dw = db = None
    Mo, K, KFF = g.out_pixels, g.K, g.KFF
    slab_bias = want_b and not (fold and ups)
    acc_w = _grad_target(w) if (sigma is not None or not fold) and not torch.is_grad_enabled() else None
    acc_b = _grad_target(bias) if (slab_bias and acc_w is not None) else None
    route, ns = _wgrad_route(g, sh, acc_w is not None, sigma is not None, want_b and slab_bias and acc_b is None,
                             xp is not None and dy.is_contiguous())
    fold_code = (2 if ups else 1) if fold else 0
    queued = route in ("queued", "queued_rows")
    if queued:
        q = _queue()
        n = Cout * K
        if Cout * KFF >= 1 << 31:
            raise RuntimeError("weight gradient of more than 2^31 elements (gim_wgrad_finish_batched indexes with 32 bits)")
        n_chunks = (n + q.CHUNK - 1) // q.CHUNK
        rows = route == "queued_rows"
        src = q.take(Cout * KH * ((KH * Cin + 15) & ~15) if rows else Cout * KFF, dev)
        bsrc = q.take(Cout, dev) if slab_bias else None
        sn = sigma is not None
        tmp = q.take(n, dev) if ((fold or rows) and sn) else None
        part = q.take(n_chunks, dev) if sn else None
        if rows:
            check(lib.gim_conv2d_wgrad_rows_acc(_p(dy), _p(xp), src, bsrc, sh, st), "conv2d_wgrad_rows_acc")
        else:
            check(lib.gim_conv2d_wgrad_acc(_p(dy), _p(x), src, bsrc, sh, st), "conv2d_wgrad_acc")
        q.add((src, bsrc or 0, _p(wp) if sn else 0, _p(sigma) or 0, _p(u_s) or 0, _p(v_s) or 0, tmp or 0, part or 0,
               _p(acc_w), _p(acc_b) or 0, Cout, Cin, KH, 3 if rows else fold_code, n_chunks), (sigma, u_s, v_s))
    else:
        dwp = torch.empty(Cout * K, device=dev, dtype=torch.float32)
        if want_b and acc_b is None:
            db = torch.empty(Cout, device=dev, dtype=torch.float32)
        if route == "direct":
            check(lib.gim_conv2d_wgrad(_p(dy), _p(x), _p(dwp), _p(db) if slab_bias else None, 1, sh, st), "conv2d_wgrad")
        else:
            slabs = torch.empty(ns * Cout * KFF, device=dev, dtype=torch.float32)
            bslabs = torch.empty(ns * Cout, device=dev, dtype=torch.float32) if slab_bias else None
            scratch = torch.empty(512 + (Cout * KFF if fold else 0), device=dev, dtype=torch.float32)
            check(lib.gim_conv2d_wgrad(_p(dy), _p(x), _p(slabs), _p(bslabs), ns, sh, st), "conv2d_wgrad")
            check(lib.gim_wgrad_finish(_p(slabs), _p(bslabs), ns, _p(wp), _p(sigma), _p(u_s), _p(v_s), _p(dwp),
                                       _p(db) if (slab_bias and acc_b is None) else None, _p(scratch), Cout, Cin, KH,
                                       fold_code, _p(acc_w), _p(acc_b), st), "wgrad_finish")
        if acc_w is None:
            dw = dwp.view(Cout, KH, KH, Cin).permute(0, 3, 1, 2) if w.dim() == 4 else dwp.view(Cout, Cin)
    if want_b and not slab_bias:
        scr = torch.empty(256 * Cout, device=dev, dtype=torch.float32)
        tgt_b = _grad_target(bias) if queued else None
        if tgt_b is not None:
            check(lib.gim_colsum_acc(_p(dy), _p(tgt_b), _p(scr), Mo, Cout, st), "colsum_acc")
        else:
            if db is None:
                db = torch.empty(Cout, device=dev, dtype=torch.float32)
            check(lib.gim_colsum(_p(dy), _p(db), _p(scr), Mo, Cout, st), "colsum")
    return dw, db


class ConvDgradFn(Function):
    N_EXTRA = 6

    @staticmethod
    def forward(ctx, dy, w, x, sigma, u_s, v_s, wf, geom):
        dx = _conv_dgrad(_lib.load(), dy, x, weight_phys(w), wf, sigma, geom.shape(None), geom, _stream(), w)
        ctx.save_for_backward(dy, w, x, sigma, u_s, v_s, wf)
        ctx.cfg = geom
        return dx

    @staticmethod
    def backward(ctx, g):
        lib = _lib.load()
        dy, w, x, sigma, u_s, v_s, wf = ctx.saved_tensors
        geom = ctx.cfg
        if torch.is_grad_enabled():
            raise NotImplementedError("third-order gradients are not supported")
        g = _req(g, "g")
        st = _stream()
        wp = weight_phys(w)
        if geom.pre_slope != 1.0:
            gm = torch.empty_like(g)
            check(lib.gim_lrelu_mask_mul(_p(g), _p(x), geom.pre_slope, _p(gm), g.numel(), st), "lrelu_mask_mul")
        else:
            gm = g
        lin = geom.linear_map()
        sh = lin.shape(None)
        g_dy = g_w = None
        if ctx.needs_input_grad[0]:
            g_dy = torch.empty_like(dy)
            check(lib.gim_conv2d_fwd(_p(gm), _p(wf if lin.fold else wp), None, _p(sigma), None, _p(g_dy), sh, st), "conv2d_fwd")
            if _FLOPS is not None:
                _note_conv("fwd", lin, sh, 0)
        if ctx.needs_input_grad[1]:
            g_w, _ = _conv_wgrad(lib, dy, gm, w, wp, None, sigma, u_s, v_s, sh, lin, False, st)
        return (g_dy, g_w) + (None,) * ConvDgradFn.N_EXTRA


def _grad_target(p):
    if p is None:
        return None
    g = p.grad
    if g is None:
        return None
    try:
        c = g._gim_tgt
        if c[0] == g.data_ptr():
            return c[1]
    except AttributeError:
        pass
    if not g.is_cuda or g.dtype != torch.float32 or g.shape != p.shape:
        return None
    gp = g.permute(0, 2, 3, 1) if g.dim() == 4 else g
    if not gp.is_contiguous():
        return None
    g._gim_tgt = (g.data_ptr(), gp)
    return gp


def _req_w(w):
    if not (w.is_cuda and w.dtype == torch.float32):
        raise RuntimeError("weights must be CUDA float32 (got %s on %s): the GIM engine has no CPU path" % (w.dtype, w.device))
    return w


def conv2d(x, w, bias=None, res=None, sigma=None, u_s=None, v_s=None, ups=0, pre_slope=1.0, pool=False, res_ups=False, wf=None,
           guard=None, x_act=False):
    return ConvFn.apply(x, w, bias, res, sigma, u_s, v_s, ups, pre_slope, pool, res_ups, wf, guard, 1.0, x_act)


def conv2d_post_act(x, w, bias=None, res=None, sigma=None, u_s=None, v_s=None, ups=0, pre_slope=1.0, pool=False, res_ups=False, wf=None,
                    guard=None, post_slope=1.0, x_act=False):
    act = post_slope != 1.0 and _stores_activated(ConvGeom.of(x, w, ups, pre_slope, pool, res_ups, bias, res, x_act), post_slope)
    y = ConvFn.apply(x, w, bias, res, sigma, u_s, v_s, ups, pre_slope, pool, res_ups, wf, guard, post_slope if act else 1.0, x_act)
    return y, act


class ConvForkPoolFn(Function):

    @staticmethod
    def forward(ctx, x, w, bias, res, sigma, u_s, v_s, ups, pre_slope, pool, res_ups, wf, guard, post_slope, x_act, in_slope):
        x, pooled = _avgpool2(x, in_slope)
        y = ConvFn.forward(ctx, x, w, bias, None, sigma, u_s, v_s, 0, pre_slope, False, False, None, guard, post_slope, x_act)
        return y, pooled

    @staticmethod
    def backward(ctx, dy, dpooled):
        x_shape = (ctx.cfg.N, ctx.cfg.H, ctx.cfg.W, ctx.cfg.Cin)
        if dy is None:
            return (AvgPool2BwdFn.apply(dpooled, x_shape) if dpooled is not None else None,) + (None,) * (3 + ConvFn.N_EXTRA + 1)
        if dpooled is not None and (torch.is_grad_enabled() or not ctx.needs_input_grad[0]):
            grads = ConvFn.backward(ctx, dy)
            gp = AvgPool2BwdFn.apply(dpooled, x_shape) if ctx.needs_input_grad[0] else None
            dx = gp if grads[0] is None else (grads[0] if gp is None else grads[0] + gp)
            return (dx,) + grads[1:] + (None,)
        ctx.dgrad_res = dpooled
        try:
            grads = ConvFn.backward(ctx, dy)
        finally:
            ctx.dgrad_res = None
        return grads + (None,)


_FUSED_FORKPOOL = os.environ.get("GIM_NO_FUSED_FORKPOOL") is None


def conv2d_forkpool(x, w, bias, sigma, u_s, v_s, pre_slope, guard, post_slope, x_act, in_slope):
    act = post_slope != 1.0 and _stores_activated(ConvGeom.of(x, w, 0, pre_slope, False, False, bias, None, x_act), post_slope)
    ps = post_slope if act else 1.0
    if _FUSED_FORKPOOL and x.requires_grad and torch.is_grad_enabled():
        y, pooled = ConvForkPoolFn.apply(x, w, bias, None, sigma, u_s, v_s, 0, pre_slope, False, False, None, guard, ps, x_act, in_slope)
    else:
        xa, pooled = fork_pool(x, in_slope)
        y = ConvFn.apply(xa, w, bias, None, sigma, u_s, v_s, 0, pre_slope, False, False, None, guard, ps, x_act)
    return y, act, pooled


def linear(x, w, bias=None, pre_slope=1.0):
    shp = x.shape
    y = ConvFn.apply(x.reshape(-1, shp[-1]), w, bias, None, None, None, None, 0, pre_slope, False, False, None, None)
    return y.view(*shp[:-1], w.shape[0])


_GEMM_TABLES = _TableCache("grouped linears", 64)


def _gemm_tables(jobs, col_tiles_only=False, raw=None):
    def build():
        arr = (GimGemmJob * len(jobs))(*jobs)
        tiles = [(j, it, jt) for j, jb in enumerate(jobs) for it in range(1 if col_tiles_only else (jb[4] + 63) // 64)
                 for jt in range((jb[5] + 63) // 64)]
        return _DeviceTable(arr, tiles, extra=len(tiles))
    ent = _GEMM_TABLES.get((tuple(jobs), col_tiles_only), build)
    ent.use_on_current_stream(raw)
    return ent.ptrs[0], ent.ptrs[1], ent.extra


class GroupedLinearFn(Function):

    @staticmethod
    def forward(ctx, x, *wb):
        lib = _lib.load()
        x = _req(x, "x")
        M, K = x.shape
        ws, bs = wb[0::2], wb[1::2]
        for w in ws:
            if not (w.is_cuda and w.dtype == torch.float32 and w.dim() == 2 and w.shape[1] == K and w.is_contiguous()):
                raise RuntimeError("grouped linear: weights must be contiguous CUDA float32 [out, %d]" % K)
        sizes = [w.shape[0] for w in ws]
        buf = torch.empty(M * sum(sizes), device=x.device, dtype=torch.float32)
        ys, off = [], 0
        for n_ in sizes:
            ys.append(buf[off:off + M * n_].view(M, n_))
            off += M * n_
        jobs = [(_p(x), _p(w), _p(y), _p(b) or 0, M, n_, K, n_, K, 1, 1, K, 0) for w, b, y, n_ in zip(ws, bs, ys, sizes)]
        st = _stream()
        check(lib.gim_bgemm_grouped(*_gemm_tables(jobs, raw=st), st), "bgemm_grouped")
        for n_ in sizes:
            _note_bgemm(1, M, n_, K)
        ctx.save_for_backward(x, *wb)
        return tuple(ys)

    @staticmethod
    @once_differentiable
    def backward(ctx, *dys):
        lib = _lib.load()
        x, *wb = ctx.saved_tensors
        ws, bs = wb[0::2], wb[1::2]
        M, K = x.shape
        st = _stream()
        need_x = ctx.needs_input_grad[0]
        dx = torch.zeros((M, K), device=x.device, dtype=torch.float32) if need_x else None
        jobs, cjobs, grads = [], [], []
        for g, (w, b, dy) in enumerate(zip(ws, bs, dys)):
            gw = gb = None
            if dy is not None:
                dy = _req(dy, "dy")
                n_ = w.shape[0]
                if need_x:
                    jobs.append((_p(dy), _p(w), _p(dx), 0, M, K, n_, K, n_, 1, K, 1, 2))
                if ctx.needs_input_grad[1 + 2 * g]:
                    tgt = _grad_target(w)
                    if tgt is None:
                        gw = torch.empty_like(w)
                    jobs.append((_p(dy), _p(x), _p(tgt if tgt is not None else gw), 0, n_, K, M, K, 1, n_, K, 1, 1 if tgt is not None else 0))
                if b is not None and ctx.needs_input_grad[2 + 2 * g]:
                    tgt = _grad_target(b)
                    if tgt is None:
                        gb = torch.empty_like(b)
                    cjobs.append((_p(dy), 0, _p(tgt if tgt is not None else gb), 0, M, n_, 0, 0, n_, 1, 0, 0, 1 if tgt is not None else 0))
                _note_bgemm(1, M, n_, K, 2)
            grads += [gw, gb]
        if jobs:
            check(lib.gim_bgemm_grouped(*_gemm_tables(jobs, raw=st), st), "bgemm_grouped")
        if cjobs:
            check(lib.gim_colsum_grouped(*_gemm_tables(cjobs, True, st), st), "colsum_grouped")
        return (dx, *grads)
# ... 1580 lines not shown
```

Baseline: 459.0.

## Merge per-sample-set convolutions into one segmented launch with per-segment sigma

Measured after the change: 454.1. -1.1%, worse.

```diff
diff --git a/include/gim_hip.h b/include/gim_hip.h
--- a/include/gim_hip.h
+++ b/include/gim_hip.h
@@ -81,6 +81,17 @@
 int gim_depth_to_space2(const float* y4, const float* bias, float* y, int N, int Hs, int Ws, int C, float post_slope, void* stream);
 
 int gim_conv_launch_plan(const gim_conv_shape* shape, int kind, int32_t* out);
+
+int gim_conv2d_fwd_seg(const float* x, const float* w, const float* bias, const float* sigma0, const float* sigma1, const float* sigma2,
+                       int n0, int n1, int n2, const float* residual, float* y, const gim_conv_shape* s, void* stream);
+int gim_conv2d_fwd_rows_seg(const float* xp, const float* wp, const float* bias, const float* sigma0, const float* sigma1,
+                            const float* sigma2, int n0, int n1, int n2, const float* residual, float* y, const gim_conv_shape* s,
+                            void* stream);
+int gim_conv2d_dgrad_seg(const float* dy, const float* w, const float* sigma0, const float* sigma1, const float* sigma2, int n0, int n1,
+                         int n2, const float* mask_x, const float* res_half, float res_scale, float* dx, const gim_conv_shape* s,
+                         int transposed, void* stream);
+int gim_conv_seg_merges(int BM, int rows_per_image, int pm, int n0, int n1, int n2);
+int gim_conv_launch_plan_seg(const gim_conv_shape* shape, int kind, int n0, int n1, int n2, int32_t* out);
 
 int gim_conv2d_wgrad_acc(const float* dy, const float* x, float* acc, float* bias_acc, const gim_conv_shape* shape, void* stream);
 
diff --git a/optimalstrategiesagainstgenerativeattacks_amd/_lib.py b/optimalstrategiesagainstgenerativeattacks_amd/_lib.py
--- a/optimalstrategiesagainstgenerativeattacks_amd/_lib.py
+++ b/optimalstrategiesagainstgenerativeattacks_amd/_lib.py
@@ -94,6 +94,11 @@
     "gim_colsum_acc": [P, P, P, c_int64, c_int, P],
     "gim_colsum2": [P, P, P, P, c_int, c_int, c_int, P],
     "gim_conv_launch_plan": [SP, c_int, P],
+    "gim_conv2d_fwd_seg": [P, P, P, P, P, P, c_int, c_int, c_int, P, P, SP, P],
+    "gim_conv2d_fwd_rows_seg": [P, P, P, P, P, P, c_int, c_int, c_int, P, P, SP, P],
+    "gim_conv2d_dgrad_seg": [P, P, P, P, P, c_int, c_int, c_int, P, P, c_float, P, SP, c_int, P],
+    "gim_conv_seg_merges": [c_int, c_int, c_int, c_int, c_int, c_int],
+    "gim_conv_launch_plan_seg": [SP, c_int, c_int, c_int, c_int, P],
     "gim_conv2d_transpose_weights": [P, P, c_int, c_int, c_int, P],
     "gim_conv2d_dgrad_t": [P, P, P, P, P, SP, P],
     "gim_conv2d_xfold_weights": [P, P, c_int, c_int, c_int, c_int, P],
diff --git a/optimalstrategiesagainstgenerativeattacks_amd/csrc/conv_f16.inc b/optimalstrategiesagainstgenerativeattacks_amd/csrc/conv_f16.inc
--- a/optimalstrategiesagainstgenerativeattacks_amd/csrc/conv_f16.inc
+++ b/optimalstrategiesagainstgenerativeattacks_amd/csrc/conv_f16.inc
@@ -176,7 +176,7 @@
     EpiCtx ec;
     const bool first = kslice == 0;
     bool has_res, has_mask;
-    epi_fill<false, false>(ec, p, g, first, has_res, has_mask);
+    epi_fill<false, false>(ec, p, g, m0, first, has_res, has_mask);
     auto run = [&](auto MODEC) {
         constexpr int MODE = decltype(MODEC)::value;
 #pragma unroll
@@ -354,7 +354,7 @@
     EpiCtx ec;
     const bool first = kslice == 0;
     bool has_res, has_mask;
-    epi_fill<true, false>(ec, p, g, first, has_res, has_mask);
+    epi_fill<true, false>(ec, p, g, m0, first, has_res, has_mask);
     auto run = [&](auto MODEC) {
         constexpr int MODE = decltype(MODEC)::value;
 #pragma unroll
diff --git a/optimalstrategiesagainstgenerativeattacks_amd/csrc/conv_igemm.hip b/optimalstrategiesagainstgenerativeattacks_amd/csrc/conv_igemm.hip
--- a/optimalstrategiesagainstgenerativeattacks_amd/csrc/conv_igemm.hip
+++ b/optimalstrategiesagainstgenerativeattacks_amd/csrc/conv_igemm.hip
@@ -96,6 +96,10 @@
     const float* slope;
     int epi;
     int no_split;
+    int seg_end0, seg_end1;
+    const float* sigma1;
+    const float* sigma2;
+    int no_pm;
 };
 
 __device__ __attribute__((aligned(16))) float g_zero4[4] = {0.f, 0.f, 0.f, 0.f};
@@ -218,8 +222,13 @@
 }
 
 template <bool PLAIN, bool PM>
-__device__ __forceinline__ void epi_fill(EpiCtx& ec, const ConvP& p, const Geo& g, bool first, bool& has_res, bool& has_mask) {
-    ec.scale = p.out_scale * (p.sigma ? 1.0f / p.sigma[0] : 1.0f);
+__device__ __forceinline__ void epi_fill(EpiCtx& ec, const ConvP& p, const Geo& g, int m0, bool first, bool& has_res, bool& has_mask) {
+    const float* sg = p.sigma;
+    if (p.seg_end0 > 0) {
+        const int n = m0 >> (g.logH + g.logW);
+        sg = n < p.seg_end0 ? p.sigma : (n < p.seg_end1 ? p.sigma1 : p.sigma2);
+    }
+    ec.scale = p.out_scale * (sg ? 1.0f / sg[0] : 1.0f);
     ec.mask_slope = p.mask_slope;
     ec.post_slope = p.post_slope;
     ec.res_scale = p.res_scale;
@@ -646,7 +655,7 @@
     EpiCtx ec;
     const bool first = kslice == 0;
     bool has_res, has_mask;
-    epi_fill<false, true>(ec, p, g, first, has_res, has_mask);
+    epi_fill<false, true>(ec, p, g, m0, first, has_res, has_mask);
     auto run = [&](auto MODEC) {
         constexpr int MODE = decltype(MODEC)::value;
         if constexpr (N16) {
@@ -863,7 +872,7 @@
     EpiCtx ec;
     const bool first = kslice == 0;
     bool has_res, has_mask;
-    epi_fill<true, false>(ec, p, g, first, has_res, has_mask);
+    epi_fill<true, false>(ec, p, g, m0, first, has_res, has_mask);
     auto run = [&](auto MODEC) {
         constexpr int MODE = decltype(MODEC)::value;
 #pragma unroll
@@ -1581,6 +1590,11 @@
         return (M > 64 && t128 >= GIM_SMALL_TILES) ? 641 : 64;
     }
     return (rows128 && t128 >= GIM_SMALL_TILES) ? 1264 : 64;
+}
+
+static bool pm_shape(const ConvP& p, int KB) {
+    const int taps = p.g.Th * p.g.Tw;
+    return taps > 1 && taps <= 32 && p.g.H * p.g.W <= PM_MAX_PIXELS && p.pix == p.Ca && p.Ca % KB == 0;
 }
 
 static IgemmPlan plan_igemm(ConvP& p, int bmode, int gen) {
@@ -1631,8 +1645,7 @@
         if (t.code == cfg) { q.BM = t.BM; q.BN = t.BN; }
 #ifndef GIM_NO_PM
     if (q.family == IGEMM_TAP && gen == 0) {
-        const int taps = g.Th * g.Tw;
-        p.g.pm = (taps > 1 && taps <= 32 && HW <= PM_MAX_PIXELS && g.N >= PM_MIN_IMAGES && p.pix == p.Ca && p.Ca % q.KB == 0) ? 1 : 0;
+        p.g.pm = (!p.no_pm && g.N >= PM_MIN_IMAGES && pm_shape(p, q.KB)) ? 1 : 0;
         if (p.g.pm) pm_make_perms(p.g);
     }
 #endif
@@ -2055,12 +2068,11 @@
     return g;
 }
 
-extern "C" int gim_conv2d_fwd_rows(const float* xp, const float* wp, const float* bias, const float* sigma, const float* residual,
-                                   float* y, const gim_conv_shape* s, void* stream) {
+static int rows_call(ConvCall& c, const float* xp, const float* wp, const float* bias, const float* sigma, const float* residual, float* y,
+                     const gim_conv_shape* s) {
     int rc = rows_shape_ok(s);
     if (rc) return rc;
     GIM_CHECK_ARG(xp && wp && y && !((uintptr_t)xp & 15) && !((uintptr_t)wp & 15), "conv fwd (rows form): null or unaligned pointer");
-    ConvCall c;
     const int CaP = (s->KH * s->Cin + 15) & ~15;
     rc = convp_begin(c, geo_rows(s), CaP, s->Cout, s->Cin, 6, s, "conv fwd (rows form): the padded image batch exceeds 2 GiB (32-bit buffer offsets): split the batch");
     if (rc) return rc;
@@ -2069,8 +2081,160 @@
     p.Cin_w = CaP;
     rc = set_post_slope(p, s->post_slope);
     if (!rc) rc = set_y_elems(c, (size_t)s->N * s->H * s->W * s->Cout, "conv: the output exceeds 2 GiB (32-bit buffer offsets): split the batch");
+    return rc;
+}
+
+extern "C" int gim_conv2d_fwd_rows(const float* xp, const float* wp, const float* bias, const float* sigma, const float* residual,
+                                   float* y, const gim_conv_shape* s, void* stream) {
+    ConvCall c;
+    const int rc = rows_call(c, xp, wp, bias, sigma, residual, y, s);
     return rc ? rc : plan_and_run(c, stream, "gim_conv2d_fwd_rows");
 }
+
+struct Segs { int n; int images[3]; const float* sigma[3]; };
+
+static int segs_fill(Segs& sg, const gim_conv_shape* s, const float* s0, const float* s1, const float* s2, int n0, int n1, int n2) {
+    GIM_CHECK_ARG(n0 > 0 && n1 > 0 && n2 >= 0 && (long long)n0 + n1 + n2 == s->N, "conv (segmented): two or three segments of > 0 images that add up to N");
+    sg = Segs{n2 ? 3 : 2, {n0, n1, n2}, {s0, s1, s2}};
+    return GIM_OK;
+}
+
+extern "C" int gim_conv_seg_merges(int BM, int rows_per_image, int pm, int n0, int n1, int n2) {
+    if (BM <= 0 || rows_per_image <= 0 || pm || n0 <= 0 || n1 <= 0 || n2 < 0) return 0;
+    const long long b0 = (long long)n0 * rows_per_image, b1 = b0 + (long long)n1 * rows_per_image;
+    return (b0 % BM == 0 && (n2 == 0 || b1 % BM == 0)) ? 1 : 0;
+}
+
+static bool seg_plan_merged(ConvCall& c, IgemmPlan& q, const Segs& sg) {
+    ConvP& p = c.p;
+    p.no_pm = 1;
+    q = plan_igemm(p, c.bmode, c.gen);
+    if (q.family == IGEMM_F16 || q.family == IGEMM_PATCH_F16) return false;
+    if (q.family == IGEMM_TAP && c.gen == 0 && pm_shape(p, q.KB))
+        for (int i = 0; i < sg.n; ++i)
+            if (sg.images[i] >= PM_MIN_IMAGES) return false;
+    if (!gim_conv_seg_merges(q.BM, p.g.H * p.g.W, p.g.pm, sg.images[0], sg.images[1], sg.images[2])) return false;
+    p.seg_end0 = sg.images[0];
+    p.seg_end1 = sg.images[0] + sg.images[1];
+    p.sigma1 = sg.sigma[1];
+    p.sigma2 = sg.n == 3 ? sg.sigma[2] : sg.sigma[1];
+    return true;
+}
+
+static bool fits_one_launch(const gim_conv_shape* s, size_t xi, size_t yi) { return (xi > yi ? xi : yi) * s->N * sizeof(float) <= BUF_MAX_BYTES; }
+
+#define SEG_PLAN_FALLBACK 1000
+static void plan_row(int32_t* out, int table_hit, int bm, int bn, int slices, int gx, int gy, int gz, int form);
+static int seg_plan_row(const IgemmPlan& q, int32_t* plan) {
+    plan_row(plan, q.table_hit, q.BM, q.BN, q.ksplit, q.gx, q.gy, q.gz, q.family == IGEMM_PATCH ? 1 : 0);
+    return GIM_OK;
+}
+
+static int fwd_seg_impl(const float* x, const float* w, const float* bias, const Segs& sg, const float* residual, float* y,
+                        const gim_conv_shape* s, void* stream, int32_t* plan) {
+    GIM_CHECK_ARG(x && w && y, "conv fwd (segmented): null pointer");
+    size_t xi, yi;
+    image_elems(s, false, xi, yi);
+    const size_t ri = s->res_ups ? yi / 4 : yi;
+    if (!tiny_route(s) && fits_one_launch(s, xi, yi)) {
+        ConvCall c;
+        IgemmPlan q;
+        const int rc = fwd_call(c, x, w, bias, sg.sigma[0], residual, y, s);
+        if (rc) return rc;
+        if (seg_plan_merged(c, q, sg)) return plan ? seg_plan_row(q, plan) : run_planned(c, q, stream, "gim_conv2d_fwd_seg");
+    }
+    if (plan) return SEG_PLAN_FALLBACK;
+    size_t n = 0;
+    for (int i = 0; i < sg.n; n += sg.images[i++]) {
+        gim_conv_shape h = *s;
+        h.N = sg.images[i];
+        const int rc = gim_conv2d_fwd(x + n * xi, w, bias, sg.sigma[i], residual ? residual + n * ri : nullptr, y + n * yi, &h, stream);
+        if (rc) return rc;
+    }
+    return GIM_OK;
+}
+
+extern "C" int gim_conv2d_fwd_seg(const float* x, const float* w, const float* bias, const float* sigma0, const float* sigma1,
+                                  const float* sigma2, int n0, int n1, int n2, const float* residual, float* y, const gim_conv_shape* s,
+                                  void* stream) {
+    int rc = check_shape(s);
+    if (rc) return rc;
+    Segs sg;
+    rc = segs_fill(sg, s, sigma0, sigma1, sigma2, n0, n1, n2);
+    return rc ? rc : fwd_seg_impl(x, w, bias, sg, residual, y, s, stream, nullptr);
+}
+
+static int rows_seg_impl(const float* xp, const float* wp, const float* bias, const Segs& sg, const float* residual, float* y,
+                         const gim_conv_shape* s, void* stream, int32_t* plan) {
+    {
+        ConvCall c;
+        IgemmPlan q;
+        const int rc = rows_call(c, xp, wp, bias, sg.sigma[0], residual, y, s);
+        if (rc) return rc;
+        if (seg_plan_merged(c, q, sg)) return plan ? seg_plan_row(q, plan) : run_planned(c, q, stream, "gim_conv2d_fwd_rows_seg");
+    }
+    if (plan) return SEG_PLAN_FALLBACK;
+    const int pad = (s->KH - 1) / 2;
+    const size_t xi = (size_t)(s->H + 2 * pad) * (s->W + 2 * pad) * s->Cin, yi = (size_t)s->H * s->W * s->Cout;
+    size_t n = 0;
+    for (int i = 0; i < sg.n; n += sg.images[i++]) {
+        gim_conv_shape h = *s;
+        h.N = sg.images[i];
+        const int rc = gim_conv2d_fwd_rows(xp + n * xi, wp, bias, sg.sigma[i], residual ? residual + n * yi : nullptr, y + n * yi, &h, stream);
+        if (rc) return rc;
+    }
+    return GIM_OK;
+}
+
+extern "C" int gim_conv2d_fwd_rows_seg(const float* xp, const float* wp, const float* bias, const float* sigma0, const float* sigma1,
+                                       const float* sigma2, int n0, int n1, int n2, const float* residual, float* y,
+                                       const gim_conv_shape* s, void* stream) {
+    int rc = rows_shape_ok(s);
+    if (rc) return rc;
+    Segs sg;
+    rc = segs_fill(sg, s, sigma0, sigma1, sigma2, n0, n1, n2);
+    return rc ? rc : rows_seg_impl(xp, wp, bias, sg, residual, y, s, stream, nullptr);
+}
+
+static int dgrad_seg_impl(const float* dy, const float* w, const Segs& sg, const float* mask_x, const float* res_half, float res_scale,
+                          float* dx, const gim_conv_shape* s, int transposed, void* stream, int32_t* plan) {
+    GIM_CHECK_ARG(dy && w && dx, "conv dgrad (segmented): null pointer");
+    if (res_half) {
+        GIM_CHECK_ARG(!transposed && !s->ups && !s->pool && !s->wfold && s->H >= 2 && s->W >= 2 && mask_x,
+                      "conv dgrad (segmented, + half-resolution residual): plain k-major convolutions on maps of >= 2 x 2 with mask_x only");
+    }
+    size_t xi, yi;
+    image_elems(s, true, xi, yi);
+    const bool tiny = !transposed && !res_half && tiny_route(s);
+    if (!tiny && fits_one_launch(s, xi, yi)) {
+        ConvCall c;
+        IgemmPlan q;
+        const int rc = dgrad_call(c, dy, w, sg.sigma[0], mask_x, dx, s, transposed != 0, res_half, res_scale);
+        if (rc) return rc;
+        if (seg_plan_merged(c, q, sg)) return plan ? seg_plan_row(q, plan) : run_planned(c, q, stream, "gim_conv2d_dgrad_seg");
+    }
+    if (plan) return SEG_PLAN_FALLBACK;
+    size_t n = 0;
+    for (int i = 0; i < sg.n; n += sg.images[i++]) {
+        gim_conv_shape h = *s;
+        h.N = sg.images[i];
+        const int rc = dgrad_impl(dy + n * yi, w, sg.sigma[i], mask_x ? mask_x + n * xi : nullptr, dx + n * xi, &h, stream, transposed != 0,
+                                  res_half ? res_half + n * (xi / 4) : nullptr, res_scale);
+        if (rc) return rc;
+    }
+    return GIM_OK;
+}
+
+extern "C" int gim_conv2d_dgrad_seg(const float* dy, const float* w, const float* sigma0, const float* sigma1, const float* sigma2,
+                                    int n0, int n1, int n2, const float* mask_x, const float* res_half, float res_scale, float* dx,
+                                    const gim_conv_shape* s, int transposed, void* stream) {
+    int rc = check_shape(s);
+    if (rc) return rc;
+    Segs sg;
+    rc = segs_fill(sg, s, sigma0, sigma1, sigma2, n0, n1, n2);
+    return rc ? rc : dgrad_seg_impl(dy, w, sg, mask_x, res_half, res_scale, dx, s, transposed, stream, nullptr);
+}
+
 template <int VA, int VB, bool FASTB>
 static void launch_wgrad(const WgP& p, int bm, int bn, int bk, dim3 g, hipStream_t st) {
     if constexpr (VA == 4 && VB == 4) {
@@ -2427,6 +2591,40 @@
     return launch_plan(s, kind, out);
 }
 
+extern "C" int gim_conv_launch_plan_seg(const gim_conv_shape* s, int kind, int n0, int n1, int n2, int32_t* out) {
+    GIM_CHECK_ARG(s && out && (kind == 0 || kind == 1 || kind == 2 || kind == 4), "conv_launch_plan_seg: bad args");
+    for (int i = 0; i < 9; ++i) out[i] = -1;
+    float* const fake = reinterpret_cast<float*>(uintptr_t(4096));
+    int rc = kind == 4 ? rows_shape_ok(s) : check_shape(s);
+    if (rc) return rc;
+    Segs sg;
+    rc = segs_fill(sg, s, nullptr, nullptr, nullptr, n0, n1, n2);
+    if (rc) return rc;
+    if (kind == 0) rc = fwd_seg_impl(fake, fake, nullptr, sg, nullptr, fake, s, nullptr, out);
+    else if (kind == 4) rc = rows_seg_impl(fake, fake, nullptr, sg, nullptr, fake, s, nullptr, out);
+    else rc = dgrad_seg_impl(fake, fake, sg, nullptr, nullptr, 0.f, fake, s, kind == 2, nullptr, out);
+    out[8] = rc == GIM_OK ? 1 : 0;
+    if (rc != SEG_PLAN_FALLBACK) return rc;
+    int ks = 1;
+    for (int i = 0; i < sg.n; ++i) {
+        gim_conv_shape h = *s;
+        h.N = sg.images[i];
+        if (kind == 4) {
+            ConvCall c;
+            rc = rows_call(c, fake, fake, nullptr, nullptr, nullptr, fake, &h);
+            if (rc) return rc;
+            const IgemmPlan q = plan_igemm(c.p, c.bmode, c.gen);
+            plan_row(out, q.table_hit, q.BM, q.BN, q.ksplit, q.gx, q.gy, q.gz, 0);
+        } else {
+            rc = launch_plan(&h, kind, out);
+            if (rc) return rc;
+        }
+        if (out[3] > ks) ks = out[3];
+    }
+    out[3] = ks;
+    return GIM_OK;
+}
+
 
 extern "C" int gim_conv2d_strided_fwd(const float* x, const float* w, const float* bias, float* y, const gim_infer_conv* s, void* stream) {
     const int rc = check_infer_conv(s, "conv2d_strided_fwd", true);
diff --git a/optimalstrategiesagainstgenerativeattacks_amd/gim_img_models.py b/optimalstrategiesagainstgenerativeattacks_amd/gim_img_models.py
--- a/optimalstrategiesagainstgenerativeattacks_amd/gim_img_models.py
+++ b/optimalstrategiesagainstgenerativeattacks_amd/gim_img_models.py
@@ -12,6 +12,7 @@
 _TWO_STREAMS = os.environ.get("GIM_SINGLE_STREAM") is None
 _PER_SAMPLE_STREAMS = os.environ.get("GIM_PER_SAMPLE_STREAMS") is not None
 _LANE1_SIDE = os.environ.get("GIM_NO_LANE1_SIDE") is None
+_MERGE_SETS = os.environ.get("GIM_NO_MERGED_SETS") is None
 _STREAMS = {}
 
 
@@ -323,6 +324,8 @@
         return self.dis(test_src=test_src, test_env=test_env, si_src=si_src, si_env=si_env)
 
     def encode_samples(self, samples):
+        if self._merges(samples):
+            return self._encode_merged(samples)
         cur = torch.cuda.current_stream()
         if not _use_side_streams(samples[0]):
             return ([self.src_encode_sample(s) for s in samples], [self.env_encode_sample(s) for s in samples])
@@ -341,6 +344,36 @@
                 smp.record_stream(st)
                 feats.append(f)
             outs.append(feats)
+        for st in streams:
+            ops.stream_wait(cur, st)
+        return outs[0], outs[1]
+
+    @staticmethod
+    def _merges(samples):
+        return (_MERGE_SETS and not _PER_SAMPLE_STREAMS and 2 <= len(samples) <= 3 and all(s.is_cuda and not s.requires_grad for s in samples)
+                and all(s.shape[2:] == samples[0].shape[2:] for s in samples))
+
+    def _encode_merged(self, samples):
+        cur = torch.cuda.current_stream()
+        counts = [s.size(0) * s.size(1) for s in samples]
+        x = ops.to_nhwc(torch.cat([s.reshape(n, *s.shape[2:]) for s, n in zip(samples, counts)]))
+
+        def encode(enc):
+            with ops.merged_sets(counts):
+                f = enc(x)
+            return [p.view(s.size(0), s.size(1), -1) for p, s in zip(f.split(counts), samples)]
+        if not _use_side_streams(samples[0]):
+            return encode(self.src_encoder), encode(self.env_encoder)
+        streams = _side_streams(samples[0].device, 2)
+        outs = []
+        for st, enc in zip(streams, (self.src_encoder, self.env_encoder)):
+            ops.stream_wait(st, cur)
+            with torch.cuda.stream(st):
+                feats = encode(enc)
+            for f in feats:
+                f.record_stream(cur)
+            outs.append(feats)
+            x.record_stream(st)
         for st in streams:
             ops.stream_wait(cur, st)
         return outs[0], outs[1]
diff --git a/optimalstrategiesagainstgenerativeattacks_amd/model_blocks.py b/optimalstrategiesagainstgenerativeattacks_amd/model_blocks.py
--- a/optimalstrategiesagainstgenerativeattacks_amd/model_blocks.py
+++ b/optimalstrategiesagainstgenerativeattacks_amd/model_blocks.py
@@ -138,8 +138,16 @@
             ops.weight_phys(self.weight_orig), self.out_channels, self.in_channels, self.kernel_size))
 
     def forward(self, x, res=None, ups=0, pre_slope=1.0, pool=False, res_ups=False, post_slope=1.0, x_act=False, fork_pool_slope=None):
-        guard = None
-        if self._sn_queue:
+        guard = seg = None
+        counts = ops.merged_counts()
+        if counts is not None:
+            if len(self._sn_queue) < len(counts):
+                raise RuntimeError("merged sample sets: %d spectral-norm rounds are queued for a conv that stands for %d calls "
+                                   "(prefetch_spectral must run one round per set)" % (len(self._sn_queue), len(counts)))
+            ents = [self._sn_queue.popleft() for _ in counts]
+            sigma, u_s, v_s, guard = ents[0]
+            seg = ops.Seg(counts, tuple(e[0] for e in ents), tuple(e[1] for e in ents), tuple(e[2] for e in ents))
+        elif self._sn_queue:
             sigma, u_s, v_s, guard = self._sn_queue.popleft()
         elif _SN_REPLAY[0] is not None:
             sigma, u_s, v_s = self._sn_tape.next(_SN_REPLAY[0], None, lambda: ops.spectral_sigma(
@@ -148,11 +156,11 @@
             sigma, u_s, v_s = ops.spectral_sigma(self.weight_orig, self.weight_u, self.weight_v, self.training)
         if fork_pool_slope is not None:
             assert res is None and not ups and not pool and not res_ups
-            return ops.conv2d_forkpool(x, self.weight_orig, self.bias, sigma, u_s, v_s, pre_slope, guard, post_slope, x_act, fork_pool_slope)
+            return ops.conv2d_forkpool(x, self.weight_orig, self.bias, sigma, u_s, v_s, pre_slope, guard, post_slope, x_act, fork_pool_slope, seg)
         wf = self.folded() if (pool or (ups and self.kernel_size > 1)) else None
         if post_slope != 1.0:
-            return ops.conv2d_post_act(x, self.weight_orig, self.bias, res, sigma, u_s, v_s, ups, pre_slope, pool, res_ups, wf, guard, post_slope, x_act)
-        return ops.conv2d(x, self.weight_orig, self.bias, res, sigma, u_s, v_s, ups, pre_slope, pool, res_ups, wf, guard, x_act)
+            return ops.conv2d_post_act(x, self.weight_orig, self.bias, res, sigma, u_s, v_s, ups, pre_slope, pool, res_ups, wf, guard, post_slope, x_act, seg)
+        return ops.conv2d(x, self.weight_orig, self.bias, res, sigma, u_s, v_s, ups, pre_slope, pool, res_ups, wf, guard, x_act, seg)
 
     def extra_repr(self):
         return "%d, %d, kernel_size=%d (spectral norm)" % (self.in_channels, self.out_channels, self.kernel_size)
diff --git a/optimalstrategiesagainstgenerativeattacks_amd/ops.py b/optimalstrategiesagainstgenerativeattacks_amd/ops.py
--- a/optimalstrategiesagainstgenerativeattacks_amd/ops.py
+++ b/optimalstrategiesagainstgenerativeattacks_amd/ops.py
@@ -290,8 +290,68 @@
     return v
 
 
-def _conv_out(sh, plan_kind, key, shape, device):
-    if _ZERO_POOL and _launch_plan(sh, plan_kind, key).ksplit > 1 and not torch.cuda.is_current_stream_capturing():
+Seg = collections.namedtuple("Seg", "counts sigmas us vs")
+_MERGED_SETS = [None]
+_SegPlan = collections.namedtuple("_SegPlan", "ksplit merged")
+
+
+class merged_sets:
+    def __init__(self, counts):
+        self.counts = tuple(int(c) for c in counts)
+        if not (2 <= len(self.counts) <= 3 and all(c > 0 for c in self.counts)):
+            raise ValueError("merged_sets: two or three sets of at least one image (got %r)" % (self.counts,))
+
+    def __enter__(self):
+        self.prev = _MERGED_SETS[0]
+        _MERGED_SETS[0] = self.counts
+
+    def __exit__(self, *exc):
+        _MERGED_SETS[0] = self.prev
+
+
+def merged_counts():
+    return _MERGED_SETS[0]
+
+
+def _seg_counts3(counts):
+    return counts[0], counts[1], counts[2] if len(counts) == 3 else 0
+
+
+def _seg_args(seg):
+    s = seg.sigmas
+    return (_p(s[0]), _p(s[1]), _p(s[2]) if len(s) == 3 else None) + _seg_counts3(seg.counts)
+
+
+def _seg_plan(sh, plan_kind, key, counts):
+    k_ = (plan_kind, counts) + key
+    v = _SPLITS_K.get(k_)
+    if v is None:
+        out = (ctypes.c_int32 * 9)()
+        check(_lib.load().gim_conv_launch_plan_seg(ctypes.byref(sh), plan_kind, *_seg_counts3(counts), ctypes.cast(out, ctypes.c_void_p)),
+              "conv_launch_plan_seg")
+        v = _SPLITS_K[k_] = _SegPlan(out[3], out[8] == 1)
+    return v
+
+
+def _ksplit(sh, plan_kind, key, counts=None):
+    return _launch_plan(sh, plan_kind, key).ksplit if counts is None else _seg_plan(sh, plan_kind, key, counts).ksplit
+
+
+def _seg_geom(g, n):
+    return g._replace(N=n, key=(n,) + g.key[1:])
+
+
+def _note_seg_conv(kind, geom, sh, plan_kind, counts):
+    if _seg_plan(sh, plan_kind, geom.key, counts).merged:
+        return _note_conv(kind, geom)
+    for n in counts:
+        shn = GimConvShape.from_buffer_copy(sh)
+        shn.N = n
+        _note_conv(kind, _seg_geom(geom, n), shn, plan_kind)
+
+
+def _conv_out(sh, plan_kind, key, shape, device, counts=None):
+    if _ZERO_POOL and _ksplit(sh, plan_kind, key, counts) > 1 and not torch.cuda.is_current_stream_capturing():
         sh.out_zeroed = 1
         return _zeros_from_pool(shape, device)
     return torch.empty(shape, device=device, dtype=torch.float32)
@@ -626,22 +686,29 @@
     return ("direct" if (ns == 1 and not has_sigma and not g.fold and not has_target) else "slabs"), ns
 
 
-def _stores_activated(g, post_slope):
+def _stores_activated(g, post_slope, counts=None):
     if not (_ACT_STORAGE and post_slope != 1.0) or g.linear:
         return False
     gl, sh = _fwd_launch(g)
-    return _fwd_route(g, sh.tune_tile) == "subpixel" or _launch_plan(sh, 0, gl.key).ksplit == 1
+    return _fwd_route(g, sh.tune_tile) == "subpixel" or _ksplit(sh, 0, gl.key, counts) == 1
 
 
 def _merged_subpixel(x, w, ups, res, sh):
     return _fwd_route(ConvGeom.of(x, w, ups, 1.0, False, False, None, res, False), sh.tune_tile) == "subpixel"
 
 
+def _conv_fwd(lib, x, w, bias, sigma, res, y, sh, seg):
+    if seg is None:
+        check(lib.gim_conv2d_fwd(_p(x), _p(w), _p(bias), _p(sigma), _p(res), _p(y), sh, _stream()), "conv2d_fwd")
+    else:
+        check(lib.gim_conv2d_fwd_seg(_p(x), _p(w), _p(bias), *_seg_args(seg), _p(res), _p(y), sh, _stream()), "conv2d_fwd_seg")
+
+
 class ConvFn(Function):
-    N_EXTRA = 11
-
-    @staticmethod
-    def forward(ctx, x, w, bias, res, sigma, u_s, v_s, ups, pre_slope, pool, res_ups, wf=None, guard=None, post_slope=1.0, x_act=False):
+    N_EXTRA = 12
+
+    @staticmethod
+    def forward(ctx, x, w, bias, res, sigma, u_s, v_s, ups, pre_slope, pool, res_ups, wf=None, guard=None, post_slope=1.0, x_act=False, seg=None):
         lib = _lib.load()
         x = _req(x, "x")
         wp = weight_phys(_req_w(w))
@@ -650,8 +717,14 @@
         tap_slope = 1.0 if x_act else pre_slope
         gl, sh = _fwd_launch(g, tap_slope)
         route = _fwd_route(g, sh.tune_tile)
+        counts = None
+        if seg is not None:
+            counts = seg.counts
+            if sum(counts) != N or route == "subpixel":
+                raise RuntimeError("conv: a segmented call needs runs that add up to the batch (%r of %d images) and is not the "
+                                   "stacked sub-pixel form" % (counts, N))
         if post_slope != 1.0 and route != "subpixel":
-            if g.linear or _launch_plan(sh, 0, gl.key).ksplit > 1:
+            if g.linear or _ksplit(sh, 0, gl.key, counts) > 1:
                 raise RuntimeError("conv: an activated output (post_slope) cannot be combined with a split-K launch or a linear layer")
             sh.post_slope = post_slope
         if res is not None:
@@ -664,7 +737,10 @@
             wrows = _transposed(lib, w, wp, Cout, Cin, KH, rows=True)
             sh.tune_ksplit = 1
             y = torch.empty(g.out_shape, device=x.device, dtype=torch.float32)
-            check(lib.gim_conv2d_fwd_rows(_p(xp), _p(wrows), _p(bias), _p(sigma), _p(res), _p(y), sh, _stream()), "conv2d_fwd_rows")
+            if seg is not None:
+                check(lib.gim_conv2d_fwd_rows_seg(_p(xp), _p(wrows), _p(bias), *_seg_args(seg), _p(res), _p(y), sh, _stream()), "conv2d_fwd_rows_seg")
+            else:
+                check(lib.gim_conv2d_fwd_rows(_p(xp), _p(wrows), _p(bias), _p(sigma), _p(res), _p(y), sh, _stream()), "conv2d_fwd_rows")
         elif route == "subpixel":
             if wf is None:
                 wf = _folded(wp, Cout, Cin, KH)
@@ -678,18 +754,22 @@
         elif gl is not g:
             xp = torch.empty((N, H + 1, W + 1, Cin), device=x.device, dtype=torch.float32)
             check(lib.gim_box2_fwd(_p(x), _p(xp), N, H, W, Cin, tap_slope, _stream()), "box2_fwd")
-            y = _conv_out(sh, 0, gl.key, g.out_shape, x.device)
-            check(lib.gim_conv2d_fwd(_p(xp), _p(wp), _p(bias), _p(sigma), _p(res), _p(y), sh, _stream()), "conv2d_fwd")
+            y = _conv_out(sh, 0, gl.key, g.out_shape, x.device, counts)
+            _conv_fwd(lib, xp, wp, bias, sigma, res, y, sh, seg)
         else:
-            y = _conv_out(sh, 0, g.key, g.out_shape, x.device)
+            y = _conv_out(sh, 0, g.key, g.out_shape, x.device, counts)
             if g.fold and wf is None:
                 wf = _folded(wp, Cout, Cin, KH)
-            check(lib.gim_conv2d_fwd(_p(x), _p(wf if g.fold else wp), _p(bias), _p(sigma), _p(res), _p(y), sh, _stream()), "conv2d_fwd")
+            _conv_fwd(lib, x, wf if g.fold else wp, bias, sigma, res, y, sh, seg)
         ctx.save_for_backward(x, w, sigma, u_s, v_s, wf if g.fold else None, bias, xp)
         ctx.cfg = g
         ctx.guard = guard
+        ctx.seg = seg
         if _FLOPS is not None:
-            _note_conv("fwd", gl, sh, 0)
+            if seg is None:
+                _note_conv("fwd", gl, sh, 0)
+            else:
+                _note_seg_conv("fwd", gl, sh, 4 if route == "rows" else 0, counts)
         return y
 
     @staticmethod
@@ -702,11 +782,15 @@
             raise RuntimeError("the spectral-norm state (sigma, u, v) of this forward pass was overwritten by later forward "
                                "passes of the same model: run backward before the third forward")
         need = ctx.needs_input_grad
+        seg = ctx.seg
         box = g.pool and xp is not None
         if g.fold and wf is None and need[0]:
             with torch.no_grad():
                 wf = _folded(weight_phys(w), g.Cout, g.Cin, g.KH)
         if _second_order():
+            if seg is not None:
+                raise NotImplementedError("second-order backward of a segmented convolution (merged sample sets): the R1 path encodes "
+                                          "its sample sets one by one")
             if g.ups or g.res_ups:
                 raise NotImplementedError("second-order backward of an upsampling convolution is not on the R1 path")
             dx = ConvDgradFn.apply(dy, w, x, sigma, u_s, v_s, wf, g) if need[0] else None
@@ -716,13 +800,22 @@
         dev = dy.device
         dx = dw = db = dres = None
         if need[0]:
-            dx = _conv_dgrad(lib, dy, x, wp, wf, sigma, g.shape("dgrad"), g, st, w, getattr(ctx, "dgrad_res", None))
+            dx = _conv_dgrad(lib, dy, x, wp, wf, sigma, g.shape("dgrad"), g, st, w, getattr(ctx, "dgrad_res", None), seg)
         want_b = g.has_bias and need[2]
-        if need[1] and box:
-            gb = g.box()
-            dw, db = _conv_wgrad(lib, dy, xp, w, wp, bias, sigma, u_s, v_s, gb.shape("wgrad"), gb, want_b, st)
-        elif need[1]:
-            dw, db = _conv_wgrad(lib, dy, x, w, wp, bias, sigma, u_s, v_s, g.shape("wgrad", 1.0 if g.x_act else None), g, want_b, st, xp)
+        if need[1]:
+            gw, xw, xpw = (g.box(), xp, None) if box else (g, x, xp)
+            slope_w = None if box else (1.0 if g.x_act else None)
+            if seg is None:
+                dw, db = _conv_wgrad(lib, dy, xw, w, wp, bias, sigma, u_s, v_s, gw.shape("wgrad", slope_w), gw, want_b, st, xpw)
+            else:
+                n0 = 0
+                for n, sg_, us_, vs_ in zip(seg.counts, seg.sigmas, seg.us, seg.vs):
+                    gn = _seg_geom(gw, n)
+                    dwn, dbn = _conv_wgrad(lib, dy[n0:n0 + n], xw[n0:n0 + n], w, wp, bias, sg_, us_, vs_, gn.shape("wgrad", slope_w), gn, want_b,
+                                           st, None if xpw is None else xpw[n0:n0 + n])
+                    dw = dwn if dw is None else (dw if dwn is None else dw + dwn)
+                    db = dbn if db is None else (db if dbn is None else db + dbn)
+                    n0 += n
         elif want_b:
             db = torch.empty(g.Cout, device=dev, dtype=torch.float32)
             scratch = torch.empty(256 * g.Cout, device=dev, dtype=torch.float32)
@@ -784,10 +877,18 @@
     return _WT_CACHE.get(w, (KF, layout), make, raw)
 
 
-def _conv_dgrad(lib, dy, x, wp, wf, sigma, sh, g, st, w=None, res_half=None):
+def _conv_dgrad(lib, dy, x, wp, wf, sigma, sh, g, st, w=None, res_half=None, seg=None):
     route, J, add_res = _dgrad_route(g, sh.prec, w is not None, res_half is not None)
+    counts = None
+    if seg is not None:
+        counts = seg.counts
+        if route in ("xfold", "ups"):
+            raise RuntimeError("conv dgrad: no segmented form of the %r route (image layers, 1x1 behind an upsample)" % route)
     if _FLOPS is not None:
-        _note_conv("dgrad", g, sh, 1)
+        if seg is None:
+            _note_conv("dgrad", g, sh, 1)
+        else:
+            _note_seg_conv("dgrad", g, sh, 2 if route == "t" else 1, counts)
     N, H, W, Cin, Cout, KH = g.N, g.H, g.W, g.Cin, g.Cout, g.KH
     mask = x if g.pre_slope != 1.0 else None
     wk = wf if g.fold else wp
@@ -797,16 +898,23 @@
         check(lib.gim_conv2d_dgrad_xfold(_p(dy), _p(wx), _p(sigma), _p(mask), _p(dx), sh, J, st), "conv2d_dgrad_xfold")
     elif route == "t":
         wt = _transposed(lib, w, wk, Cout, Cin, KH + 1 if g.fold else KH)
-        dx = _conv_out(sh, 2, g.key, tuple(x.shape), x.device)
-        check(lib.gim_conv2d_dgrad_t(_p(dy), _p(wt), _p(sigma), _p(mask), _p(dx), sh, st), "conv2d_dgrad_t")
+        dx = _conv_out(sh, 2, g.key, tuple(x.shape), x.device, counts)
+        if seg is not None:
+            check(lib.gim_conv2d_dgrad_seg(_p(dy), _p(wt), *_seg_args(seg), _p(mask), None, 0.0, _p(dx), sh, 1, st), "conv2d_dgrad_seg")
+        else:
+            check(lib.gim_conv2d_dgrad_t(_p(dy), _p(wt), _p(sigma), _p(mask), _p(dx), sh, st), "conv2d_dgrad_t")
     elif route == "ups":
         dxu = _conv_out(sh, 1, g.key, (N, H, W, Cin), dy.device)
         dx = torch.empty_like(x)
         check(lib.gim_conv2d_dgrad(_p(dy), _p(wk), _p(sigma), None, _p(dxu), sh, st), "conv2d_dgrad")
         check(lib.gim_upsample2x_bwd(_p(dxu), _p(mask), g.pre_slope, _p(dx), N, H >> 1, W >> 1, Cin, st), "upsample2x_bwd")
     else:
-        dx = _conv_out(sh, 1, g.key, tuple(x.shape), x.device)
-        if route == "res":
+        dx = _conv_out(sh, 1, g.key, tuple(x.shape), x.device, counts)
+        if seg is not None:
+            rh = _p(_req(res_half, "res_half")) if route == "res" else None
+            check(lib.gim_conv2d_dgrad_seg(_p(dy), _p(wk), *_seg_args(seg), _p(mask), rh, 0.25 if route == "res" else 0.0, _p(dx), sh, 0, st),
+                  "conv2d_dgrad_seg")
+        elif route == "res":
             check(lib.gim_conv2d_dgrad_res(_p(dy), _p(wk), _p(sigma), _p(mask), _p(_req(res_half, "res_half")), 0.25, _p(dx), sh, st), "conv2d_dgrad_res")
         else:
             check(lib.gim_conv2d_dgrad(_p(dy), _p(wk), _p(sigma), _p(mask), _p(dx), sh, st), "conv2d_dgrad")
@@ -943,23 +1051,24 @@
 
 
 def conv2d(x, w, bias=None, res=None, sigma=None, u_s=None, v_s=None, ups=0, pre_slope=1.0, pool=False, res_ups=False, wf=None,
-           guard=None, x_act=False):
-    return ConvFn.apply(x, w, bias, res, sigma, u_s, v_s, ups, pre_slope, pool, res_ups, wf, guard, 1.0, x_act)
+           guard=None, x_act=False, seg=None):
+    return ConvFn.apply(x, w, bias, res, sigma, u_s, v_s, ups, pre_slope, pool, res_ups, wf, guard, 1.0, x_act, seg)
 
 
 def conv2d_post_act(x, w, bias=None, res=None, sigma=None, u_s=None, v_s=None, ups=0, pre_slope=1.0, pool=False, res_ups=False, wf=None,
-                    guard=None, post_slope=1.0, x_act=False):
-    act = post_slope != 1.0 and _stores_activated(ConvGeom.of(x, w, ups, pre_slope, pool, res_ups, bias, res, x_act), post_slope)
-    y = ConvFn.apply(x, w, bias, res, sigma, u_s, v_s, ups, pre_slope, pool, res_ups, wf, guard, post_slope if act else 1.0, x_act)
+                    guard=None, post_slope=1.0, x_act=False, seg=None):
+    act = post_slope != 1.0 and _stores_activated(ConvGeom.of(x, w, ups, pre_slope, pool, res_ups, bias, res, x_act), post_slope,
+                                                  seg.counts if seg is not None else None)
+    y = ConvFn.apply(x, w, bias, res, sigma, u_s, v_s, ups, pre_slope, pool, res_ups, wf, guard, post_slope if act else 1.0, x_act, seg)
     return y, act
 
 
 class ConvForkPoolFn(Function):
 
     @staticmethod
-    def forward(ctx, x, w, bias, res, sigma, u_s, v_s, ups, pre_slope, pool, res_ups, wf, guard, post_slope, x_act, in_slope):
+    def forward(ctx, x, w, bias, res, sigma, u_s, v_s, ups, pre_slope, pool, res_ups, wf, guard, post_slope, x_act, seg, in_slope):
         x, pooled = _avgpool2(x, in_slope)
-        y = ConvFn.forward(ctx, x, w, bias, None, sigma, u_s, v_s, 0, pre_slope, False, False, None, guard, post_slope, x_act)
+        y = ConvFn.forward(ctx, x, w, bias, None, sigma, u_s, v_s, 0, pre_slope, False, False, None, guard, post_slope, x_act, seg)
         return y, pooled
 
     @staticmethod
@@ -983,14 +1092,15 @@
 _FUSED_FORKPOOL = os.environ.get("GIM_NO_FUSED_FORKPOOL") is None
 
 
-def conv2d_forkpool(x, w, bias, sigma, u_s, v_s, pre_slope, guard, post_slope, x_act, in_slope):
-    act = post_slope != 1.0 and _stores_activated(ConvGeom.of(x, w, 0, pre_slope, False, False, bias, None, x_act), post_slope)
+def conv2d_forkpool(x, w, bias, sigma, u_s, v_s, pre_slope, guard, post_slope, x_act, in_slope, seg=None):
+    act = post_slope != 1.0 and _stores_activated(ConvGeom.of(x, w, 0, pre_slope, False, False, bias, None, x_act), post_slope,
+                                                  seg.counts if seg is not None else None)
     ps = post_slope if act else 1.0
     if _FUSED_FORKPOOL and x.requires_grad and torch.is_grad_enabled():
-        y, pooled = ConvForkPoolFn.apply(x, w, bias, None, sigma, u_s, v_s, 0, pre_slope, False, False, None, guard, ps, x_act, in_slope)
+        y, pooled = ConvForkPoolFn.apply(x, w, bias, None, sigma, u_s, v_s, 0, pre_slope, False, False, None, guard, ps, x_act, seg, in_slope)
     else:
         xa, pooled = fork_pool(x, in_slope)
-        y = ConvFn.apply(xa, w, bias, None, sigma, u_s, v_s, 0, pre_slope, False, False, None, guard, ps, x_act)
+        y = ConvFn.apply(xa, w, bias, None, sigma, u_s, v_s, 0, pre_slope, False, False, None, guard, ps, x_act, seg)
     return y, act, pooled
 
 
```
